# qq456cvb/CanonicalVoting

Measured on AMD Instinct MI355X. Metric: scenes/sec (80k-pt synthetic scans), higher is better.
Workload: dtype f32

## Files before the change

canonicalvoting_amd/_lib.py:

```python
import ctypes
import os
import threading

_HERE = os.path.dirname(os.path.abspath(__file__))
LIB_PATH = os.path.join(_HERE, "_C", "libcvhip.so")

c_float_p = ctypes.POINTER(ctypes.c_float)
c_int_p = ctypes.POINTER(ctypes.c_int)
c_i32_p = ctypes.POINTER(ctypes.c_int32)
c_i64_p = ctypes.POINTER(ctypes.c_int64)
vp = ctypes.c_void_p
ABI_VERSION = 6


class CvError(RuntimeError):
    pass


class DecodeParams(ctypes.Structure):
    _fields_ = [("thresh_high", ctypes.c_float), ("thresh_low", ctypes.c_float),
                ("valid_ratio", ctypes.c_float), ("elimination", ctypes.c_int),
                ("prob_thresh", ctypes.c_float), ("elim_hi_plus1", ctypes.c_int),
                ("max_iters", ctypes.c_int), ("err_thresh", ctypes.c_double)]

# ... 214 lines not shown
    "cv_hv_forward_workspace_bytes": (ctypes.c_size_t, [ctypes.c_int64, ctypes.c_int, c_int_p, ctypes.c_int]),
    "cv_hv_forward_f32": (ctypes.c_int, [vp, vp, vp, vp, ctypes.c_int64, ctypes.c_float, ctypes.c_int,
                                         c_float_p, c_int_p, vp, vp, vp, vp, ctypes.c_size_t,
                                         ctypes.c_int, vp]),
    "cv_hv_forward_cat_workspace_bytes": (ctypes.c_size_t, [ctypes.c_int64, ctypes.c_int, c_int_p, ctypes.c_int, ctypes.c_int]),
    "cv_hv_forward_cat_f32": (ctypes.c_int, [vp, vp, vp, vp, ctypes.c_int64, ctypes.c_float, ctypes.c_int, c_float_p, c_int_p,
                                             ctypes.c_int, vp, vp, vp, vp, ctypes.c_size_t, ctypes.c_int, vp]),
    "cv_hv_forward_peaks_f32": (ctypes.c_int, [vp, vp, vp, vp, ctypes.c_int64, ctypes.c_float, ctypes.c_int,
                                               c_float_p, c_int_p, vp, vp, vp, vp, ctypes.c_size_t,
                                               ctypes.c_int, ctypes.c_float, vp]),
    "cv_hv_forward_peaks_cat_f32": (ctypes.c_int, [vp, vp, vp, vp, ctypes.c_int64, ctypes.c_float, ctypes.c_int, c_float_p, c_int_p,
                                                   ctypes.c_int, vp, vp, vp, vp, ctypes.c_size_t, ctypes.c_int, ctypes.c_float,
                                                   vp]),
    "cv_hv_set_kernel_events": (ctypes.c_int, [vp, vp]),
    "cv_hv_backward_f32": (ctypes.c_int, [vp, vp, vp, vp, vp, ctypes.c_int64, ctypes.c_float,
                                          ctypes.c_int, c_float_p, c_int_p, vp, vp, vp, vp]),
    "cv_hv_count_votes_f32": (ctypes.c_int, [vp, vp, vp, ctypes.c_int64, ctypes.c_float, ctypes.c_int,
                                             c_float_p, c_int_p, c_i64_p, vp, ctypes.c_size_t, vp]),
    "cv_prop_workspace_bytes": (ctypes.c_size_t, [ctypes.c_int]),
    "cv_prop_columns_f32": (ctypes.c_int, [vp, c_int_p, ctypes.c_double, vp, vp, vp, vp, vp]),
    "cv_prop_select_f32": (ctypes.c_int, [ctypes.POINTER(PropSelectDesc), vp]),
    "cv_prop_cloud_ranges_i32": (ctypes.c_int, [vp, ctypes.c_longlong, ctypes.c_int, vp, vp, vp]),
    "cv_sizeof_prop_select_desc": (ctypes.c_size_t, []),
    "cv_decode_workspace_bytes": (ctypes.c_size_t, [c_int_p, ctypes.c_int64, ctypes.c_int]),
    "cv_decode_f32": (ctypes.c_int, [vp, vp, vp, c_int_p, c_float_p, ctypes.c_float, vp, vp, vp, vp,
                                     ctypes.c_int64, ctypes.POINTER(DecodeParams), ctypes.c_int, vp,
                                     ctypes.c_size_t, c_int_p, c_i64_p, c_i32_p, c_int_p, c_float_p,
                                     c_float_p, c_i32_p, c_int_p, vp]),
    "cv_decode_cat_workspace_bytes": (ctypes.c_size_t, [c_int_p, ctypes.c_int64, ctypes.c_int, ctypes.c_int]),
    "cv_decode_cat_f32": (ctypes.c_int, [vp, vp, vp, c_int_p, c_float_p, ctypes.c_float, vp, vp, vp, vp, ctypes.c_int64,
                                         ctypes.c_int, ctypes.POINTER(DecodeParams), ctypes.c_int, vp, ctypes.c_size_t, c_int_p,
                                         c_i64_p, c_i32_p, c_int_p, c_float_p, c_float_p, c_i32_p, c_int_p, vp]),
    "cv_detect_scene_separate_f32": (ctypes.c_int, [ctypes.POINTER(SceneSeparateDesc), ctypes.POINTER(SceneSeparateResult), vp]),
    "cv_sp_table_capacity": (ctypes.c_longlong, [ctypes.c_longlong]),
    "cv_sp_levels_workspace_bytes": (ctypes.c_size_t, [ctypes.c_longlong]),
    "cv_sp_build_levels": (ctypes.c_int, [ctypes.POINTER(vp), ctypes.POINTER(vp), ctypes.POINTER(vp),
                                          ctypes.c_longlong, ctypes.c_longlong, ctypes.c_int, vp,
                                          c_i32_p, vp, ctypes.c_size_t, vp]),
    "cv_sp_quantize_workspace_bytes": (ctypes.c_size_t, [ctypes.c_longlong]),
    "cv_sp_quantize_f32": (ctypes.c_int, [vp, ctypes.c_longlong, ctypes.c_longlong, ctypes.c_float, ctypes.c_int, c_i64_p,
                                          ctypes.c_int, vp, vp, vp, vp, c_i32_p, vp, ctypes.c_size_t, vp]),
    "cv_sp_quantize_f64": (ctypes.c_int, [vp, ctypes.c_longlong, ctypes.c_longlong, ctypes.c_double, ctypes.c_int, c_i64_p,
                                          ctypes.c_int, vp, vp, vp, vp, c_i32_p, vp, ctypes.c_size_t, vp]),
    "cv_sp_voxel_rows_f32": (ctypes.c_int, [vp, vp, ctypes.c_longlong, ctypes.c_float, vp, ctypes.POINTER(GatherJob), ctypes.c_int, vp]),
    "cv_sizeof_gather_job": (ctypes.c_size_t, []),
    "cv_sp_scan_rows_f32": (ctypes.c_int, [ctypes.POINTER(ScanRowsDesc), vp]),
    "cv_sizeof_scan_rows_desc": (ctypes.c_size_t, []),
    "cv_sym_loss_fwd_f32": (ctypes.c_int, [ctypes.POINTER(SymLossDesc), vp]),
    "cv_sym_loss_bwd_f32": (ctypes.c_int, [ctypes.POINTER(SymLossDesc), vp]),
    "cv_sym_loss_workspace_bytes": (ctypes.c_size_t, [ctypes.c_longlong, ctypes.c_int]),
    "cv_sym_loss_chunk_rows": (ctypes.c_int, []),
    "cv_sizeof_sym_loss_desc": (ctypes.c_size_t, []),
    "cv_row_loss_fwd_f32": (ctypes.c_int, [ctypes.POINTER(RowLossDesc), vp]),
    "cv_row_loss_bwd_f32": (ctypes.c_int, [ctypes.POINTER(RowLossDesc), vp]),
    "cv_row_loss_workspace_bytes": (ctypes.c_size_t, [ctypes.c_longlong]),
    "cv_row_loss_chunk_rows": (ctypes.c_int, []),
    "cv_sizeof_row_loss_desc": (ctypes.c_size_t, []),
    "cv_sp_sym_rows_f32": (ctypes.c_int, [ctypes.POINTER(SymRowsDesc), vp]),
    "cv_sp_sym_rows_workspace_bytes": (ctypes.c_size_t, [ctypes.c_longlong, ctypes.c_longlong, ctypes.c_int, ctypes.c_int]),
    "cv_sp_sym_rows_block": (ctypes.c_int, []),
    "cv_sp_sym_rows_scan_span": (ctypes.c_longlong, []),
    "cv_sizeof_sym_rows_desc": (ctypes.c_size_t, []),
    "cv_sp_morton_keys": (ctypes.c_int, [vp, ctypes.c_longlong, vp, vp]),
    "cv_sp_sort_workspace_bytes": (ctypes.c_size_t, [ctypes.c_longlong]),
    "cv_sp_sort_rows": (ctypes.c_int, [vp, ctypes.c_longlong, vp, vp, vp, vp, ctypes.c_size_t, vp]),
    "cv_sp_pack_weights_stem_h2_f32": (ctypes.c_int, [vp, ctypes.c_int, ctypes.c_int, vp, ctypes.c_int, vp, vp]),
    "cv_sp_to_hl_f32": (ctypes.c_int, [vp, ctypes.c_longlong, ctypes.c_int, ctypes.c_int, vp, ctypes.c_int, vp, vp]),
    "cv_sp_from_hl_f32": (ctypes.c_int, [vp, ctypes.c_longlong, ctypes.c_int, ctypes.c_int, vp, ctypes.c_int, vp]),
    "cv_sp_kernel_map": (ctypes.c_int, [vp, ctypes.c_longlong, vp, vp, ctypes.c_longlong, ctypes.c_int,
                                        ctypes.c_int, vp, vp]),
    "cv_sp_up_map": (ctypes.c_int, [vp, ctypes.c_longlong, ctypes.c_longlong, vp, vp]),
    "cv_sp_conv_workspace_bytes": (ctypes.c_size_t, [ctypes.c_longlong, ctypes.c_int, ctypes.c_int]),
    "cv_sp_conv_f32": (ctypes.c_int, [ctypes.POINTER(ConvDesc), vp]),
    "cv_sp_set_split_target": (ctypes.c_int, [ctypes.c_int]),
    "cv_hv_set_part_records": (ctypes.c_int, [ctypes.c_int]),
    "cv_hv_set_part_records_thread": (ctypes.c_int, [ctypes.c_int]),
    "cv_sp_pack_weights_h2_batch_f32": (ctypes.c_int, [ctypes.POINTER(PackJob), ctypes.c_int, vp, vp]),
    "cv_sp_copy_unless_flag": (ctypes.c_int, [ctypes.POINTER(vp), ctypes.POINTER(vp), ctypes.POINTER(ctypes.c_longlong), ctypes.c_int, vp, vp]),
    "cv_sp_pack_weights_t_f32": (ctypes.c_int, [vp, ctypes.c_int, ctypes.c_int, ctypes.c_int, ctypes.c_int, ctypes.c_int, vp, vp]),
    "cv_sp_set_split_target_thread": (ctypes.c_int, [ctypes.c_int]),
    "cv_sp_set_ablation": (ctypes.c_int, [ctypes.c_int]),
    "cv_sp_set_option": (ctypes.c_int, [ctypes.c_char_p, ctypes.c_longlong, ctypes.POINTER(ctypes.c_longlong)]),
    "cv_sp_get_option": (ctypes.c_int, [ctypes.c_char_p, ctypes.POINTER(ctypes.c_longlong)]),
    "cv_sp_pack_weights_x6_f32": (ctypes.c_int, [vp, ctypes.c_int, ctypes.c_int, ctypes.c_int, vp, vp, vp]),
    "cv_sp_pack_weights_h2_f32": (ctypes.c_int, [vp, ctypes.c_int, ctypes.c_int, ctypes.c_int, vp, ctypes.c_int, vp, vp]),
    "cv_sp_pack_weights_bf16_f32": (ctypes.c_int, [vp, ctypes.c_int, ctypes.c_int, ctypes.c_int, vp, vp, vp]),
    "cv_sp_scene_maps_words": (ctypes.c_size_t, [c_i64_p, ctypes.c_longlong, ctypes.c_int, ctypes.c_int,
                                                 ctypes.c_longlong, ctypes.POINTER(SceneMaps)]),
    "cv_sp_scene_maps": (ctypes.c_int, [ctypes.POINTER(vp), ctypes.POINTER(vp), ctypes.POINTER(vp), ctypes.c_longlong,
                                        c_i64_p, vp, ctypes.c_longlong, ctypes.c_int,
                                        ctypes.c_int, ctypes.c_longlong, vp, ctypes.c_size_t, vp]),
    "cv_sp_scene_plan_words": (ctypes.c_size_t, [ctypes.c_longlong, ctypes.c_int, ctypes.c_int, ctypes.c_longlong]),
    "cv_sp_scene_plan": (ctypes.c_int, [vp, ctypes.c_longlong, vp, vp, ctypes.POINTER(vp), ctypes.POINTER(vp),
                                        ctypes.POINTER(vp), ctypes.c_longlong, vp, c_i32_p, ctypes.c_int, ctypes.c_int,
                                        ctypes.c_longlong, vp, ctypes.c_size_t, ctypes.POINTER(SceneMaps), vp,
                                        ctypes.c_size_t, vp, ctypes.c_size_t, vp]),
    "cv_sp_scene_plan_layout": (ctypes.c_int, [ctypes.c_longlong, ctypes.c_int, ctypes.c_int, ctypes.c_longlong,
                                               ctypes.POINTER(ScenePlanLayout)]),
    "cv_sp_scene_plan_slots": (ctypes.c_int, [ctypes.POINTER(ScenePlanLayout), ctypes.POINTER(SceneMaps), c_i64_p,
                                              ctypes.c_longlong, vp, ctypes.POINTER(vp), ctypes.POINTER(vp)]),
    "cv_sp_scene_conv_workspace_bytes": (ctypes.c_size_t, [c_i64_p, c_int_p, ctypes.c_int, ctypes.c_int]),
    "cv_net_arena_bytes": (ctypes.c_size_t, [ctypes.POINTER(NetBuf), ctypes.c_int, c_i64_p, ctypes.c_int]),
    "cv_net_run_f32": (ctypes.c_int, [ctypes.POINTER(NetOp), ctypes.c_int, ctypes.POINTER(NetBuf), ctypes.c_int,
                                      c_i64_p, ctypes.c_int, vp, ctypes.c_size_t, ctypes.POINTER(vp), c_int_p,
                                      ctypes.POINTER(vp), ctypes.c_int, ctypes.POINTER(vp), ctypes.c_int,
                                      vp, ctypes.c_size_t, vp, vp]),
    "cv_net_models_params_bytes": (ctypes.c_size_t, [ctypes.c_int, ctypes.c_int]),
    "cv_net_models_params_fill": (ctypes.c_int, [ctypes.POINTER(vp), ctypes.c_int, ctypes.c_int, vp, ctypes.c_size_t]),
    "cv_net_models_arena_bytes": (ctypes.c_size_t, [ctypes.POINTER(NetBuf), ctypes.c_int, c_i64_p, ctypes.c_int, ctypes.c_int]),
    "cv_net_models_workspace_bytes": (ctypes.c_size_t, [ctypes.c_size_t, ctypes.c_int]),
    "cv_net_run_models_f32": (ctypes.c_int, [ctypes.POINTER(vp), ctypes.POINTER(vp), ctypes.c_int, ctypes.c_int, ctypes.c_int,
                                             c_i64_p, ctypes.c_int, vp, ctypes.c_size_t, ctypes.POINTER(vp), c_int_p,
                                             ctypes.POINTER(vp), ctypes.c_int, ctypes.POINTER(vp), ctypes.c_int,
                                             vp, ctypes.c_size_t, vp, vp, ctypes.c_int, vp]),
    "cv_head_separate_models_f32": (ctypes.c_int, [ctypes.POINTER(vp), ctypes.c_int, ctypes.c_longlong, ctypes.c_int, ctypes.c_int,
                                                   vp, vp, vp, vp]),
    "cv_sp_mask_keys": (ctypes.c_int, [vp, ctypes.c_longlong, ctypes.c_int, ctypes.c_int, ctypes.c_int, vp, vp]),
    "cv_sp_mask_perms": (ctypes.c_int, [vp, ctypes.c_longlong, ctypes.c_int, ctypes.c_int, vp, vp, ctypes.c_size_t,
                                        ctypes.c_int, vp]),
    "cv_sp_transpose_map": (ctypes.c_int, [vp, ctypes.c_longlong, ctypes.c_int, ctypes.c_longlong, vp, vp]),
    "cv_sp_wgrad_workspace_bytes": (ctypes.c_size_t, [ctypes.c_longlong, ctypes.c_int, ctypes.c_int, ctypes.c_int]),
    "cv_sp_conv_wgrad_f32": (ctypes.c_int, [vp, ctypes.c_int, ctypes.c_int, vp, ctypes.c_int, ctypes.c_int, vp,
                                            ctypes.c_int, ctypes.c_longlong, vp, vp, ctypes.c_size_t, vp]),
    "cv_sp_conv_wgrad_px_f32": (ctypes.c_int, [vp, ctypes.c_int, ctypes.c_int, vp, ctypes.c_int, ctypes.c_int, vp,
                                               ctypes.c_int, ctypes.c_longlong, vp, vp, ctypes.c_size_t, ctypes.c_int,
                                               vp]),
    "cv_sp_col_sum_f32": (ctypes.c_int, [vp, ctypes.c_longlong, ctypes.c_int, ctypes.c_int, vp, vp]),
    "cv_sp_col_sum_workspace_bytes": (ctypes.c_size_t, [ctypes.c_longlong, ctypes.c_int]),
    "cv_sp_col_sum_det_f32": (ctypes.c_int, [vp, ctypes.c_longlong, ctypes.c_int, ctypes.c_int, vp, vp, ctypes.c_size_t, vp]),
    "cv_sp_bn_workspace_bytes": (ctypes.c_size_t, [ctypes.c_int]),
    "cv_sp_bn_stats_f32": (ctypes.c_int, [vp, ctypes.c_longlong, ctypes.c_int, ctypes.c_int, vp, vp, ctypes.c_float,
                                          ctypes.c_float, vp, vp, vp, vp, vp, vp, vp, ctypes.c_size_t, vp]),
    "cv_sp_bn_backward_f32": (ctypes.c_int, [vp, vp, vp, ctypes.c_longlong, ctypes.c_int, ctypes.c_int, vp, vp,
                                             ctypes.c_float, vp, vp, vp, vp, vp, vp, ctypes.c_size_t, vp]),
    "cv_sp_bn_backward_hl_f32": (ctypes.c_int, [vp, vp, vp, ctypes.c_longlong, ctypes.c_int, ctypes.c_int, vp, vp,
                                                ctypes.c_float, vp, vp, vp, vp, vp, vp, ctypes.c_size_t, vp, vp, vp, vp, vp]),
    "cv_sp_affine_f32": (ctypes.c_int, [vp, ctypes.c_longlong, ctypes.c_int, ctypes.c_int, vp, vp, vp, ctypes.c_int,
                                        ctypes.c_int, vp, ctypes.c_int, vp]),
    "cv_sp_affine_hl_f32": (ctypes.c_int, [vp, ctypes.c_longlong, ctypes.c_int, ctypes.c_int, vp, vp, vp, ctypes.c_int,
                                           ctypes.c_int, vp, ctypes.c_int, vp, ctypes.c_int, vp, vp, vp]),
    "cv_sp_bn_fold_f32": (ctypes.c_int, [vp, vp, vp, vp, vp, ctypes.c_float, ctypes.c_int, vp, vp, vp]),
    "cv_head_joint_f32": (ctypes.c_int, [vp, ctypes.c_longlong, ctypes.c_int, ctypes.c_int, ctypes.c_int,
                                         vp, vp, vp, vp, vp]),
    "cv_head_separate_f32": (ctypes.c_int, [vp, ctypes.c_longlong, ctypes.c_int, ctypes.c_int, vp, vp, vp, vp]),
    "cv_detect_scene_f32": (ctypes.c_int, [ctypes.POINTER(SceneDesc), ctypes.POINTER(SceneResult), vp]),
    "cv_detect_points_f32": (ctypes.c_int, [ctypes.POINTER(PointsDesc), ctypes.POINTER(PointsResult), vp]),
    "cv_detect_points_separate_f32": (ctypes.c_int, [ctypes.POINTER(PointsSeparateDesc), ctypes.POINTER(PointsSeparateResult), vp]),
    "cv_sizeof_points_desc": (ctypes.c_size_t, []),
    "cv_sizeof_points_separate_desc": (ctypes.c_size_t, []),
    "cv_sizeof_points_result": (ctypes.c_size_t, []),
    "cv_sizeof_points_separate_result": (ctypes.c_size_t, []),
    "cv_iou_obb": (ctypes.c_double, [c_float_p, c_float_p]),
    "cv_nms_obb": (ctypes.c_int, [c_float_p, c_float_p, ctypes.c_int, ctypes.c_double, c_i32_p]),
}

_lib = None


def lib():
    global _lib
    if _lib is None:
        if not os.path.exists(LIB_PATH):
            raise CvError(
                "canonicalvoting_amd: HIP library %s not found. Build it with "
                "`python -m canonicalvoting_amd.csrc.build` (hipcc, gfx950). There is no CPU "
                "fallback for this op." % LIB_PATH)
# ... 60 lines not shown
```

canonicalvoting_amd/csrc/conv_prep.hip:

```cpp
#include "cv_common.h"

#include <algorithm>

#include "sparse_conv_common.h"

using namespace cvsc;

namespace {

__global__ __launch_bounds__(256) void pack_weights_h2(const float* __restrict__ w, int K, int cin, int cout,
                                                       const float* __restrict__ col_scale, float mult,
                                                       unsigned short* __restrict__ wp, int trans = 0) {
    const long long total = (long long)K * cin * cout / 2;
    const int nch = cin / 32;
    for (long long i = blockIdx.x * 256ll + threadIdx.x; i < total; i += (long long)gridDim.x * 256) {
        long long r = i;
        const int k2 = (int)(r % 16); r /= 16;
        const int col = (int)(r % cout); r /= cout;
        const int c = (int)(r % nch); r /= nch;
        const int j = (int)r;
        const float* p = trans ? w + ((long long)j * cout + col) * cin + c * 32 + 2 * k2
                               : w + ((long long)j * cin + c * 32 + 2 * k2) * cout + col;
        const float sc = (col_scale ? col_scale[col] : 1.f) * mult;
        unsigned h, l;
// ... 30 lines not shown

__global__ __launch_bounds__(256) void pack_weights_x6(const float* __restrict__ w, int K, int cin, int cout,
                                                       const float* __restrict__ col_scale,
                                                       unsigned short* __restrict__ wp, int trans = 0) {
    const long long total = (long long)K * cin * cout / 2;
    const int nch = cin / 32;
    for (long long i = blockIdx.x * 256ll + threadIdx.x; i < total; i += (long long)gridDim.x * 256) {
        long long r = i;
        const int k2 = (int)(r % 16); r /= 16;
        const int col = (int)(r % cout); r /= cout;
        const int c = (int)(r % nch); r /= nch;
        const int j = (int)r;
        const float* p = trans ? w + ((long long)j * cout + col) * cin + c * 32 + 2 * k2
                               : w + ((long long)j * cin + c * 32 + 2 * k2) * cout + col;
        unsigned h, m, l;
        const float sc = col_scale ? col_scale[col] : 1.f;
        split3(p[0] * sc, p[trans ? 1 : cout] * sc, h, m, l);
        const long long base = ((long long)(j * nch + c) * 3 * cout + col) * 32 + 2 * k2;
        *reinterpret_cast<unsigned*>(wp + base) = h;
        *reinterpret_cast<unsigned*>(wp + base + (long long)cout * 32) = m;
        *reinterpret_cast<unsigned*>(wp + base + 2ll * cout * 32) = l;
    }
}

__global__ __launch_bounds__(256) void pack_weights_b1(const float* __restrict__ w, int K, int cin, int cout,
                                                       const float* __restrict__ col_scale,
                                                       unsigned short* __restrict__ wp, int trans = 0) {
    const long long total = (long long)K * cin * cout / 2;
    const int nch = cin / 32;
    for (long long i = blockIdx.x * 256ll + threadIdx.x; i < total; i += (long long)gridDim.x * 256) {
        long long r = i;
        const int k2 = (int)(r % 16); r /= 16;
        const int col = (int)(r % cout); r /= cout;
        const int c = (int)(r % nch); r /= nch;
        const int j = (int)r;
        const float* p = trans ? w + ((long long)j * cout + col) * cin + c * 32 + 2 * k2
                               : w + ((long long)j * cin + c * 32 + 2 * k2) * cout + col;
        const float sc = col_scale ? col_scale[col] : 1.f;
        *reinterpret_cast<unsigned*>(wp + ((long long)(j * nch + c) * cout + col) * 32 + 2 * k2) =
            cvt_pk_bf16(p[0] * sc, p[trans ? 1 : cout] * sc);
    }
}

__global__ __launch_bounds__(256) void pack_weights_stem_h2(const float* __restrict__ w, int K, int cin,
                                                            const float* __restrict__ col_scale, float mult,
                                                            unsigned short* __restrict__ wp) {
    const int total = 8 * cin * 32 * 2 * 4;
    for (int t = blockIdx.x * 256 + threadIdx.x; t < total; t += gridDim.x * 256) {
        int r = t;
        const int q = r % 4; r /= 4;
        const int hf = r % 2; r /= 2;
        const int col = r % 32; r /= 32;
        const int ci = r % cin; r /= cin;
        const int g = r;
        const int j0 = g * 16 + hf * 8 + 2 * q;
        const float sc = (col_scale ? col_scale[col] : 1.f) * mult;
        const float v0 = j0 < K ? w[((long long)j0 * cin + ci) * 32 + col] * sc : 0.f;
        const float v1 = j0 + 1 < K ? w[((long long)(j0 + 1) * cin + ci) * 32 + col] * sc : 0.f;
        unsigned h, l;
        split2h(v0, v1, h, l);
        const long long base = ((((long long)(g * cin + ci) * 2) * 32 + col) * 2 + hf) * 8 + 2 * q;
        *reinterpret_cast<unsigned*>(wp + base) = h;
        *reinterpret_cast<unsigned*>(wp + base + 512) = l;
    }
}

__global__ __launch_bounds__(256) void mask_keys(const int* __restrict__ nbr, long long n, int K, int j_begin,
                                                 int j_end, long long* __restrict__ keys) {
    const long long i = blockIdx.x * 256ll + threadIdx.x;
    if (i >= n) return;
    unsigned long long m = 0;
    for (int j = j_begin; j < j_end; ++j)
        if (nbr[i * K + j] >= 0) m |= 1ull << (j - j_begin);
    keys[i] = (long long)m;
}

constexpr int MP_BINS = 1024;
constexpr int MP_THREADS = 1024;

__device__ __forceinline__ int group_mask(const int* __restrict__ nbr, long long row, long long n, int K, int jb, int je) {
    int m = 0;
    for (int j = jb; j < je; ++j)
        if (nbr[row * K + j] >= 0) m |= 1 << (j - jb);
    if (je - jb <= 7) m |= __popc(m) << 7;
    (void)n;
    return m;
}

__device__ __forceinline__ int group_mask_of_word(int word, int jb, int je) {
    int m = (int)(((unsigned)word >> jb) & ((1u << (je - jb)) - 1u));
    if (je - jb <= 7) m |= __popc(m) << 7;
    return m;
}

__global__ __launch_bounds__(MP_THREADS) void mp_hist(const int* __restrict__ nbr, long long n, int K, int groups,
                                                      int* __restrict__ hist ) {
    __shared__ int lh[MP_BINS];
    const int g = blockIdx.y;
    const int jb = K * g / groups, je = K * (g + 1) / groups;
    for (int i = threadIdx.x; i < MP_BINS; i += MP_THREADS) lh[i] = 0;
    __syncthreads();
    const long long row = blockIdx.x * (long long)MP_THREADS + threadIdx.x;
    if (row < n) atomicAdd(&lh[group_mask(nbr, row, n, K, jb, je)], 1);
    __syncthreads();
    for (int i = threadIdx.x; i < MP_BINS; i += MP_THREADS)
        if (lh[i]) atomicAdd(&hist[g * MP_BINS + i], lh[i]);
}

__global__ __launch_bounds__(MP_BINS) void mp_scan(int* __restrict__ hist) {
    __shared__ int s[MP_BINS];
    int* h = hist + blockIdx.x * MP_BINS;
    const int v = h[threadIdx.x];
    s[threadIdx.x] = v;
    __syncthreads();
    for (int off = 1; off < MP_BINS; off <<= 1) {
        const int t = threadIdx.x >= off ? s[threadIdx.x - off] : 0;
        __syncthreads();
        s[threadIdx.x] += t;
        __syncthreads();
    }
    h[threadIdx.x] = s[threadIdx.x] - v;
}

__global__ __launch_bounds__(MP_THREADS) void mp_scatter(const int* __restrict__ nbr, long long n, int K, int groups,
                                                         int* __restrict__ cursor, int* __restrict__ perm,
                                                         int* __restrict__ nbrp, int W) {
    unsigned char* gv = nbrp ? reinterpret_cast<unsigned char*>(nbrp + (long long)groups * n * W) : nullptr;
    __shared__ int lh[MP_BINS];
    const int g = blockIdx.y;
    const int jb = K * g / groups, je = K * (g + 1) / groups;
    for (int i = threadIdx.x; i < MP_BINS; i += MP_THREADS) lh[i] = 0;
    __syncthreads();
    const long long row = blockIdx.x * (long long)MP_THREADS + threadIdx.x;
    int key = 0, rank = 0;
    if (row < n) {
        key = group_mask(nbr, row, n, K, jb, je);
        rank = atomicAdd(&lh[key], 1);
    }
    __syncthreads();
    for (int i = threadIdx.x; i < MP_BINS; i += MP_THREADS)
        if (lh[i]) lh[i] = atomicAdd(&cursor[g * MP_BINS + i], lh[i]);
    __syncthreads();
    if (row < n) {
        const long long pos = (long long)g * n + lh[key] + rank;
        perm[pos] = (int)row;
        if (nbrp) {
            for (int j = jb; j < je; ++j) nbrp[pos * W + (j - jb)] = nbr[row * K + j];
            gv[(long long)g * n + row] = key != 0;
        }
    }
}

struct PermJobsDev {
    CvPermJob j[CV_MAX_PERM_JOBS];
    int group_begin[CV_MAX_PERM_JOBS + 1];
    int n;
};

__device__ __forceinline__ int perm_job_of(const PermJobsDev& jobs, int gy) {
    int ji = 0;
    while (ji + 1 < jobs.n && gy >= jobs.group_begin[ji + 1]) ++ji;
    return ji;
}

__global__ __launch_bounds__(MP_THREADS) void mp_hist_batch(const PermJobsDev jobs, int* __restrict__ hist) {
    __shared__ int lh[MP_BINS];
    const int ji = perm_job_of(jobs, blockIdx.y);
    const CvPermJob& jb = jobs.j[ji];
    const long long row = blockIdx.x * (long long)MP_THREADS + threadIdx.x;
    if (blockIdx.x * (long long)MP_THREADS >= jb.n) return;
    const int g = blockIdx.y - jobs.group_begin[ji];
    const int jlo = jb.K * g / jb.groups, jhi = jb.K * (g + 1) / jb.groups;
    for (int i = threadIdx.x; i < MP_BINS; i += MP_THREADS) lh[i] = 0;
    __syncthreads();
// ... 230 lines not shown
```

canonicalvoting_amd/csrc/cv_common.h:

```cpp
#pragma once
#include <hip/hip_runtime.h>

#include <cstdarg>
#include <cstdint>
#include <cstdio>

#include "cv_hip.h"

void cv_set_error(const char* fmt, ...);

#define CV_HIP_CHECK(expr)                                                                  \
    do {                                                                                    \
        hipError_t e_ = (expr);                                                             \
        if (e_ != hipSuccess) {                                                             \
            cv_set_error("%s failed: %s (%s:%d)", #expr, hipGetErrorString(e_), __FILE__,   \
                         __LINE__);                                                         \
            return CV_EHIP;                                                                 \
        }                                                                                   \
    } while (0)

#define CV_LAUNCH_CHECK() CV_HIP_CHECK(hipGetLastError())

#define CV_REQUIRE(cond, code, ...)     \
    do {                                \
        if (!(cond)) {                  \
            cv_set_error(__VA_ARGS__);  \
            return (code);              \
        }                               \
    } while (0)

__host__ __device__ static inline size_t cv_align_up(size_t v, size_t a) { return (v + a - 1) / a * a; }

struct CvCarver {
    char* base;
    size_t off = 0;
    explicit CvCarver(void* p) : base(static_cast<char*>(p)) {}
    template <typename T>
    T* take(size_t count) {
        off = cv_align_up(off, 256);
        T* r = reinterpret_cast<T*>(base + off);
        off += count * sizeof(T);
        return r;
    }
};

struct CvMapJob {
    const int32_t* out_coords; long long n_out;
    const unsigned long long* keys; const int32_t* vals; long long cap;
    int k, ts;
    int32_t* nbr;
    const int32_t* compose;
    const unsigned* bitmap;
    const int32_t* bbox;
    int up;
    int32_t* nbr3;
    int32_t* mask_words;
};
constexpr int CV_MAX_MAP_JOBS = 12;
int cv_sp_kernel_maps_batch(const CvMapJob* jobs, int n_jobs, void* stream);
constexpr long long CV_BITMAP_WORDS = 1ll << 20;

int cv_sp_build_levels_zero(int32_t* const* d_coords, unsigned long long* const* d_keys, int32_t* const* d_vals,
                            long long n, long long cap, int num_levels, int32_t* d_counts, int32_t* h_counts, void* d_ws,
                            size_t ws_bytes, int32_t* d_zero, long long n_zero, int32_t* d_bbox, uint32_t* d_bits,
                            void* stream);

struct CvPermJob {
    const int32_t* nbr; long long n; int K, groups; int32_t* perm; int with_map;
    const int32_t* mask_words;
};
constexpr int CV_MAX_PERM_JOBS = 8;
int cv_hv_minmax_async_ex(const float* d_points, int64_t n, float* h_minmax6, void* d_ws, size_t ws_bytes, int32_t* d_zero_word,
                          int32_t* d_fill7f, void* stream);
struct DecodeCall {
    float* d_grid_obj; const float* d_grid_rot; const float* d_grid_scale;
    const int* dims; const float* h_corner3; float res;
    const float* d_points; const float* d_xyz; const float* d_prob; const int32_t* d_class; int64_t n;
    const cv_decode_params* params; int mutate_grid;
    void* d_ws; size_t ws_bytes;
    int* h_n_cand; int64_t* h_cand_idx; int32_t* h_verdict; int* h_n_boxes; float* h_boxes; float* h_scores; int32_t* h_classes;
    int* h_truncated;
    void* stream; void* ev_done;
};
int cv_decode_run(const DecodeCall& c, int num_cats, bool need_class);
int cv_sp_sort_rows_ex(const int32_t* d_coords, long long n, int32_t* d_sorted, int32_t* d_perm, int32_t* d_inv, void* d_ws,
                       size_t ws_bytes, bool single_batch, void* stream, bool bounds_prefilled);
int cv_sp_scene_plan_ex(const int32_t* d_input, long long n, int32_t* d_perm, int32_t* d_inv, int32_t* const* d_coords,
                        unsigned long long* const* d_keys, int32_t* const* d_vals, long long cap, int32_t* d_counts,
                        int32_t* h_counts, int stem_k, int mask_groups, long long masked_min_rows,
                        int32_t* d_arena, size_t arena_words, cv_scene_maps* offsets, void* d_sort_ws, size_t sort_ws_bytes,
                        void* d_levels_ws, size_t levels_ws_bytes, bool single_batch, void* stream,
                        bool bounds_prefilled);
int cv_net_run_ex(const cv_net_op* ops, int n_ops, const cv_net_buf* bufs, int n_bufs, const long long* level_rows,
                  int n_levels, void* d_arena, size_t arena_bytes, const void* const* ext_ptr, const int* ext_ld,
                  const int32_t* const* maps, int n_maps, const int32_t* const* perms, int n_perms,
                  void* d_ws, size_t ws_bytes, int32_t* range_flag, bool plan_maps, void* stream);
int cv_net_run_models_ex(const cv_net_op* const* ops, const cv_net_buf* const* bufs, int n_ops, int n_bufs, int K,
                         const long long* level_rows, int n_levels, void* d_arena, size_t arena_bytes,
                         const void* const* const* ext_ptr, const int* ext_ld, const int32_t* const* maps, int n_maps,
                         const int32_t* const* perms, int n_perms, void* d_ws, size_t ws_bytes, int32_t* range_flag,
                         const void* d_params, int params_ld, bool plan_maps, void* stream);
int cv_sp_mask_perms_batch(const CvPermJob* jobs, int n_jobs, void* d_ws, size_t ws_bytes, void* stream,
                           bool pre_zeroed);

struct CvConvModels {
    int models;
    const cv_net_model_params* d_params;
    long long in_stride, in2_stride, res_stride, out_stride, ws_stride;
    int out_ext;
    float* ext_out[CV_MAX_CATEGORIES];
};
int cv_sp_conv_models_f32(const cv_conv_desc* d, const CvConvModels* mm, void* stream);
```

canonicalvoting_amd/csrc/net_exec.cpp:

```cpp
#include <algorithm>
#include <mutex>
#include <unordered_map>
#include <vector>

#include "cv_common.h"

namespace {

struct Slot { char* ptr; int ld; long long rows; int ext; };

struct NetModels {
    int K;
    const void* const* const* ext_ptr;
    size_t arena_stride, ws_stride;
    const cv_net_model_params* d_params;
    int params_ld;
};

int net_run(const cv_net_op* ops, int n_ops, const cv_net_buf* bufs, int n_bufs, const long long* level_rows, int n_levels,
            void* d_arena, size_t arena_bytes, const void* const* ext_ptr, const int* ext_ld, const int32_t* const* maps,
            int n_maps, const int32_t* const* perms, int n_perms, void* d_ws, size_t ws_bytes, int32_t* range_flag,
            const NetModels* nm, bool plan_maps, void* stream);

}

extern "C" {

static void scene_maps_layout(const long long* rows, int stem_k, int mask_groups, long long masked_min_rows, cv_scene_maps* o,
                              size_t* total) {
    size_t off = 0;
    auto take = [&](size_t words) { const size_t at = off; off += cv_align_up(words, 64); return (long long)at; };
    const size_t K5 = (size_t)stem_k * stem_k * stem_k;
    const size_t mp_w = mask_groups > 1 ? (size_t)mask_groups * (1 + (27 + mask_groups - 1) / mask_groups) + (mask_groups + 3) / 4 : 0;
    o->stem = take((size_t)rows[0] * K5);
    o->k3[0] = take((size_t)rows[0] * 28);
    o->mask_perm[0] = (mask_groups > 1 && rows[0] >= masked_min_rows) ? take(mp_w * rows[0]) : -1;
    o->scratch = take((size_t)(5 * std::max(mask_groups, 1) + 4) * 2048);
    o->bitmap = take((size_t)CV_BITMAP_WORDS);
    o->out = -1;
    for (int i = 0; i < 4; ++i) o->down[i] = take((size_t)rows[i + 1] * 8);
    for (int i = 1; i < 5; ++i) o->k3[i] = take((size_t)rows[i] * 28);
    for (int i = 0; i < 4; ++i) o->up[i] = take((size_t)rows[3 - i] * 8);
    for (int i = 1; i < 5; ++i) o->mask_perm[i] = (mask_groups > 1 && rows[i] >= masked_min_rows) ? take(mp_w * rows[i]) : -1;
    for (int i = 0; i < 4; ++i) o->up_perm[i] = take((size_t)rows[3 - i]);
    *total = off;
}

static int32_t* scene_mask_words(int32_t* d_arena, const cv_scene_maps& o, int level, long long rows) {
    return d_arena + o.k3[level] + rows * 27;
}

size_t cv_sp_scene_maps_words(const long long* level_rows, long long n_orig, int stem_k, int mask_groups,
                              long long masked_min_rows, cv_scene_maps* offsets) {
    if (!level_rows || !offsets || n_orig <= 0 || stem_k < 1) return 0;
    size_t total = 0;
    scene_maps_layout(level_rows, stem_k, mask_groups, masked_min_rows, offsets, &total);
    return total;
}

static int scene_maps_level0(int32_t* const* d_coords, const unsigned long long* const* d_keys, const int32_t* const* d_vals,
                             long long cap, long long n, const int32_t* d_perm, int stem_k, int mask_groups,
                             const cv_scene_maps& o, int32_t* d_arena, const int32_t* d_bbox, void* stream) {
    const unsigned* bits = d_bbox ? reinterpret_cast<const unsigned*>(d_arena + o.bitmap) : nullptr;
    CvMapJob mj[2];
    int32_t* mw = scene_mask_words(d_arena, o, 0, n);
    int nm = 1;
    if (stem_k == 5) {
        mj[0] = {d_coords[0], n, d_keys[0], d_vals[0], cap, 5, 1, d_arena + o.stem, d_perm, bits, d_bbox, 0, d_arena + o.k3[0], mw};
    } else {
        mj[0] = {d_coords[0], n, d_keys[0], d_vals[0], cap, stem_k, 1, d_arena + o.stem, d_perm, bits, d_bbox, 0, nullptr, nullptr};
        mj[1] = {d_coords[0], n, d_keys[0], d_vals[0], cap, 3, 1, d_arena + o.k3[0], nullptr, bits, d_bbox, 0, nullptr, mw};
        nm = 2;
    }
    int rc = cv_sp_kernel_maps_batch(mj, nm, stream);
    if (rc != CV_OK) return rc;
    if (o.mask_perm[0] >= 0) {
        CvPermJob pj = {d_arena + o.k3[0], n, 27, mask_groups, d_arena + o.mask_perm[0], 1, mw};
        rc = cv_sp_mask_perms_batch(&pj, 1, d_arena + o.scratch, sizeof(int) * (size_t)mask_groups * 2048, stream,
                                     d_bbox != nullptr);
        if (rc != CV_OK) return rc;
    }
    return CV_OK;
}

static int scene_maps_coarse(int32_t* const* d_coords, const unsigned long long* const* d_keys, const int32_t* const* d_vals,
                             long long cap, const long long* level_rows, int mask_groups, const cv_scene_maps& o,
                             int32_t* d_arena, void* stream, bool from_plan) {
    CvMapJob mj[CV_MAX_MAP_JOBS];
    int nm = 0;
    for (int i = 0; i < 4; ++i)
        mj[nm++] = {d_coords[i + 1], level_rows[i + 1], d_keys[i], d_vals[i], cap, 2, 1 << i, d_arena + o.down[i], nullptr, nullptr, nullptr, 0,
                    nullptr, nullptr};
    for (int i = 1; i < 5; ++i)
        mj[nm++] = {d_coords[i], level_rows[i], d_keys[i], d_vals[i], cap, 3, 1 << i, d_arena + o.k3[i], nullptr, nullptr, nullptr, 0,
                    nullptr, o.mask_perm[i] >= 0 ? scene_mask_words(d_arena, o, i, level_rows[i]) : nullptr};
    for (int i = 0; i < 4; ++i) {
        const int fine = 3 - i;
        mj[nm++] = {d_coords[fine], level_rows[fine], d_keys[fine + 1], d_vals[fine + 1], cap, 2, 1 << fine, d_arena + o.up[i],
                    nullptr, nullptr, nullptr, 1, nullptr, nullptr};
    }
    int rc = cv_sp_kernel_maps_batch(mj, nm, stream);
    if (rc != CV_OK) return rc;
    CvPermJob pj[CV_MAX_PERM_JOBS];
    int np = 0, groups = 0;
    for (int i = 1; i < 5; ++i)
        if (o.mask_perm[i] >= 0) {
            pj[np++] = {d_arena + o.k3[i], level_rows[i], 27, mask_groups, d_arena + o.mask_perm[i], 1,
                        scene_mask_words(d_arena, o, i, level_rows[i])};
            groups += mask_groups;
        }
    for (int i = 0; i < 4; ++i) {
        pj[np++] = {d_arena + o.up[i], level_rows[3 - i], 8, 1, d_arena + o.up_perm[i], 0, nullptr};
        groups += 1;
    }
    return cv_sp_mask_perms_batch(pj, np, d_arena + o.scratch + (size_t)std::max(mask_groups, 1) * 2048,
                                  sizeof(int) * (size_t)groups * 2048, stream,  from_plan);
}

int cv_sp_scene_maps(int32_t* const* d_coords, const unsigned long long* const* d_keys, const int32_t* const* d_vals,
                     long long cap, const long long* level_rows, const int32_t* d_perm, long long n_orig, int stem_k,
                     int mask_groups, long long masked_min_rows, int32_t* d_arena, size_t arena_words, void* stream) {
    CV_REQUIRE(d_coords && d_keys && d_vals && level_rows && d_perm && d_arena, CV_EINVAL, "null pointer argument");
    CV_REQUIRE(n_orig == level_rows[0], CV_EINVAL, "the sorted set must hold the caller's %lld rows", n_orig);
    cv_scene_maps o;
    size_t total = 0;
    scene_maps_layout(level_rows, stem_k, mask_groups, masked_min_rows, &o, &total);
    CV_REQUIRE(arena_words >= total, CV_ENOMEM, "scene map arena too small");
    int rc = scene_maps_level0(d_coords, d_keys, d_vals, cap, n_orig, d_perm, stem_k, mask_groups, o, d_arena,
                                nullptr, stream);
    if (rc != CV_OK) return rc;
    return scene_maps_coarse(d_coords, d_keys, d_vals, cap, level_rows, mask_groups, o, d_arena, stream,  false);
}

namespace {
struct PlanSide { hipEvent_t ev; int32_t* h_pinned; int device; };
std::mutex g_plan_mu;
std::unordered_map<int, std::vector<PlanSide>> g_plan_free;
int plan_side_acquire(PlanSide* out) {
    int dev = 0;
    CV_HIP_CHECK(hipGetDevice(&dev));
    {
        std::lock_guard<std::mutex> lk(g_plan_mu);
        auto& pool = g_plan_free[dev];
        if (!pool.empty()) {
            *out = pool.back();
            pool.pop_back();
            return CV_OK;
        }
    }
    PlanSide p{};
    p.device = dev;
    CV_HIP_CHECK(hipEventCreateWithFlags(&p.ev, hipEventDisableTiming));
    CV_HIP_CHECK(hipHostMalloc(reinterpret_cast<void**>(&p.h_pinned), 64, hipHostMallocDefault));
    *out = p;
    return CV_OK;
}
struct PlanSideLease {
    PlanSide ps{};
    bool held = false;
    ~PlanSideLease() {
        if (!held) return;
        (void)hipEventSynchronize(ps.ev);
        std::lock_guard<std::mutex> lk(g_plan_mu);
        g_plan_free[ps.device].push_back(ps);
    }
};
}

size_t cv_sp_scene_plan_words(long long n, int stem_k, int mask_groups, long long masked_min_rows) {
    if (n <= 0 || stem_k < 1) return 0;
    const long long rows[5] = {n, n, n, n, n};
    cv_scene_maps o;
    size_t total = 0;
    scene_maps_layout(rows, stem_k, mask_groups, masked_min_rows, &o, &total);
    return total;
}

int cv_sp_scene_plan_layout(long long n, int stem_k, int mask_groups, long long masked_min_rows, cv_scene_plan_layout* out) {
    CV_REQUIRE(out && n > 0, CV_EINVAL, "bad scene plan layout arguments");
    auto up64 = [](long long v) { return (v + 63) / 64 * 64; };
    cv_scene_plan_layout& l = *out;
    l.cap = cv_sp_table_capacity(n);
    l.perm = 0, l.inv = up64(n);
    for (int i = 0; i < 5; ++i) l.coords[i] = l.inv + up64(n) + i * up64(4 * n);
    for (int i = 0; i < 5; ++i) l.vals[i] = l.coords[4] + up64(4 * n) + i * up64(l.cap);
    l.counts = l.vals[4] + up64(l.cap), l.arena = l.counts + 64;
    l.int_words = l.arena + (long long)cv_sp_scene_plan_words(n, stem_k, mask_groups, masked_min_rows);
    l.key_words = 5 * l.cap;
    l.sort_ws_bytes = cv_sp_sort_workspace_bytes(n), l.levels_ws_bytes = cv_sp_levels_workspace_bytes(n);
    return CV_OK;
}

int cv_sp_scene_plan_slots(const cv_scene_plan_layout* layout, const cv_scene_maps* offsets, const long long* level_rows,
                           long long min_rows, const int32_t* d_ibuf, const int32_t** maps, const int32_t** perms) {
    CV_REQUIRE(layout && offsets && level_rows && maps && perms, CV_EINVAL, "null pointer argument");
    const cv_scene_maps& off = *offsets;
    const int32_t* ap = d_ibuf + layout->arena;
    maps[0] = ap + off.stem;
    for (int i = 0; i < 4; ++i) maps[1 + i] = ap + off.down[i];
    for (int i = 0; i < 5; ++i) maps[5 + i] = ap + off.k3[i];
    for (int i = 0; i < 4; ++i) maps[10 + i] = ap + off.up[i];
    maps[14] = d_ibuf + layout->inv;
    for (int i = 0; i < 5; ++i) perms[i] = (off.mask_perm[i] >= 0 && level_rows[i] >= min_rows) ? ap + off.mask_perm[i] : nullptr;
    for (int i = 0; i < 4; ++i) perms[5 + i] = ap + off.up_perm[i];
    return CV_OK;
}

size_t cv_sp_scene_conv_workspace_bytes(const long long* level_rows, const int* masked, int mask_groups, int max_channels) {
    if (!level_rows || !masked) return 0;
    size_t bytes = 0;
    for (int i = 0; i < 5; ++i) {
        if (masked[i]) bytes = std::max(bytes, (size_t)4 * mask_groups * (size_t)level_rows[i] * max_channels + 256);
        bytes = std::max(bytes, cv_sp_conv_workspace_bytes(std::min<long long>(level_rows[i], 128 * 384 - 1), max_channels, 27));
    }
    return bytes;
}

int cv_sp_scene_plan(const int32_t* d_input, long long n, int32_t* d_perm, int32_t* d_inv, int32_t* const* d_coords,
                     unsigned long long* const* d_keys, int32_t* const* d_vals, long long cap, int32_t* d_counts,
                     int32_t* h_counts, int stem_k, int mask_groups, long long masked_min_rows, int32_t* d_arena,
                     size_t arena_words, cv_scene_maps* offsets, void* d_sort_ws, size_t sort_ws_bytes, void* d_levels_ws,
                     size_t levels_ws_bytes, void* stream) {
    return cv_sp_scene_plan_ex(d_input, n, d_perm, d_inv, d_coords, d_keys, d_vals, cap, d_counts, h_counts, stem_k, mask_groups,
                               masked_min_rows, d_arena, arena_words, offsets, d_sort_ws, sort_ws_bytes, d_levels_ws,
                               levels_ws_bytes,  false, stream,  false);
}

}

int cv_sp_scene_plan_ex(const int32_t* d_input, long long n, int32_t* d_perm, int32_t* d_inv, int32_t* const* d_coords,
                        unsigned long long* const* d_keys, int32_t* const* d_vals, long long cap, int32_t* d_counts,
                        int32_t* h_counts, int stem_k, int mask_groups, long long masked_min_rows,
                        int32_t* d_arena, size_t arena_words, cv_scene_maps* offsets, void* d_sort_ws, size_t sort_ws_bytes,
                        void* d_levels_ws, size_t levels_ws_bytes, bool single_batch, void* stream, bool bounds_prefilled) {
    CV_REQUIRE(d_input && d_perm && d_inv && d_coords && d_keys && d_vals && d_counts && h_counts && d_arena && offsets &&
                   d_sort_ws && d_levels_ws, CV_EINVAL, "null pointer argument");
    CV_REQUIRE(arena_words >= cv_sp_scene_plan_words(n, stem_k, mask_groups, masked_min_rows), CV_ENOMEM,
               "scene map arena too small (cv_sp_scene_plan_words)");
    hipStream_t st = static_cast<hipStream_t>(stream);
    int rc = cv_sp_sort_rows_ex(d_input, n, d_coords[0], d_perm, d_inv, d_sort_ws, sort_ws_bytes, single_batch, stream, bounds_prefilled);
    if (rc != CV_OK) return rc;
    long long rows[5] = {n, 1, 1, 1, 1};
    cv_scene_maps o;
    size_t total = 0;
    scene_maps_layout(rows, stem_k, mask_groups, masked_min_rows, &o, &total);
    int32_t* d_bbox = static_cast<int32_t*>(d_sort_ws);
    rc = cv_sp_build_levels_zero(d_coords, d_keys, d_vals, n, cap, 5, d_counts, nullptr, d_levels_ws, levels_ws_bytes,
                                 d_arena + o.scratch, o.bitmap + CV_BITMAP_WORDS - o.scratch, d_bbox,
                                 reinterpret_cast<uint32_t*>(d_arena + o.bitmap), stream);
    if (rc != CV_OK) return rc;
    PlanSideLease lease;
    rc = plan_side_acquire(&lease.ps);
    if (rc != CV_OK) return rc;
    lease.held = true;
    const PlanSide& ps = lease.ps;
    CV_HIP_CHECK(hipMemcpyAsync(ps.h_pinned, d_counts, sizeof(int32_t) * 8, hipMemcpyDeviceToHost, st));
    CV_HIP_CHECK(hipEventRecord(ps.ev, st));
    rc = scene_maps_level0(d_coords, d_keys, d_vals, cap, n, d_perm, stem_k, mask_groups, o, d_arena, d_bbox, stream);
    if (rc != CV_OK) return rc;
    CV_HIP_CHECK(hipEventSynchronize(ps.ev));
    for (int i = 0; i < 8; ++i) h_counts[i] = ps.h_pinned[i];
    if (h_counts[5] != 0 || h_counts[6] != 0) return CV_OK;
    for (int i = 0; i < 5; ++i) rows[i] = h_counts[i];
    CV_REQUIRE(rows[0] == n, CV_EINVAL, "level 0 lost rows (%lld of %lld)", rows[0], n);
    scene_maps_layout(rows, stem_k, mask_groups, masked_min_rows, &o, &total);
    CV_REQUIRE(arena_words >= total, CV_ENOMEM, "scene map arena too small");
    *offsets = o;
    return scene_maps_coarse(d_coords, d_keys, d_vals, cap, rows, mask_groups, o, d_arena, stream,  true);
}

extern "C" {

size_t cv_net_arena_bytes(const cv_net_buf* bufs, int n_bufs, const long long* level_rows, int n_levels) {
    if (!bufs || !level_rows || n_bufs <= 0) return 0;
    size_t total = 256;
    for (int i = 0; i < n_bufs; ++i) {
        if (bufs[i].level < 0 || bufs[i].level >= n_levels) continue;
        total += cv_align_up(sizeof(float) * (size_t)level_rows[bufs[i].level] * (size_t)bufs[i].channels, 256);
    }
    return total;
}

int cv_net_run_f32(const cv_net_op* ops, int n_ops, const cv_net_buf* bufs, int n_bufs, const long long* level_rows,
                   int n_levels, void* d_arena, size_t arena_bytes, const void* const* ext_ptr, const int* ext_ld,
                   const int32_t* const* maps, int n_maps, const int32_t* const* perms, int n_perms,
                   void* d_ws, size_t ws_bytes, int32_t* range_flag, void* stream) {
    return cv_net_run_ex(ops, n_ops, bufs, n_bufs, level_rows, n_levels, d_arena, arena_bytes, ext_ptr, ext_ld, maps, n_maps, perms,
                         n_perms, d_ws, ws_bytes, range_flag,  false, stream);
}

}

int cv_net_run_ex(const cv_net_op* ops, int n_ops, const cv_net_buf* bufs, int n_bufs, const long long* level_rows,
                  int n_levels, void* d_arena, size_t arena_bytes, const void* const* ext_ptr, const int* ext_ld,
                  const int32_t* const* maps, int n_maps, const int32_t* const* perms, int n_perms,
                  void* d_ws, size_t ws_bytes, int32_t* range_flag, bool plan_maps, void* stream) {
    return net_run(ops, n_ops, bufs, n_bufs, level_rows, n_levels, d_arena, arena_bytes, ext_ptr, ext_ld, maps, n_maps, perms,
                   n_perms, d_ws, ws_bytes, range_flag, nullptr, plan_maps, stream);
}

extern "C" {

size_t cv_net_models_params_bytes(int n_ops, int K) {
    if (n_ops <= 0 || K < 1 || K > CV_MAX_CATEGORIES) return 0;
    return sizeof(cv_net_model_params) * (size_t)n_ops * (size_t)K;
}

int cv_net_models_params_fill(const cv_net_op* const* ops, int n_ops, int K, void* h_params, size_t params_bytes) {
    CV_REQUIRE(K >= 1 && K <= CV_MAX_CATEGORIES, CV_EINVAL, "number of models out of range (%d, 1..%d)", K, CV_MAX_CATEGORIES);
    CV_REQUIRE(ops && h_params && n_ops > 0, CV_EINVAL, "bad model table arguments");
    CV_REQUIRE(params_bytes >= cv_net_models_params_bytes(n_ops, K), CV_ENOMEM, "model table too small (cv_net_models_params_bytes)");
    for (int m = 0; m < K; ++m) CV_REQUIRE(ops[m], CV_EINVAL, "model %d: null program", m);
    cv_net_model_params* t = static_cast<cv_net_model_params*>(h_params);
    for (int k = 0; k < n_ops; ++k)
        for (int m = 0; m < K; ++m) {
            const cv_net_op& o = ops[m][k];
            t[(size_t)k * K + m] = {o.weight_x6, o.weight2_x6, o.scale, o.shift, o.acc_scale != 0.f ? o.acc_scale : 1.f, {0, 0, 0}};
        }
    return CV_OK;
}

size_t cv_net_models_arena_bytes(const cv_net_buf* bufs, int n_bufs, const long long* level_rows, int n_levels, int K) {
    if (K < 1 || K > CV_MAX_CATEGORIES) return 0;
    return (size_t)K * cv_net_arena_bytes(bufs, n_bufs, level_rows, n_levels);
}

size_t cv_net_models_workspace_bytes(size_t one_model_bytes, int K) {
    if (K < 1 || K > CV_MAX_CATEGORIES) return 0;
    return (size_t)(K - 1) * cv_align_up(one_model_bytes, 256) + one_model_bytes;
}

int cv_net_run_models_f32(const cv_net_op* const* ops, const cv_net_buf* const* bufs, int n_ops, int n_bufs, int K,
                          const long long* level_rows, int n_levels, void* d_arena, size_t arena_bytes,
                          const void* const* const* ext_ptr, const int* ext_ld, const int32_t* const* maps, int n_maps,
                          const int32_t* const* perms, int n_perms, void* d_ws, size_t ws_bytes, int32_t* range_flag,
                          const void* d_params, int params_ld, void* stream) {
    return cv_net_run_models_ex(ops, bufs, n_ops, n_bufs, K, level_rows, n_levels, d_arena, arena_bytes, ext_ptr, ext_ld, maps, n_maps,
                                perms, n_perms, d_ws, ws_bytes, range_flag, d_params, params_ld,  false, stream);
}

}

int cv_net_run_models_ex(const cv_net_op* const* ops, const cv_net_buf* const* bufs, int n_ops, int n_bufs, int K,
                         const long long* level_rows, int n_levels, void* d_arena, size_t arena_bytes,
                         const void* const* const* ext_ptr, const int* ext_ld, const int32_t* const* maps, int n_maps,
                         const int32_t* const* perms, int n_perms, void* d_ws, size_t ws_bytes, int32_t* range_flag,
                         const void* d_params, int params_ld, bool plan_maps, void* stream) {
    CV_REQUIRE(K >= 1 && K <= CV_MAX_CATEGORIES, CV_EINVAL, "number of models out of range (%d, 1..%d)", K, CV_MAX_CATEGORIES);
    CV_REQUIRE(ops && bufs && level_rows && d_arena && ext_ptr && n_ops > 0 && n_bufs > 0 && n_levels > 0, CV_EINVAL,
               "bad network program arguments");
    CV_REQUIRE(d_params, CV_EINVAL, "null model parameter table (cv_net_models_params_fill)");
    CV_REQUIRE(params_ld >= K, CV_EINVAL, "params_ld (%d) is smaller than the number of models (%d)", params_ld, K);
    for (int m = 0; m < K; ++m)
        CV_REQUIRE(ops[m] && bufs[m] && ext_ptr[m], CV_EINVAL, "model %d: null program, buffer list or pointer table", m);
    for (int m = 1; m < K; ++m) {
        for (int i = 0; i < n_bufs; ++i) {
            const cv_net_buf &x = bufs[0][i], &y = bufs[m][i];
            CV_REQUIRE(x.level == y.level && x.channels == y.channels && x.rows_level == y.rows_level && x.hl == y.hl, CV_EINVAL,
                       "buffer %d of model %d differs from model 0's: the programs are not structurally identical", i, m);
        }
        for (int k = 0; k < n_ops; ++k) {
            const cv_net_op &x = ops[0][k], &y = ops[m][k];
            const bool same = x.in_buf == y.in_buf && x.in_col == y.in_col && x.cin == y.cin && x.out_buf == y.out_buf &&
                              x.out_col == y.out_col && x.cout == y.cout && x.res_buf == y.res_buf && x.res_col == y.res_col &&
                              x.map == y.map && x.K == y.K && x.perm == y.perm && x.perm_groups == y.perm_groups &&
                              x.relu == y.relu && x.in2_buf == y.in2_buf && x.in2_col == y.in2_col && x.cin2 == y.cin2 &&
                              x.weight_pieces == y.weight_pieces && !x.weight == !y.weight && !x.scale == !y.scale &&
                              !x.shift == !y.shift && !x.weight_x6 == !y.weight_x6 && !x.weight2_x6 == !y.weight2_x6;
            CV_REQUIRE(same, CV_EINVAL, "op %d of model %d differs from model 0's: the programs are not structurally identical", k, m);
        }
    }
    for (int k = 0; k < n_ops; ++k)
        for (int m = 0; m < K; ++m) {
            const cv_net_op& o = ops[m][k];
            CV_REQUIRE(o.weight_pieces == 2, CV_EINVAL, "op %d: the model axis runs fp16-pair programs only (weight_pieces == 2)", k);
            CV_REQUIRE(((reinterpret_cast<uintptr_t>(o.scale) | reinterpret_cast<uintptr_t>(o.shift) |
                         reinterpret_cast<uintptr_t>(o.weight_x6) | reinterpret_cast<uintptr_t>(o.weight2_x6)) & 15) == 0, CV_EINVAL,
                       "op %d of model %d: scale, shift and packed weights must be 16-byte aligned", k, m);
        }
    const size_t arena_one = cv_net_arena_bytes(bufs[0], n_bufs, level_rows, n_levels);
    CV_REQUIRE(arena_bytes >= (size_t)K * arena_one, CV_ENOMEM, "arena too small (cv_net_models_arena_bytes)");
    const size_t ws_stride = K > 1 ? (ws_bytes / (size_t)K) & ~(size_t)255 : 0;
    const size_t ws_one = K > 1 ? ws_stride : ws_bytes;
    NetModels nm = {K, ext_ptr, arena_one, ws_stride, static_cast<const cv_net_model_params*>(d_params), params_ld};
    return net_run(ops[0], n_ops, bufs[0], n_bufs, level_rows, n_levels, d_arena, arena_one, ext_ptr[0], ext_ld, maps, n_maps,
                   perms, n_perms, d_ws, ws_one, range_flag, &nm, plan_maps, stream);
}

namespace {

int net_run(const cv_net_op* ops, int n_ops, const cv_net_buf* bufs, int n_bufs, const long long* level_rows, int n_levels,
            void* d_arena, size_t arena_bytes, const void* const* ext_ptr, const int* ext_ld, const int32_t* const* maps,
            int n_maps, const int32_t* const* perms, int n_perms, void* d_ws, size_t ws_bytes, int32_t* range_flag,
            const NetModels* nm, bool plan_maps, void* stream) {
    CV_REQUIRE(ops && bufs && level_rows && d_arena && n_ops > 0 && n_bufs > 0 && n_levels > 0, CV_EINVAL,
               "bad network program arguments");
    CV_REQUIRE(arena_bytes >= cv_net_arena_bytes(bufs, n_bufs, level_rows, n_levels), CV_ENOMEM, "arena too small");
    std::vector<Slot> slot((size_t)n_bufs);
    {
        CvCarver cv(d_arena);
        int ext = 0;
        for (int i = 0; i < n_bufs; ++i) {
            const int lv = bufs[i].level;
            if (lv < 0 || lv >= n_levels) {
                CV_REQUIRE(ext_ptr && ext_ld && ext_ptr[ext], CV_EINVAL, "external buffer %d has no pointer", ext);
                slot[i] = {static_cast<char*>(const_cast<void*>(ext_ptr[ext])), ext_ld[ext], bufs[i].rows_level >= 0 &&
                           bufs[i].rows_level < n_levels ? level_rows[bufs[i].rows_level] : 0, ext};
                if (nm)
                    for (int m = 1; m < nm->K; ++m)
                        CV_REQUIRE(nm->ext_ptr[m][ext], CV_EINVAL, "external buffer %d of model %d has no pointer", ext, m);
                ++ext;
            } else {
                slot[i] = {reinterpret_cast<char*>(cv.take<float>((size_t)level_rows[lv] * bufs[i].channels)),
                           bufs[i].channels, level_rows[lv], -1};
            }
        }
    }
    for (int k = 0; k < n_ops; ++k) {
        const cv_net_op& o = ops[k];
        CV_REQUIRE(o.in_buf >= 0 && o.in_buf < n_bufs && o.out_buf >= 0 && o.out_buf < n_bufs &&
                       o.res_buf < n_bufs && o.map < n_maps && o.perm < n_perms, CV_EINVAL, "op %d: bad slot", k);
        const Slot& in = slot[o.in_buf];
        const Slot& out = slot[o.out_buf];
        cv_conv_desc d = {};
        d.in_hl = bufs[o.in_buf].hl;
        d.out_hl = bufs[o.out_buf].hl;
        d.res_hl = o.res_buf >= 0 ? bufs[o.res_buf].hl : 0;
        CV_REQUIRE(o.in2_buf < 0 || bufs[o.in2_buf].hl == d.in_hl, CV_EINVAL, "op %d: both sources must share a format", k);
        d.in = reinterpret_cast<const float*>(in.ptr) + o.in_col;
        d.n_in = in.rows;
        d.in_ld = in.ld;
        d.cin = o.cin;
        d.weight = o.weight;
        d.weight_x6 = o.weight_x6;
        d.weight_pieces = o.weight_pieces;
        d.acc_scale = o.acc_scale;
        d.range_flag = (o.weight_pieces == 2 || d.out_hl) ? range_flag : nullptr;
        if (o.in2_buf >= 0) {
            CV_REQUIRE(o.in2_buf < n_bufs, CV_EINVAL, "op %d: bad second-source slot", k);
            d.in2 = reinterpret_cast<const float*>(slot[o.in2_buf].ptr) + o.in2_col;
            d.in2_ld = slot[o.in2_buf].ld;
            d.cin2 = o.cin2;
            d.weight2_x6 = o.weight2_x6;
        }
        d.K = o.K;
        d.cout = o.cout;
        d.nbr = o.map >= 0 ? maps[o.map] : nullptr;
        d.n_out = out.rows;
        d.scale = o.scale;
        d.shift = o.shift;
        if (o.res_buf >= 0) {
            d.residual = reinterpret_cast<const float*>(slot[o.res_buf].ptr) + o.res_col;
            d.res_ld = slot[o.res_buf].ld;
        }
        d.relu = o.relu;
        d.out = reinterpret_cast<float*>(out.ptr) + o.out_col;
        d.out_ld = out.ld;
        d.ws = d_ws;
        d.ws_bytes = ws_bytes;
        const int32_t* perm = o.perm >= 0 ? perms[o.perm] : nullptr;
        if (perm) {
            d.row_perm = perm;
            d.perm_groups = o.perm_groups;
            d.perm_has_map = o.perm_groups > 1;
            if (plan_maps && d.perm_has_map && o.K == 27 && d.nbr) d.valid_words = d.nbr + out.rows * 27;
        }
        int rc;
        if (nm) {
            CvConvModels cm = {};
            cm.models = nm->K;
            cm.d_params = nm->d_params + (size_t)k * nm->params_ld;
            cm.ws_stride = (long long)nm->ws_stride;
            auto stride_of = [&](int buf, long long* stride) -> int {
                const int e = slot[buf].ext;
                if (e < 0) { *stride = (long long)nm->arena_stride; return CV_OK; }
                for (int m = 1; m < nm->K; ++m)
                    CV_REQUIRE(nm->ext_ptr[m][e] == nm->ext_ptr[0][e], CV_EINVAL,
                               "op %d: the external buffer it reads must be the same tensor for every model (model %d differs)", k, m);
                *stride = 0;
                return CV_OK;
            };
            if ((rc = stride_of(o.in_buf, &cm.in_stride)) != CV_OK) return rc;
            if (o.in2_buf >= 0 && (rc = stride_of(o.in2_buf, &cm.in2_stride)) != CV_OK) return rc;
            if (o.res_buf >= 0 && (rc = stride_of(o.res_buf, &cm.res_stride)) != CV_OK) return rc;
            if (out.ext >= 0) {
                cm.out_ext = 1;
                for (int m = 0; m < nm->K; ++m) {
                    float* p = reinterpret_cast<float*>(const_cast<void*>(nm->ext_ptr[m][out.ext])) + o.out_col;
                    CV_REQUIRE((reinterpret_cast<uintptr_t>(p) & 15) == 0, CV_EINVAL, "op %d: output of model %d is not 16-byte aligned", k, m);
                    cm.ext_out[m] = p;
                }
            } else {
                cm.out_stride = (long long)nm->arena_stride;
            }
            rc = cv_sp_conv_models_f32(&d, &cm, stream);
        } else {
            rc = cv_sp_conv_f32(&d, stream);
        }
        if (rc != CV_OK) return rc;
    }
    return CV_OK;
}

}
```

canonicalvoting_amd/csrc/scene_exec.cpp:

```cpp
#include <algorithm>
#include <atomic>
#include <chrono>
#include <cstdlib>
#include <cstring>
#include <vector>

#include "cv_common.h"

namespace {

struct Carver {
    char* base; size_t off = 0, cap;
    Carver(void* p, size_t c) : base(static_cast<char*>(p)), cap(c) {}
    template <typename T> T* take(size_t count) {
        off = cv_align_up(off, 256);
        T* r = (base && off + count * sizeof(T) <= cap) ? reinterpret_cast<T*>(base + off) : nullptr;
        off += count * sizeof(T);
        return r;
    }
};

std::atomic<int> g_scenes_inside{0};
struct SceneCount {
    int before;
    bool set_target, set_records;
    int prev_target = 0, prev_records = 0;
    SceneCount(bool adaptive, int split_target, int part_records)
        : before(g_scenes_inside.fetch_add(1, std::memory_order_relaxed)), set_target(adaptive || split_target > 0),
          set_records(part_records > 0) {
        if (set_target) prev_target = cv_sp_set_split_target_thread(split_target > 0 ? split_target : before + 1 >= 4 ? 256 : 768);
        if (set_records) prev_records = cv_hv_set_part_records_thread(part_records);
    }
    ~SceneCount() {
        if (set_target) cv_sp_set_split_target_thread(prev_target);
        if (set_records) cv_hv_set_part_records_thread(prev_records);
        g_scenes_inside.fetch_sub(1, std::memory_order_relaxed);
    }
};

struct StageClock {
    void* const* events; hipStream_t st; float* host_us;
    std::chrono::steady_clock::time_point t_prev = std::chrono::steady_clock::now();
    hipError_t mark(int i) const { return events[i] ? hipEventRecord(static_cast<hipEvent_t>(events[i]), st) : hipSuccess; }
    void lap(int i) {
        const auto t = std::chrono::steady_clock::now();
        host_us[i] += std::chrono::duration<float, std::micro>(t - t_prev).count();
        t_prev = t;
    }
};

struct SceneFront {
    const int32_t* d_coords4; long long n; const float* d_points; float res;
    int stem_k, mask_groups; long long masked_min_rows; int max_channels;
    float* h_minmax;
    cv_scene_plan_layout lay;
    void* mm_ws; int32_t* ibuf; unsigned long long* kbuf; char* sort_ws; char* lev_ws;
    cv_scene_maps off;
    long long rows[5];
    float mn[3]; int dims[3]; size_t cells;
    const int32_t* maps[CV_NET_MAP_SLOTS]; const int32_t* perms[CV_NET_PERM_SLOTS];
    size_t conv_ws_b;

    template <class D> explicit SceneFront(const D* d)
        : d_coords4(d->d_coords4), n(d->n), d_points(d->d_points), res(d->res), stem_k(d->stem_k), mask_groups(d->mask_groups),
          masked_min_rows(d->masked_min_rows), max_channels(d->max_channels), h_minmax(static_cast<float*>(d->h_pinned)) {}

    bool carve(Carver& cv) {
        mm_ws = cv.take<char>(cv_hv_minmax_workspace_bytes());
        cv_sp_scene_plan_layout(n, stem_k, mask_groups, masked_min_rows, &lay);
        ibuf = cv.take<int32_t>((size_t)lay.int_words);
        kbuf = cv.take<unsigned long long>((size_t)lay.key_words);
        sort_ws = cv.take<char>(lay.sort_ws_bytes);
        lev_ws = cv.take<char>(lay.levels_ws_bytes);
        return mm_ws && ibuf && kbuf && sort_ws && lev_ws;
    }

    template <class R> int run(int32_t* d_zero_word, R* r, StageClock& clock, void* stream) {
        int rc = cv_hv_minmax_async_ex(d_points, n, h_minmax, mm_ws, cv_hv_minmax_workspace_bytes(), d_zero_word,
                                       reinterpret_cast<int32_t*>(sort_ws), stream);
        if (rc != CV_OK) return rc;
        int32_t *c_coords[5], *c_vals[5];
        unsigned long long* c_keys[5];
        for (int i = 0; i < 5; ++i) {
            c_coords[i] = ibuf + lay.coords[i];
            c_keys[i] = kbuf + (size_t)lay.cap * i;
            c_vals[i] = ibuf + lay.vals[i];
        }
        int32_t counts_h[8] = {0};
        rc = cv_sp_scene_plan_ex(d_coords4, n, ibuf + lay.perm, ibuf + lay.inv, c_coords, c_keys, c_vals, lay.cap, ibuf + lay.counts,
                                 counts_h, stem_k, mask_groups, masked_min_rows, ibuf + lay.arena, (size_t)(lay.int_words - lay.arena),
                                 &off, sort_ws, lay.sort_ws_bytes, lev_ws, lay.levels_ws_bytes,
                                  true, stream,  true);
        if (rc != CV_OK) return rc;
        r->duplicates = counts_h[5];
        r->out_of_window = counts_h[6];
        CV_REQUIRE(counts_h[5] == 0 && counts_h[6] == 0, CV_EINVAL,
                   "duplicate coordinates (%d) or coordinates outside the 16-bit key window (%d)", counts_h[5], counts_h[6]);
        clock.lap(0);
        for (int i = 0; i < 5; ++i) { rows[i] = counts_h[i]; r->level_rows[i] = counts_h[i]; }
        float mx[3];
        for (int k = 0; k < 3; ++k) { mn[k] = h_minmax[k]; mx[k] = h_minmax[3 + k]; r->corner[k] = mn[k]; }
        rc = cv_hv_grid_dims_f32(mn, mx, res, dims);
        if (rc != CV_OK) return rc;
        for (int k = 0; k < 3; ++k) r->dims[k] = dims[k];
        cells = (size_t)dims[0] * dims[1] * dims[2];
        int masked[5];
        for (int i = 0; i < 5; ++i) masked[i] = off.mask_perm[i] >= 0;
        conv_ws_b = cv_sp_scene_conv_workspace_bytes(rows, masked, mask_groups, max_channels);
        return cv_sp_scene_plan_slots(&lay, &off, rows, masked_min_rows, ibuf, maps, perms);
    }
};

template <class R> int fixed_part_too_small(R* r, size_t fixed_end) {
    r->needed_ws_bytes = fixed_end * 2 + ((size_t)256 << 20);
    cv_set_error("scene workspace too small (needs at least %zu bytes)", r->needed_ws_bytes);
    return CV_ENOMEM;
}

}

extern "C" {

int cv_detect_scene_f32(const cv_scene_desc* d, cv_scene_result* r, void* stream) {
    CV_REQUIRE(d && r, CV_EINVAL, "null scene descriptor / result");
    CV_REQUIRE(d->d_coords4 && d->d_feats && d->d_points && d->n > 0 && d->ops && d->bufs && d->n_ops > 0 && d->n_bufs > 0,
               CV_EINVAL, "bad scene descriptor");
    CV_REQUIRE(d->d_out_feats && d->out_ld >= d->out_channels && d->out_channels > 0, CV_EINVAL, "bad network output buffer");
    CV_REQUIRE(d->h_pinned && d->pinned_bytes >= 256 && d->d_ws, CV_EINVAL, "pinned scratch (>= 256 bytes) and a device workspace are required");
    CV_REQUIRE(d->h_boxes && d->h_scores && d->h_classes && d->h_cand_idx && d->h_verdict && d->h_pick && d->max_candidates > 0,
               CV_EINVAL, "null result arrays");
    hipStream_t st = static_cast<hipStream_t>(stream);
    const long long n = d->n;
    std::memset(r, 0, sizeof(*r));
    CV_REQUIRE(d->conv_split_target >= 0 && d->vote_part_records >= 0, CV_EINVAL, "negative launch sizing");
    CV_REQUIRE(d->vote_algo >= 0 && d->vote_algo <= 2, CV_EINVAL, "vote_algo out of range (%d: 0 auto, 1 direct, 2 tiles)", d->vote_algo);
    SceneCount in_flight(d->adaptive_split != 0, d->conv_split_target, d->vote_part_records);
    r->scenes_in_flight = in_flight.before + 1;
    Carver cv(d->d_ws, d->ws_bytes);
    StageClock clock{d->events, st, r->host_us};
    CV_HIP_CHECK(clock.mark(0));

    SceneFront f(d);
    int32_t* h_flag = reinterpret_cast<int32_t*>(static_cast<char*>(d->h_pinned) + 64);
    const bool plan_fits = f.carve(cv);
    float* xyz = cv.take<float>((size_t)n * 3);
    float* scale = cv.take<float>((size_t)n * 3);
    float* prob = cv.take<float>((size_t)n);
    int32_t* cls = cv.take<int32_t>((size_t)n);
    int32_t* d_flag = cv.take<int32_t>(64);
    if (!plan_fits || !xyz || !scale || !prob || !cls || !d_flag) return fixed_part_too_small(r, cv.off);
    int rc = f.run(d_flag, r, clock, stream);
    if (rc != CV_OK) return rc;
    const size_t cells = f.cells;

    const size_t arena_b = cv_net_arena_bytes(d->bufs, d->n_bufs, f.rows, 5);
    const size_t vote_ws_b = cv_hv_forward_workspace_bytes(n, d->num_rots, f.dims, d->vote_algo);
    const size_t dec_ws_b = cv_decode_workspace_bytes(f.dims, n, d->max_candidates);
    char* arena = cv.take<char>(arena_b);
    char* conv_ws = cv.take<char>(f.conv_ws_b);
    char* vote_ws = cv.take<char>(std::max<size_t>(vote_ws_b, 256));
    char* dec_ws = cv.take<char>(dec_ws_b);
    float* grids = d->d_grids ? d->d_grids : cv.take<float>(6 * cells);
    r->needed_ws_bytes = cv.off + 4096;
    r->needed_grid_floats = 6 * cells;
    CV_REQUIRE(arena && conv_ws && vote_ws && dec_ws && grids, CV_ENOMEM, "scene workspace too small (needs %zu bytes)", r->needed_ws_bytes);
    CV_REQUIRE(!d->d_grids || d->grid_capacity_floats >= 6 * cells, CV_ENOMEM, "grid buffer too small (needs %zu floats)", 6 * cells);
    float* g_obj = grids;
    float* g_rot = grids + cells;
    float* g_scale = grids + 3 * cells;
    r->d_grid_obj = g_obj; r->d_grid_rot = g_rot; r->d_grid_scale = g_scale;

    const void* ext_ptr[2] = {d->d_feats, d->d_out_feats};
    const int ext_ld[2] = {d->feats_ld, d->out_ld};
    rc = cv_net_run_ex(d->ops, d->n_ops, d->bufs, d->n_bufs, f.rows, 5, arena, arena_b, ext_ptr, ext_ld, f.maps, CV_NET_MAP_SLOTS,
                       f.perms, CV_NET_PERM_SLOTS, conv_ws, f.conv_ws_b, d->use_range_flag ? d_flag : nullptr,  true, stream);
    if (rc != CV_OK) return rc;
    clock.lap(1);
    CV_HIP_CHECK(clock.mark(1));
    rc = cv_head_joint_f32(d->d_out_feats, n, d->out_ld, d->nclasses, d->log_scale, xyz, scale, prob, cls, stream);
    if (rc != CV_OK) return rc;
    if (d->use_range_flag) CV_HIP_CHECK(hipMemcpyAsync(h_flag, d_flag, sizeof(int32_t), hipMemcpyDeviceToHost, st));
    r->d_xyz = xyz; r->d_scale = scale; r->d_prob = prob; r->d_class = cls;
    CV_HIP_CHECK(clock.mark(2));

    const float* v_xyz = d->d_xyz_in ? d->d_xyz_in : xyz;
    const float* v_scale = d->d_scale_in ? d->d_scale_in : scale;
    const float* v_prob = d->d_prob_in ? d->d_prob_in : prob;
    const int32_t* v_cls = d->d_class_in ? d->d_class_in : cls;
    rc = d->peak_quotients
             ? cv_hv_forward_peaks_f32(d->d_points, v_xyz, v_scale, v_prob, n, d->res, d->num_rots, f.mn, f.dims, g_obj, g_rot, g_scale,
                                       vote_ws, std::max<size_t>(vote_ws_b, 256), d->vote_algo, d->decode.thresh_high, stream)
             : cv_hv_forward_f32(d->d_points, v_xyz, v_scale, v_prob, n, d->res, d->num_rots, f.mn, f.dims, g_obj, g_rot, g_scale, vote_ws,
                                 std::max<size_t>(vote_ws_b, 256), d->vote_algo, stream);
    if (rc != CV_OK) return rc;
    CV_HIP_CHECK(clock.mark(3));
    clock.lap(2);
    cv_decode_params prm = d->decode;
    prm.max_iters = d->max_candidates;
    int n_cand = 0, n_boxes = 0, truncated = 0;
    const DecodeCall dc{g_obj, g_rot, g_scale, f.dims, f.mn, d->res, d->d_points, v_xyz, v_prob, v_cls, n, &prm, 0, dec_ws, dec_ws_b, &n_cand,
                        d->h_cand_idx, d->h_verdict, &n_boxes, d->h_boxes, d->h_scores, d->h_classes, &truncated, stream, d->events[4]};
    rc = cv_decode_run(dc, 1, true);
    if (rc != CV_OK) return rc;
    r->n_cand = n_cand;
    r->n_boxes = n_boxes;
    r->truncated = truncated;
    r->range_flag = d->use_range_flag ? *h_flag : 0;

    int n_det = 0;
    std::vector<float> bc, sc;
    std::vector<int32_t> idx, pick;
    for (int c = 0; c < d->nclasses; ++c) {
        bc.clear(); sc.clear(); idx.clear();
        for (int i = 0; i < n_boxes; ++i)
            if (d->h_classes[i] == c) {
                bc.insert(bc.end(), d->h_boxes + (size_t)i * 24, d->h_boxes + (size_t)i * 24 + 24);
                sc.push_back(d->h_scores[i]);
                idx.push_back(i);
            }
        if (idx.empty()) continue;
        pick.assign(idx.size(), 0);
        const int k = cv_nms_obb(bc.data(), sc.data(), (int)idx.size(), d->nms_threshold, pick.data());
        if (k < 0) return k;
        for (int j = 0; j < k; ++j) d->h_pick[n_det++] = idx[(size_t)pick[j]];
    }
    r->n_det = n_det;
    clock.lap(3);
    return CV_OK;
}

int cv_detect_scene_separate_f32(const cv_scene_separate_desc* d, cv_scene_separate_result* r, void* stream) {
    CV_REQUIRE(d && r, CV_EINVAL, "null scene descriptor / result");
    std::memset(r, 0, sizeof(*r));
    const int K = d->num_models;
    CV_REQUIRE(K >= 1 && K <= CV_MAX_CATEGORIES, CV_EINVAL, "num_models out of range (%d, 1..%d)", K, CV_MAX_CATEGORIES);
    CV_REQUIRE(d->d_coords4 && d->d_feats && d->d_points && d->n > 0 && d->ops && d->n_ops && d->bufs && d->n_bufs && d->d_out_feats,
               CV_EINVAL, "bad scene descriptor");
    for (int k = 0; k < K; ++k)
        CV_REQUIRE(d->ops[k] && d->bufs[k] && d->n_ops[k] > 0 && d->n_bufs[k] > 0 && d->d_out_feats[k], CV_EINVAL,
                   "bad program or output buffer of model %d", k);
    CV_REQUIRE(d->out_ld >= d->out_channels && d->out_channels >= 8, CV_EINVAL, "bad network output buffer");
    CV_REQUIRE(d->h_pinned && d->pinned_bytes >= 64 + 64 * (size_t)K && d->d_ws, CV_EINVAL,
               "pinned scratch (>= 64 + 64 K bytes) and a device workspace are required");
    CV_REQUIRE(d->h_boxes && d->h_scores && d->h_cand_idx && d->h_verdict && d->h_det_cat && d->h_det_box && d->max_candidates > 0,
               CV_EINVAL, "null result arrays");
    CV_REQUIRE(!!d->d_xyz_in == !!d->d_scale_in && !!d->d_xyz_in == !!d->d_prob_in, CV_EINVAL, "predictions: all three or none");
    CV_REQUIRE(d->conv_split_target >= 0 && d->vote_part_records >= 0, CV_EINVAL, "negative launch sizing");
    CV_REQUIRE(d->vote_algo >= 0 && d->vote_algo <= 2, CV_EINVAL, "vote_algo out of range (%d: 0 auto, 1 direct, 2 tiles)", d->vote_algo);
    CV_REQUIRE(d->models_per_pass >= 0, CV_EINVAL, "negative models_per_pass (%d)", d->models_per_pass);
    const int G = std::min(d->models_per_pass, K);
    if (G > 0) {
        CV_REQUIRE(d->d_model_params, CV_EINVAL, "models_per_pass needs d_model_params (cv_net_models_params_fill)");
        for (int k = 1; k < K; ++k)
            CV_REQUIRE(d->n_ops[k] == d->n_ops[0] && d->n_bufs[k] == d->n_bufs[0], CV_EINVAL,
                       "models_per_pass: the program of model %d has another length than model 0's", k);
    }
    hipStream_t st = static_cast<hipStream_t>(stream);
    const long long n = d->n;
    SceneCount in_flight(false, d->conv_split_target, d->vote_part_records);
    Carver cv(d->d_ws, d->ws_bytes);
    StageClock clock{d->events, st, r->host_us};
    CV_HIP_CHECK(clock.mark(0));

    SceneFront f(d);
    int32_t* h_flags = reinterpret_cast<int32_t*>(static_cast<char*>(d->h_pinned) + 64);
    const bool plan_fits = f.carve(cv);
    float* xyz = cv.take<float>((size_t)K * n * 3);
    float* scale = cv.take<float>((size_t)K * n * 3);
    float* prob = cv.take<float>((size_t)K * n);
    int32_t* d_flags = cv.take<int32_t>(16 * (size_t)K);
    if (!plan_fits || !xyz || !scale || !prob || !d_flags) return fixed_part_too_small(r, cv.off);
    if (d->use_range_flag) CV_HIP_CHECK(hipMemsetAsync(d_flags, 0, sizeof(int32_t) * 16 * K, st));
    int rc = f.run(nullptr, r, clock, stream);
    if (rc != CV_OK) return rc;
    const size_t cells = f.cells;

    size_t arena_b = 0;
    for (int k = 0; k < K; ++k) arena_b = std::max(arena_b, cv_net_arena_bytes(d->bufs[k], d->n_bufs[k], f.rows, 5));
    const size_t vote_ws_b = cv_hv_forward_cat_workspace_bytes(n, d->num_rots, f.dims, d->vote_algo, K);
    const size_t dec_ws_b = cv_decode_cat_workspace_bytes(f.dims, n, d->max_candidates, K);
    const size_t arena_all = G > 0 ? (size_t)G * arena_b : arena_b;
    const size_t conv_ws_all = G > 0 ? cv_net_models_workspace_bytes(f.conv_ws_b, G) : f.conv_ws_b;
    char* arena = cv.take<char>(arena_all);
    char* conv_ws = cv.take<char>(conv_ws_all);
    char* vote_ws = cv.take<char>(std::max<size_t>(vote_ws_b, 256));
    char* dec_ws = cv.take<char>(dec_ws_b);
    float* grids = cv.take<float>(6 * cells * (size_t)K);
    r->needed_ws_bytes = cv.off + 4096;
    CV_REQUIRE(arena && conv_ws && vote_ws && dec_ws && grids, CV_ENOMEM, "scene workspace too small (needs %zu bytes)", r->needed_ws_bytes);
    float* g_obj = grids;
    float* g_rot = grids + cells * K;
    float* g_scale = grids + 3 * cells * K;
    r->d_grid_obj = g_obj; r->d_grid_rot = g_rot; r->d_grid_scale = g_scale;

    for (int m0 = 0; G > 0 && m0 < K; m0 += G) {
        const int g = std::min(G, K - m0);
        const void* ext_ptr[CV_MAX_CATEGORIES][2];
        const void* const* ext_tab[CV_MAX_CATEGORIES];
        for (int m = 0; m < g; ++m) {
            ext_ptr[m][0] = d->d_feats, ext_ptr[m][1] = d->d_out_feats[m0 + m];
            ext_tab[m] = ext_ptr[m];
        }
        const int ext_ld[2] = {d->feats_ld, d->out_ld};
        rc = cv_net_run_models_ex(d->ops + m0, d->bufs + m0, d->n_ops[0], d->n_bufs[0], g, f.rows, 5, arena, arena_all, ext_tab, ext_ld,
                                  f.maps, CV_NET_MAP_SLOTS, f.perms, CV_NET_PERM_SLOTS, conv_ws, conv_ws_all,
                                  d->use_range_flag ? d_flags + 16 * m0 : nullptr,
                                  static_cast<const cv_net_model_params*>(d->d_model_params) + m0, K,  true, stream);
        if (rc != CV_OK) return rc;
    }
    for (int k = 0; G == 0 && k < K; ++k) {
        const void* ext_ptr[2] = {d->d_feats, d->d_out_feats[k]};
        const int ext_ld[2] = {d->feats_ld, d->out_ld};
        rc = cv_net_run_ex(d->ops[k], d->n_ops[k], d->bufs[k], d->n_bufs[k], f.rows, 5, arena, arena_b, ext_ptr, ext_ld, f.maps,
                           CV_NET_MAP_SLOTS, f.perms, CV_NET_PERM_SLOTS, conv_ws, f.conv_ws_b,
                           d->use_range_flag ? d_flags + 16 * k : nullptr,  true, stream);
        if (rc != CV_OK) return rc;
    }
    clock.lap(1);
    CV_HIP_CHECK(clock.mark(1));
    if (G > 0) {
        rc = cv_head_separate_models_f32(d->d_out_feats, K, n, d->out_ld, d->log_scale, xyz, scale, prob, stream);
        if (rc != CV_OK) return rc;
    }
    for (int k = 0; G == 0 && k < K; ++k) {
        rc = cv_head_separate_f32(d->d_out_feats[k], n, d->out_ld, d->log_scale, xyz + (size_t)k * n * 3, scale + (size_t)k * n * 3,
                                  prob + (size_t)k * n, stream);
        if (rc != CV_OK) return rc;
    }
    if (d->use_range_flag) CV_HIP_CHECK(hipMemcpyAsync(h_flags, d_flags, sizeof(int32_t) * 16 * K, hipMemcpyDeviceToHost, st));
    r->d_xyz = xyz; r->d_scale = scale; r->d_prob = prob;
    CV_HIP_CHECK(clock.mark(2));

    const float* v_xyz = d->d_xyz_in ? d->d_xyz_in : xyz;
    const float* v_scale = d->d_xyz_in ? d->d_scale_in : scale;
    const float* v_prob = d->d_xyz_in ? d->d_prob_in : prob;
    rc = cv_hv_forward_cat_f32(d->d_points, v_xyz, v_scale, v_prob, n, d->res, d->num_rots, f.mn, f.dims, K, g_obj, g_rot, g_scale, vote_ws,
                               std::max<size_t>(vote_ws_b, 256), d->vote_algo, stream);
    if (rc != CV_OK) return rc;
    CV_HIP_CHECK(clock.mark(3));
    clock.lap(2);
    cv_decode_params prm = d->decode;
    prm.max_iters = d->max_candidates;
    const int M = d->max_candidates;
    std::vector<int32_t> classes((size_t)K * M);
    const DecodeCall dc{g_obj, g_rot, g_scale, f.dims, f.mn, d->res, d->d_points, v_xyz, v_prob, nullptr, n, &prm, 0, dec_ws, dec_ws_b,
                        r->n_cand, d->h_cand_idx, d->h_verdict, r->n_boxes, d->h_boxes, d->h_scores, classes.data(), r->truncated, stream,
                        d->events[4]};
    rc = cv_decode_run(dc, K, false);
    if (rc != CV_OK) return rc;
    if (d->use_range_flag)
        for (int k = 0; k < K; ++k) r->range_flag |= h_flags[16 * k] ? (1 << k) : 0;

    int n_det = 0;
    std::vector<int32_t> pick((size_t)M);
    for (int k = 0; k < K; ++k) {
        const int nb = r->n_boxes[k];
        if (nb == 0) continue;
        const int kept = cv_nms_obb(d->h_boxes + (size_t)k * M * 24, d->h_scores + (size_t)k * M, nb, d->nms_threshold, pick.data());
        if (kept < 0) return kept;
        for (int j = 0; j < kept; ++j) { d->h_det_cat[n_det] = k; d->h_det_box[n_det] = pick[(size_t)j]; ++n_det; }
    }
    r->n_det = n_det;
    clock.lap(3);
    return CV_OK;
}

}

namespace {

int check_points_front(const cv_points_front& f, bool joint) {
    CV_REQUIRE(f.d_raw_points && f.d_raw_feats && f.d_coords4 && f.d_index, CV_EINVAL, "raw cloud: null pointer argument");
    CV_REQUIRE(f.m > 0 && f.m <= (1ll << 29), CV_EINVAL, "raw cloud: bad point count %lld", f.m);
    CV_REQUIRE(f.points_ld >= 3, CV_EINVAL, "raw cloud: bad row stride %lld", f.points_ld);
    CV_REQUIRE(f.quantization_size > 0 && f.quantization_size <= 3.0e38 && (float)f.quantization_size > 0.0f, CV_EINVAL,
               "raw cloud: quantization_size must be positive and finite (got %g)", f.quantization_size);
    CV_REQUIRE(f.in_channels > 0 && f.in_channels <= f.raw_feats_ld, CV_EINVAL, "raw cloud: bad feature width %d (row stride %lld)",
               f.in_channels, f.raw_feats_ld);
    CV_REQUIRE(f.recentre_from <= f.in_channels, CV_EINVAL, "raw cloud: recentre_from %d beyond the feature width %d", f.recentre_from,
               f.in_channels);
    const int given = !!f.d_raw_xyz + !!f.d_raw_scale + !!f.d_raw_prob + (joint ? !!f.d_raw_class : 0);
    CV_REQUIRE(given == 0 || given == (joint ? 4 : 3), CV_EINVAL, "raw cloud: predictions: all %d arrays or none", joint ? 4 : 3);
    CV_REQUIRE(joint || !f.d_raw_class, CV_EINVAL, "raw cloud: separate mode takes no class array");
    return CV_OK;
}

template <class PD, class PR, class Inner>
int detect_points(const PD* pd, PR* r, int K, int32_t** d_class_view, Inner inner, void* stream) {
    const bool joint = d_class_view != nullptr;
    const auto t0 = std::chrono::steady_clock::now();
    const cv_points_front& f = pd->front;
    auto sd = pd->scene;
    hipStream_t st = static_cast<hipStream_t>(stream);
    const long long m = f.m;
    const int C = f.in_channels;
    const bool pred = f.d_raw_xyz != nullptr;
    const float res = (float)f.quantization_size;

// ... 120 lines not shown
```

canonicalvoting_amd/csrc/sparse_conv.hip:

```cpp
#include "cv_common.h"

#include <atomic>
#include <cstring>
#include <type_traits>
#include <utility>

#include "sparse_conv_common.h"

using namespace cvsc;

namespace {

template <int CIN, class... MA>
__global__ __launch_bounds__(THREADS, (CIN <= 3 ? 3 : 1)) void conv_stem_mfma(ConvArgs a, MA... ma) {
    model_enter_y(a, ma...);
    constexpr int G = 8;
    constexpr int W_BYTES = G * CIN * 2 * 1024;
    constexpr int EP_BYTES = 4 * 32 * EP_LD * 4;
    constexpr int SM_BYTES = W_BYTES > EP_BYTES ? W_BYTES : EP_BYTES;
    __shared__ __attribute__((aligned(16))) unsigned char w_s[SM_BYTES];
    __shared__ int rows_s[TM];
    const int tid = threadIdx.x, lane = tid & 63, wave = tid >> 6;
    const int half = lane >> 5, l31 = lane & 31;
    const long long r0 = (long long)blockIdx.x * TM;
// ... 117 lines not shown

template <int SMAX, class IDX, class... MA>
__global__ __launch_bounds__(256) void conv_finish_small(ConvArgs a, FinishMasks<SMAX> gm, MA... ma) {
    model_enter_y(a, ma...);
    const IDX cq = (IDX)(a.cout >> 2);
    const IDX total4 = (IDX)a.n_out * cq;
    const IDX e4 = (IDX)blockIdx.x * (IDX)256 + (IDX)threadIdx.x;
    if (e4 >= total4) return;
    const IDX row = e4 / cq;
    const int col = (int)(e4 - row * cq) * 4;
    const unsigned w = a.gvalid ? (unsigned)a.gvalid[row] : ~0u;
    const float4* p = reinterpret_cast<const float4*>(a.partial) + e4;
    float4 pv[SMAX];
#pragma unroll
    for (int k = 0; k < SMAX; ++k)
        pv[k] = (w & gm.m[k]) ? partial_load4(p + (long long)k * (long long)total4) : make_float4(0.f, 0.f, 0.f, 0.f);
    float4 sq[4];
#pragma unroll
    for (int q = 0; q < 4; ++q) sq[q] = make_float4(0.f, 0.f, 0.f, 0.f);
#pragma unroll
    for (int k = 0; k < SMAX; ++k)
        if (k < a.splits) { sq[k & 3].x += pv[k].x; sq[k & 3].y += pv[k].y; sq[k & 3].z += pv[k].z; sq[k & 3].w += pv[k].w; }
    const float4 x = make_float4(sq[0].x + sq[1].x + sq[2].x + sq[3].x, sq[0].y + sq[1].y + sq[2].y + sq[3].y,
                                 sq[0].z + sq[1].z + sq[2].z + sq[3].z, sq[0].w + sq[1].w + sq[2].w + sq[3].w);
    epilogue_apply4(a, (long long)row, col, x);
}

template <class... MA>
__global__ __launch_bounds__(256) void conv_finish_scalar(ConvArgs a, MA... ma) {
    model_enter_y(a, ma...);
    const long long total = a.n_out * (long long)a.cout;
    for (long long t = blockIdx.x * 256ll + threadIdx.x; t < total; t += (long long)gridDim.x * 256) {
        const long long row = t / a.cout;
        const int col = (int)(t - row * a.cout);
        float v = 0.f;
        for (int sidx = 0; sidx < a.splits; ++sidx) v += a.partial[sidx * total + t];
        epilogue_apply1(a, row, col, v);
    }
}

template <int SMAX, class IDX>
void launch_finish_small(const ConvArgs& a, hipStream_t st, const ModelArgs* ma, int models) {
    FinishMasks<SMAX> gm;
    for (int k = 0; k < SMAX; ++k) {
        gm.m[k] = k < a.splits ? ~0u : 0u;
        if (a.gvalid && k < a.splits) {
            const int jb = a.K * k / a.splits, je = a.K * (k + 1) / a.splits;
            gm.m[k] = (unsigned)(((1ull << je) - 1) & ~((1ull << jb) - 1));
        }
    }
    const long long items = a.n_out * (long long)a.cout / 4;
    const dim3 grid((unsigned)((items + 255) / 256), (unsigned)models);
    with_models(ma, [&](auto... m) { conv_finish_small<SMAX, IDX, decltype(m)...><<<grid, 256, 0, st>>>(a, gm, m...); });
}

std::atomic<int> g_ablation{0};
int launch_finish(const ConvArgs& a, hipStream_t st, const ModelArgs* ma, int models) {
    if (g_ablation.load(std::memory_order_relaxed) & 1) return CV_OK;
    const long long total = a.n_out * (long long)a.cout;
    const auto grid = [&](long long items, int per_block, long long cap) {
        return dim3((unsigned)std::min<long long>((items + per_block - 1) / per_block, cap), (unsigned)models);
    };
    if (a.wide && a.splits <= FINISH_SMALL_MAX) {
        const auto with_idx = [&](auto smax) {
            if (total < (1ll << 31)) launch_finish_small<smax.value, unsigned>(a, st, ma, models);
            else launch_finish_small<smax.value, long long>(a, st, ma, models);
        };
        if (a.splits <= 4) with_idx(std::integral_constant<int, 4>{});
        else if (a.splits <= 8) with_idx(std::integral_constant<int, 8>{});
        else with_idx(std::integral_constant<int, FINISH_SMALL_MAX>{});
    } else if (a.cout % 4 == 0)
        with_models(ma, [&](auto... m) { conv_finish<decltype(m)...><<<grid(total / 4, 64, 8192), 256, 0, st>>>(a, m...); });
    else
        with_models(ma, [&](auto... m) { conv_finish_scalar<decltype(m)...><<<grid(total, 256, 4096), 256, 0, st>>>(a, m...); });
    CV_LAUNCH_CHECK();
    return CV_OK;
}

std::atomic<long long> g_opt_zskip{getenv("CV_ZSKIP") ? atoll(getenv("CV_ZSKIP")) : 1};
std::atomic<long long> g_zskip_launches{0};
std::atomic<long long> g_opt_hd_mask{getenv("CV_HD") ? atoll(getenv("CV_HD")) : 4};
std::atomic<long long> g_opt_hd_min_rows{getenv("CV_HD_MIN_ROWS") ? atoll(getenv("CV_HD_MIN_ROWS")) : 16384};
std::atomic<long long> g_opt_hd_shape{getenv("CV_HD_SHAPE") ? atoll(getenv("CV_HD_SHAPE")) : 2};

int launch_rows(ConvArgs a, const int NB, bool vec, hipStream_t st, ModelArgs* ma, int models) {
    dim3 grid((unsigned)((a.n_out + TM - 1) / TM), (unsigned)((a.cout + NB * 32 - 1) / (NB * 32)),
              (unsigned)a.splits);
    int per_wg = 0;
    if (vec) {
        const int nj_wp = a.j_end - a.j_begin, nch_wp = a.cin / KC;
        for (int z = 0; z < a.splits; ++z) {
            long long lo, hi;
            if (a.perm_per_split) {
                lo = (long long)nj_wp * z / a.splits * nch_wp;
                hi = (long long)nj_wp * (z + 1) / a.splits * nch_wp;
            } else {
                lo = (long long)nj_wp * nch_wp * z / a.splits;
                hi = (long long)nj_wp * nch_wp * (z + 1) / a.splits;
            }
            if (hi > lo) per_wg = std::max(per_wg, (int)((hi - 1) / nch_wp - lo / nch_wp + 1));
        }
    }
    if (ma) {
        CV_REQUIRE(a.in_hl && !a.tickets, CV_EINVAL,
                   "the model axis runs fp16-pair programs on hl buffers only (no fp32 / bf16 convolution, no split_tickets)");
        ma->ncb = (int)grid.y;
        grid.y *= (unsigned)models;
    }
    if (a.in_hl) {
        CV_REQUIRE(per_wg * (a.cin / KC) + (a.in2 ? a.cin2 / KC : 0) <= HL_MAX_UNITS, CV_EINVAL,
                   "hl-format convolution: more than %d units per workgroup (Cin too wide)", HL_MAX_UNITS);
        CV_REQUIRE(vec && a.wp6 && a.pieces == 2 && a.wide && per_wg <= WP_NPRE && NB <= 4, CV_EINVAL,
                   "hl-format input needs the fp16-pair weights, Cin %% 32 == 0, 16-byte aligned operands and at most %d "
                   "kernel offsets per workgroup", WP_NPRE);
        const int hd_mask = (int)g_opt_hd_mask.load(std::memory_order_relaxed);
        const long long hd_min_rows = g_opt_hd_min_rows.load(std::memory_order_relaxed);
        const int hd_shape = (int)g_opt_hd_shape.load(std::memory_order_relaxed);
        const bool hd = NB <= 3 && ((hd_mask >> (NB - 1)) & 1) && a.n_out >= hd_min_rows;
        if (hd || !(a.splits > 1 && !a.perm_per_split && (long long)grid.x * grid.y <= CV_SPLIT_TICKETS)) a.tickets = nullptr;
        if (hd) {
            const int nw = hd_shape == 1 ? 4 : 8;
            launch_conv_hd(a, NB, hd_shape, ma, dim3((unsigned)((a.n_out + nw * 32 - 1) / (nw * 32)), grid.y, grid.z), st);
        } else {
            launch_conv_hl(a, NB, ma, grid, st);
        }
    } else if (vec && a.wp6 && per_wg <= WP_NPRE) {
        launch_conv_rows_wp(a, NB, a.pieces, false, grid, st);
    } else if (vec && a.wp6 && per_wg <= WP_NPRE_BIG) {
        launch_conv_rows_wp(a, NB, a.pieces, true, grid, st);
    } else {
        CV_REQUIRE(a.pieces != 1 || !(vec && a.wp6), CV_EINVAL, "the bf16 compute mode takes at most %d kernel offsets per workgroup", WP_NPRE_BIG);
        CV_REQUIRE(!a.in2, CV_EINVAL,
                   "a second source takes at most %d kernel offsets per workgroup (%d here: flavour 0 with a workspace splits the "
                   "launch, or pass fewer offsets per call)", WP_NPRE_BIG, per_wg);
        launch_conv_rows(a, NB, vec, grid, st);
    }
    CV_LAUNCH_CHECK();
    return a.splits > 1 && !a.tickets ? launch_finish(a, st, ma, models) : CV_OK;
}

int nb_for(int cout) {
    static const int nb_max = getenv("CV_NB_MAX") ? atoi(getenv("CV_NB_MAX")) : 0;
    if (nb_max > 0) return std::min(nb_max, nb_full(cout));
    if (cout <= 32) return 1;
    if (cout <= 64) return 2;
    if (cout <= 96) return 3;
    static const int nb_wide = getenv("CV_NB_WIDE") ? atoi(getenv("CV_NB_WIDE")) : 2;
    return std::max(1, std::min(nb_wide, 2));
}

std::atomic<long long> g_split_target{-1};
thread_local long long t_split_target = 0;
long long process_split_target() {
    long long v = g_split_target.load(std::memory_order_relaxed);
    if (v <= 0) {
        v = getenv("CV_SPLIT_TARGET") ? std::max(1ll, atoll(getenv("CV_SPLIT_TARGET"))) : 768;
        g_split_target.store(v, std::memory_order_relaxed);
    }
    return v;
}
long long split_target() { return t_split_target > 0 ? t_split_target : process_split_target(); }

int pick_splits(long long n_out, int cout, int K, int cin, bool vec) {
    const int nb = nb_for(cout);
    const long long tiles = ((n_out + TM - 1) / TM) * ((cout + nb * 32 - 1) / (nb * 32));
    const long long units = vec ? (long long)K * (cin / KC) : ((long long)K * cin + KC - 1) / KC;
    if (tiles >= 384 || units <= 1) return 1;
    const long long target = split_target();
    long long s = (target + tiles - 1) / tiles;
    s = std::min(s, units);
    static const long long traffic_mb = getenv("CV_SPLIT_TRAFFIC_MB") ? atoll(getenv("CV_SPLIT_TRAFFIC_MB")) : 24;
    const long long by_traffic = (traffic_mb << 20) / std::max<long long>(1, n_out * cout * 4);
    s = std::min(s, std::max<long long>(by_traffic, 2));
    s = std::min<long long>(s, 64);
    return (int)std::max<long long>(s, 1);
}

}

static std::atomic<long long>* option_named(const char* name) {
    return !strcmp(name, "hd_mask") ? &g_opt_hd_mask : !strcmp(name, "hd_min_rows") ? &g_opt_hd_min_rows :
           !strcmp(name, "hd_shape") ? &g_opt_hd_shape : !strcmp(name, "zskip") ? &g_opt_zskip :
           !strcmp(name, "zskip_launches") ? &g_zskip_launches : nullptr;
}

int cv_sp_set_option(const char* name, long long value, long long* previous) {
    CV_REQUIRE(name, CV_EINVAL, "null option name");
    std::atomic<long long>* o = option_named(name);
    CV_REQUIRE(o, CV_EINVAL, "unknown option '%s' (hd_mask, hd_min_rows, hd_shape, zskip, zskip_launches)", name);
    const long long before = o->exchange(value, std::memory_order_relaxed);
    if (previous) *previous = before;
    return CV_OK;
}

int cv_sp_get_option(const char* name, long long* value) {
    CV_REQUIRE(name && value, CV_EINVAL, "null option name / value");
    const std::atomic<long long>* o = option_named(name);
    CV_REQUIRE(o, CV_EINVAL, "unknown option '%s'", name);
    *value = o->load(std::memory_order_relaxed);
    return CV_OK;
}

int cv_sp_set_ablation(int bits) { return g_ablation.exchange(bits, std::memory_order_relaxed); }

int cv_sp_set_split_target_thread(int workgroups) {
    const int before = (int)t_split_target;
    t_split_target = workgroups > 0 ? workgroups : 0;
    return before;
}

int cv_sp_set_split_target(int workgroups) {
    const int before = (int)process_split_target();
    g_split_target.store(workgroups > 0 ? workgroups : -1, std::memory_order_relaxed);
    return before;
}

static int conv_dispatch(const cv_conv_desc* d, const CvConvModels* mm, void* stream);

extern "C" {

size_t cv_sp_conv_workspace_bytes(long long n_out, int cout, int K) {
    if (n_out <= 0 || cout <= 0 || K <= 0) return 0;
    const size_t one = sizeof(float) * (size_t)n_out * (size_t)cout;
    return 256 + std::min<size_t>(64 * one, std::max<size_t>((size_t)48 << 20, 3 * one));
}

int cv_sp_conv_f32(const cv_conv_desc* d, void* stream) { return conv_dispatch(d, nullptr, stream); }

}

int cv_sp_conv_models_f32(const cv_conv_desc* d, const CvConvModels* mm, void* stream) {
    CV_REQUIRE(d && mm && mm->d_params && mm->models >= 1 && mm->models <= CV_MAX_CATEGORIES, CV_EINVAL, "bad model-axis arguments");
    CV_REQUIRE(!d->split_tickets, CV_EINVAL, "the model axis does not take split_tickets");
    CV_REQUIRE(d->weight_pieces == 2 && !d->acc_in && !d->acc_scale_dev, CV_EINVAL,
               "the model axis runs fp16-pair programs only (weight_pieces == 2; no bf16 triples, no fp32 convolution)");
    CV_REQUIRE(((mm->in_stride | mm->in2_stride | mm->res_stride | mm->out_stride | mm->ws_stride) & 127) == 0, CV_EINVAL,
               "model strides must keep rows 128-byte aligned");
    return conv_dispatch(d, mm, stream);
}

static int conv_dispatch(const cv_conv_desc* d, const CvConvModels* mm, void* stream) {
    CV_REQUIRE(d, CV_EINVAL, "null descriptor");
    CV_REQUIRE(d->in && d->weight && d->out, CV_EINVAL, "null pointer argument");
    CV_REQUIRE(d->n_in > 0 && d->n_out > 0 && d->cin > 0 && d->cout > 0 && d->K > 0, CV_EINVAL, "bad conv sizes");
    CV_REQUIRE(d->nbr || (d->K == 1 && d->n_in == d->n_out), CV_EINVAL, "a kernel map is required unless K == 1");
    CV_REQUIRE(d->in_ld >= d->cin && d->out_ld >= d->cout && (!d->residual || d->res_ld >= d->cout) &&
                   (!d->acc_in || d->acc_ld >= d->cout), CV_EINVAL, "bad leading dimension");
    CV_REQUIRE(d->out != d->in, CV_EINVAL, "conv cannot run in place");
    const int jb = d->j_begin, je = d->j_end > 0 ? d->j_end : d->K;
    CV_REQUIRE(jb >= 0 && jb < je && je <= d->K, CV_EINVAL, "bad kernel offset range");
    hipStream_t st = static_cast<hipStream_t>(stream);
    ConvArgs a = {};
    a.in = d->in, a.n_in = d->n_in, a.in_ld = d->in_ld, a.cin = d->cin;
    a.w = d->weight, a.K = d->K, a.cout = d->cout;
    a.nbr = d->nbr, a.n_out = d->n_out;
    a.scale = d->scale, a.shift = d->shift;
    a.res = d->residual, a.res_ld = d->res_ld;
    a.relu = d->relu;
    a.out = d->out, a.out_ld = d->out_ld;
    a.splits = 1;
    a.row_perm = d->row_perm;
    a.j_begin = jb, a.j_end = je;
    a.acc_in = d->acc_in, a.acc_ld = d->acc_ld;
    a.wp6 = static_cast<const unsigned short*>(d->weight_x6);
    a.in2 = d->in2, a.in2_ld = d->in2_ld, a.cin2 = d->cin2;
    a.wp6_2 = static_cast<const unsigned short*>(d->weight2_x6);
    a.pieces = d->weight_pieces == 2 ? 2 : d->weight_pieces == 1 ? 1 : 3;
    a.acc_scale = d->acc_scale != 0.f ? d->acc_scale : 1.f;
    a.range_flag = d->range_flag;
    a.in_hl = d->in_hl, a.out_hl = d->out_hl, a.res_hl = d->res_hl;
    a.tickets = d->in_hl ? d->split_tickets : nullptr;
    if (d->in_hl || d->out_hl || d->res_hl) {
        CV_REQUIRE(!d->in_hl || (d->weight_pieces == 2 && d->cin % 32 == 0 && d->in_ld % 32 == 0 &&
                                 (reinterpret_cast<uintptr_t>(d->in) & 127) == 0 &&
                                 (!d->in2 || (d->cin2 % 32 == 0 && d->in2_ld % 32 == 0 &&
                                              (reinterpret_cast<uintptr_t>(d->in2) & 127) == 0))),
                   CV_EINVAL, "hl-format input: fp16-pair weights, channels and leading dimensions %% 32 == 0, 128-byte aligned rows");
        CV_REQUIRE(!d->out_hl || (d->cout % 32 == 0 && d->out_ld % 32 == 0 && (reinterpret_cast<uintptr_t>(d->out) & 127) == 0),
                   CV_EINVAL, "hl-format output: Cout and leading dimension %% 32 == 0, 128-byte aligned rows");
        CV_REQUIRE(!d->res_hl || !d->residual || (d->res_ld % 32 == 0 && (reinterpret_cast<uintptr_t>(d->residual) & 127) == 0),
                   CV_EINVAL, "hl-format residual: leading dimension %% 32 == 0, 128-byte aligned rows");
        CV_REQUIRE(d->flavour == 0, CV_EINVAL, "the hl format runs with flavour 0 only");
        CV_REQUIRE(!d->in_hl || ((unsigned long long)d->n_in * (unsigned long long)d->in_ld * 4ull + (unsigned long long)d->cin * 4ull < (1ull << 32) &&
                                 (!d->in2 || (unsigned long long)d->n_out * (unsigned long long)d->in2_ld * 4ull + (unsigned long long)d->cin2 * 4ull < (1ull << 32))),
                   CV_EINVAL, "hl-format input larger than 4 GiB (rows x leading dimension x 4): split the batch");
    }
    CV_REQUIRE(d->weight_pieces >= 0 && d->weight_pieces <= 3, CV_EINVAL,
               "weight_pieces is 0/3 (bf16 triples), 2 (fp16 pairs) or 1 (single bf16 product)");
    CV_REQUIRE(d->weight_pieces != 1 || (d->weight_x6 && d->cin % KC == 0), CV_EINVAL,
               "weight_pieces = 1 needs weight_x6 from cv_sp_pack_weights_bf16_f32 and Cin %% 32 == 0");
    const bool stem_h2 = d->weight_pieces == 2 && d->weight_x6 && d->cout == 32 && (d->cin == 3 || d->cin == 6) && d->K <= 128;
    CV_REQUIRE(d->weight_pieces != 2 || stem_h2 || (d->weight_x6 && d->cin % KC == 0), CV_EINVAL,
               "weight_pieces = 2 needs weight_x6 from cv_sp_pack_weights_h2_f32 and Cin %% 32 == 0 (or the stem shape with "
               "cv_sp_pack_weights_stem_h2_f32)");

    ModelArgs ma = {};
    if (mm) {
        ma.params = mm->d_params;
        ma.in_stride = mm->in_stride, ma.in2_stride = mm->in2_stride, ma.res_stride = mm->res_stride, ma.out_stride = mm->out_stride;
        ma.partial_stride = mm->ws_stride;
        ma.out_ext = mm->out_ext;
        for (int m = 0; m < mm->models; ++m) ma.ext_out[m] = mm->ext_out[m];
    }
    ModelArgs* const pma = mm ? &ma : nullptr;
    const int models = mm ? mm->models : 1;
    CV_REQUIRE(!d->plan_ent && !d->plan_cnt && !d->weight_packed && (d->flavour == 0 || d->flavour == 1), CV_EINVAL,
               "flavours 3 / 4 (the experimental wave / tile kernels of rounds 1-3) are gone: flavour is 0 or 1, plan_ent / plan_cnt / "
// ... 67 lines not shown
```

canonicalvoting_amd/me/__init__.py:

```python
import ctypes
import math
import os
import threading
import weakref

import numpy as np
import torch
import torch.nn as nn

from .. import _lib
from .._lib import ptr as _ptr, stream as _stream, vp
from . import utils

__version__ = "0.5.3-cvhip"


class _NoSwitch:
    def __enter__(self):
        return self

    def __exit__(self, *exc):
        return False


_NO_SWITCH = _NoSwitch()


def _on(dev):
    if dev.index is None or torch.cuda.current_device() == dev.index:
        return _NO_SWITCH
    return torch.cuda.device(dev)


class _FusedPlan:
    __slots__ = ("keep", "counts", "cap", "stem_k", "groups", "off", "layout", "map_ptrs", "perm_ptrs", "views")


class CoordinateManager:

    NUM_LEVELS = 5

    def __init__(self, coords, num_levels=NUM_LEVELS, check=True, lazy=False):
        assert coords.is_cuda and coords.dtype == torch.int32 and coords.dim() == 2 and coords.shape[1] == 4
        self.device = coords.device
        if coords.shape[0] == 0:
            raise RuntimeError("SparseTensor: empty coordinate set")
        self.cap = int(_lib.lib().cv_sp_table_capacity(coords.shape[0]))
        self._input = coords.contiguous()
        self._fused = None
        self._lazy = (num_levels, check) if lazy else None
        if not lazy:
            self._build(num_levels, check)

    def __getattr__(self, name):
        if name in ("coords", "counts", "_level", "_keys", "_vals", "_coords_buf", "_counts_d", "_verified", "_maps",
                    "num_levels") and self.__dict__.get("_lazy") is not None:
            lazy, self._lazy = self._lazy, None
            self._build(*lazy)
            return self.__dict__[name]
        raise AttributeError(name)

    @classmethod
    def _from_levels(cls, coords_buf, keys, vals, counts_d, counts, cap):
        self = object.__new__(cls)
        self.device = coords_buf[0].device
        self.cap = cap
        self._input = coords_buf[0]
        self._fused = None
        self._lazy = None
        self.num_levels = len(coords_buf)
        self._coords_buf, self._keys, self._vals, self._counts_d = coords_buf, keys, vals, counts_d
        self._verified = True
        self.counts = counts
        self.coords = {1 << i: coords_buf[i][:counts[i]] for i in range(self.num_levels)}
        self._level = {1 << i: i for i in range(self.num_levels)}
        self._maps = {}
        return self

    def _build(self, num_levels, check):
        L = _lib.lib()
        dev = self.device
        n = self._input.shape[0]
        self.num_levels = num_levels
        self._coords_buf = [self._input] + [torch.empty((n, 4), dtype=torch.int32, device=dev)
                                            for _ in range(num_levels - 1)]
        self._keys = [torch.empty(self.cap, dtype=torch.int64, device=dev) for _ in range(num_levels)]
        self._vals = [torch.empty(self.cap, dtype=torch.int32, device=dev) for _ in range(num_levels)]
        self._counts_d = torch.empty(8, dtype=torch.int32, device=dev)
        counts_h = (ctypes.c_int32 * 8)()
        ws = torch.empty(int(L.cv_sp_levels_workspace_bytes(n)), dtype=torch.uint8, device=dev)
        arr = lambda ts: (ctypes.c_void_p * len(ts))(*[t.data_ptr() for t in ts])
        sync = check or num_levels > 1
        with _on(dev):
            _lib.check(L.cv_sp_build_levels(arr(self._coords_buf), arr(self._keys), arr(self._vals), n,
                                            self.cap, num_levels, _ptr(self._counts_d),
                                            counts_h if sync else None, _ptr(ws), ws.numel(), _stream(dev)),
                       "cv_sp_build_levels")
        self._verified = sync
        if sync:
            self._raise_on_dups(counts_h[5], counts_h[6])
            self.counts = [int(counts_h[i]) for i in range(num_levels)]
        else:
            self.counts = [n]
        self.coords = {1 << i: self._coords_buf[i][:self.counts[i]] for i in range(num_levels)}
        self._level = {1 << i: i for i in range(num_levels)}
        self._maps = {}

    @staticmethod
    def _raise_on_dups(count, out_of_range=0):
        if out_of_range != 0:
            raise RuntimeError("SparseTensor: %d coordinates outside the supported window (spatial coordinates in "
                               "[-32704, 32703], batch index < 65536)" % out_of_range)
        if count != 0:
            raise RuntimeError("SparseTensor: %d duplicate coordinates (quantise with "
                               "utils.sparse_quantize first, as utils/dataloader.py:197 does)" % count)

    def _verify(self):
        if not self._verified:
            c = self._counts_d[5:7].tolist()
            self._raise_on_dups(int(c[0]), int(c[1]))
            self._verified = True

    def ensure_levels(self, num_levels=NUM_LEVELS):
        if self.num_levels < num_levels:
            self._build(num_levels, True)

    def mask_perms(self, k, ts, groups=2):
        key = ("mp", k, ts, groups)
        m = self._maps.get(key)
        if m is None:
            L = _lib.lib()
            nbr = self.kernel_map(k, ts)
            n, K = nbr.shape
            if (K + groups - 1) // groups <= 10:
                m = _perms_with_map(nbr, groups)
            else:
                m = torch.empty((groups, n), dtype=torch.int32, device=self.device)
                keys = torch.empty(n, dtype=torch.int64, device=self.device)
                for g in range(groups):
                    jb, je = K * g // groups, K * (g + 1) // groups
                    with torch.cuda.device(self.device):
                        _lib.check(L.cv_sp_mask_keys(_ptr(nbr), n, K, jb, je, _ptr(keys), _stream(self.device)),
                                   "cv_sp_mask_keys")
                    m[g] = torch.argsort(keys).to(torch.int32)
            self._maps[key] = m
        return m

    def up_perm(self, ts_coarse):
        key = ("upperm", ts_coarse)
        m = self._maps.get(key)
        if m is None:
            L = _lib.lib()
            up = self.up_map(ts_coarse)
            m = torch.empty((1, up.shape[0]), dtype=torch.int32, device=self.device)
            ws = torch.empty(4096, dtype=torch.uint8, device=self.device)
            with torch.cuda.device(self.device):
                _lib.check(L.cv_sp_mask_perms(_ptr(up), up.shape[0], 8, 1, _ptr(m), _ptr(ws), ws.numel(), 0,
                                              _stream(self.device)), "cv_sp_mask_perms")
            m = m[0]
            self._maps[key] = m
        return m

    MASK_GROUPS = int(os.environ.get("CV_NET_MASK_GROUPS", "3"))
    MASKED_MIN_ROWS = int(os.environ.get("CV_MASKED_MIN_ROWS", "16384"))
    LIB_MASKED_MIN_ROWS = MASKED_MIN_ROWS

    @classmethod
    def plan_mask_groups(cls):
        return cls.MASK_GROUPS if (27 + cls.MASK_GROUPS - 1) // cls.MASK_GROUPS <= 10 else 0

    def fused_fast(self, stem_k=5):
        cache = self.__dict__.setdefault("_fused_cache", {})
        mmr = masked_min_rows()
        if (stem_k, mmr) in cache:
            return cache[(stem_k, mmr)]
        L = _lib.lib()
        dev = self.device
        n = self._input.shape[0]
        NL = CoordinateManager.NUM_LEVELS
        G = self.plan_mask_groups()
        lay = _lib.ScenePlanLayout()
        _lib.check(L.cv_sp_scene_plan_layout(n, stem_k, G, mmr, ctypes.byref(lay)), "cv_sp_scene_plan_layout")
        ibuf = torch.empty(lay.int_words, dtype=torch.int32, device=dev)
        kbuf = torch.empty(lay.key_words, dtype=torch.int64, device=dev)
        sws_b, lws_b = lay.sort_ws_bytes, lay.levels_ws_bytes
        o_lws = (sws_b + 63) & ~63
        wbuf = _lib.scratch(dev, "scene_plan", o_lws + lws_b)
        ib, kb, wb = ibuf.data_ptr(), kbuf.data_ptr(), wbuf.data_ptr()
        c_coords = (vp * NL)(*[ib + 4 * o for o in lay.coords])
        c_keys = (vp * NL)(*[kb + 8 * lay.cap * i for i in range(NL)])
        c_vals = (vp * NL)(*[ib + 4 * o for o in lay.vals])
        counts_h = (ctypes.c_int32 * 8)()
        off = _lib.SceneMaps()
        with _on(dev):
            _lib.check(L.cv_sp_scene_plan(_ptr(self._input), n, vp(ib + 4 * lay.perm), vp(ib + 4 * lay.inv), c_coords, c_keys,
                                          c_vals, lay.cap, vp(ib + 4 * lay.counts), counts_h, stem_k, G, mmr,
                                          vp(ib + 4 * lay.arena), lay.int_words - lay.arena, ctypes.byref(off), vp(wb), sws_b,
                                          vp(wb + o_lws), lws_b, _stream(dev)), "cv_sp_scene_plan")
        self._raise_on_dups(counts_h[5], counts_h[6])
        plan = _FusedPlan()
        plan.keep = (ibuf, kbuf)
        plan.counts = [int(counts_h[i]) for i in range(NL)]
        plan.cap, plan.stem_k, plan.groups, plan.off, plan.layout = lay.cap, stem_k, G, off, lay
        maps, perms = (vp * _lib.NET_MAP_SLOTS)(), (vp * _lib.NET_PERM_SLOTS)()
        _lib.check(L.cv_sp_scene_plan_slots(ctypes.byref(lay), ctypes.byref(off), (ctypes.c_int64 * NL)(*plan.counts), 0, vp(ib),
                                            maps, perms), "cv_sp_scene_plan_slots")
        plan.map_ptrs, plan.perm_ptrs = list(maps), list(perms)
        plan.views = None
        cache[(stem_k, mmr)] = plan
        self._fused = plan
        return plan

    def fused_plan(self, stem_k=5):
        plan = self.fused_fast(stem_k)
        if plan.views is None:
            ibuf, kbuf = plan.keep
            n, cap, G, off = self._input.shape[0], plan.cap, plan.groups, plan.off
            lay, o_inv, o_counts, o_arena = plan.layout, plan.layout.inv, plan.layout.counts, plan.layout.arena
            c = plan.counts
            NL = len(c)
            coords_buf = [ibuf[o:o + 4 * n].view(n, 4) for o in lay.coords]
            keys = [kbuf[i * cap:(i + 1) * cap] for i in range(NL)]
            vals = [ibuf[o:o + cap] for o in lay.vals]
            cm_s = CoordinateManager._from_levels(coords_buf, keys, vals, ibuf[o_counts:o_counts + 8], c, cap)
            arena = ibuf[o_arena:]
            view = lambda o, r, k: arena[o:o + r * k].view(r, k)
            stem_map = view(off.stem, c[0], stem_k ** 3)
            out_map = ibuf[o_inv:o_inv + n].view(n, 1)
            for i in range(4):
                cm_s._maps[("k", 2, 1 << i, 2)] = view(off.down[i], c[i + 1], 8)
                cm_s._maps[("up", 16 >> i)] = view(off.up[i], c[3 - i], 8)
                cm_s._maps[("upperm", 16 >> i)] = arena[off.up_perm[i]:off.up_perm[i] + c[3 - i]]
            for i in range(5):
                cm_s._maps[("k", 3, 1 << i, 1)] = view(off.k3[i], c[i], 27)
                if i == 0 or off.mask_perm[i] >= 0:
                    cm_s._maps[("k", 3, 1 << i, 1)]._cv_valid_words = arena[off.k3[i] + 27 * c[i]:off.k3[i] + 28 * c[i]]
                if off.mask_perm[i] >= 0:
                    mp = view(off.mask_perm[i], G, c[i])
                    mp._cv_has_map = True
                    mp._cv_from_plan = True
                    cm_s._maps[("mp", 3, 1 << i, G)] = mp
                    cm_s._maps[("k", 3, 1 << i, 1)]._cv_mask_perms = mp
            plan.views = (cm_s, stem_map, out_map)
        return plan.views

    def num_rows(self, ts):
        if ts == 1:
            return self._input.shape[0]
        if ts not in self._level:
            self.ensure_levels()
        return self.counts[self._level[ts]]

    def kernel_map(self, k, ts_in, stride=1):
        if ts_in * stride not in self._level:
            self.ensure_levels()
        self._verify()
        key = ("k", k, ts_in, stride)
        m = self._maps.get(key)
        if m is None:
            L = _lib.lib()
            li = self._level[ts_in]
            out = self.coords[ts_in * stride]
            m = torch.empty((out.shape[0], k ** 3), dtype=torch.int32, device=self.device)
            with torch.cuda.device(self.device):
                _lib.check(L.cv_sp_kernel_map(_ptr(out), out.shape[0], _ptr(self._keys[li]),
                                              _ptr(self._vals[li]), self.cap, k, ts_in, _ptr(m),
                                              _stream(self.device)), "cv_sp_kernel_map")
            self._maps[key] = m
        return m

    def up_map(self, ts_coarse):
        key = ("up", ts_coarse)
        m = self._maps.get(key)
        if m is None:
            L = _lib.lib()
            down = self.kernel_map(2, ts_coarse // 2, 2)
            n_fine = self.num_rows(ts_coarse // 2)
            m = torch.empty((n_fine, 8), dtype=torch.int32, device=self.device)
            with torch.cuda.device(self.device):
                _lib.check(L.cv_sp_up_map(_ptr(down), down.shape[0], n_fine, _ptr(m), _stream(self.device)),
                           "cv_sp_up_map")
            self._maps[key] = m
        return m


class SparseTensor:

    def __init__(self, features, coordinates=None, device=None, coordinate_manager=None, tensor_stride=1,
                 **_):
        if device is None:
            device = features.device if coordinates is None else (
                features.device if features.is_cuda else torch.device("cuda"))
        device = torch.device(device)
        if device.type != "cuda":
            raise RuntimeError("canonicalvoting_amd SparseTensor runs on the GPU only (no CPU engine); "
                               "pass device='cuda'")
        self.F = features.to(device=device, dtype=torch.float32)
        self.F_hl = None
        if coordinate_manager is None:
            if coordinates is None:
                raise ValueError("coordinates or coordinate_manager required")
            c = coordinates
            if c.is_floating_point():
                c = torch.floor(c)
            coordinate_manager = CoordinateManager(c.to(device=device, dtype=torch.int32).contiguous(),
                                                   num_levels=1, check=False, lazy=True)
        self.coordinate_manager = coordinate_manager
        self.tensor_stride = tensor_stride if isinstance(tensor_stride, int) else int(tensor_stride[0])
        if self.F.shape[0] != coordinate_manager.num_rows(self.tensor_stride):
            raise RuntimeError("features have %d rows, coordinate set has %d" % (
                self.F.shape[0], coordinate_manager.num_rows(self.tensor_stride)))

    @property
    def C(self):
        cm = self.coordinate_manager
        if self.tensor_stride not in cm.coords:
            cm.ensure_levels()
        return cm.coords[self.tensor_stride]

    @property
    def coordinates(self):
        return self.C

    @property
# ... 930 lines not shown
```

canonicalvoting_amd/minkunet.py:

```python
import ctypes
import os

import torch
import torch.nn as nn

from . import _lib
from . import me as ME
from ._lib import ptr, stream, vp
from .me.modules.resnet_block import BasicBlock


class ResNetBase(nn.Module):
    BLOCK = None
    LAYERS = ()
    INIT_DIM = 64
    PLANES = (64, 128, 256, 512)

    def __init__(self, in_channels, out_channels, D=3):
        nn.Module.__init__(self)
        self.D = D
        assert self.BLOCK is not None
        self.network_initialization(in_channels, out_channels, D)
        self.weight_initialization()

# ... 34 lines not shown
    OUT_TENSOR_STRIDE = 1

    def network_initialization(self, in_channels, out_channels, D):
        exp = self.BLOCK.expansion
        self.inplanes = self.INIT_DIM
        self.conv0p1s1 = ME.MinkowskiConvolution(in_channels, self.inplanes, kernel_size=5, dimension=D)
        self.bn0 = ME.MinkowskiBatchNorm(self.inplanes)
        for i, (cname, bname) in enumerate(_DOWN):
            setattr(self, cname, ME.MinkowskiConvolution(self.inplanes, self.inplanes, kernel_size=2,
                                                         stride=2, dimension=D))
            setattr(self, bname, ME.MinkowskiBatchNorm(self.inplanes))
            setattr(self, "block%d" % (i + 1), self._make_layer(self.BLOCK, self.PLANES[i], self.LAYERS[i]))
        skip = (self.PLANES[2] * exp, self.PLANES[1] * exp, self.PLANES[0] * exp, self.INIT_DIM)
        for i, (cname, bname) in enumerate(_UP):
            setattr(self, cname, ME.MinkowskiConvolutionTranspose(self.inplanes, self.PLANES[4 + i],
                                                                  kernel_size=2, stride=2, dimension=D))
            setattr(self, bname, ME.MinkowskiBatchNorm(self.PLANES[4 + i]))
            self.inplanes = self.PLANES[4 + i] + skip[i]
            setattr(self, "block%d" % (5 + i),
                    self._make_layer(self.BLOCK, self.PLANES[4 + i], self.LAYERS[4 + i]))
        self.final = ME.MinkowskiConvolution(self.PLANES[7] * exp, out_channels, kernel_size=1, bias=True,
                                             dimension=D)
        self.relu = ME.MinkowskiReLU(inplace=True)

    def train(self, mode=True):
        self.__dict__.pop("_fold_cache", None)
        self.__dict__.pop("_prog", None)
        ME.invalidate_weight_caches()
        return super().train(mode)

    def forward(self, x, defer_check=None):
        if (not self.training) and (not torch.is_grad_enabled()) and self.BLOCK is BasicBlock:
            return self.program_forward(x, defer_check=defer_check) if self.USE_PROGRAM else self.fused_forward(x)
        with ME.batched_counter_updates():
            return self.modular_forward(x)

    SORTED_TRAINING = os.environ.get("CV_TRAIN_SORTED", "1") != "0"

    def modular_forward(self, x):
        if self.SORTED_TRAINING and x.tensor_stride == 1 and type(self.conv0p1s1) is ME.MinkowskiConvolution:
            cm_s, stem_map, out_map = x.coordinate_manager.fused_plan(self.conv0p1s1.kernel_size)
            n = x.F.shape[0]
            f0 = ME._ConvFn.apply(x.F, self.conv0p1s1.kernel, self.conv0p1s1.bias, stem_map, n)
            out = self._modular_body(ME.SparseTensor(f0, coordinate_manager=cm_s, tensor_stride=1))
            k = self.final.kernel
            y = ME._ConvFn.apply(out.F, k, self.final.bias, out_map, n)
            return x._like(y, 1)
        return self.final(self._modular_body(self.conv0p1s1(x)))

    def _modular_body(self, stem_out):
        out_p1 = self.bn0.forward_fused(stem_out, relu=True)
        skips = [out_p1]
        out = out_p1
        for i, (cname, bname) in enumerate(_DOWN):
            out = getattr(self, bname).forward_fused(getattr(self, cname)(out), relu=True)
            out = getattr(self, "block%d" % (i + 1))(out)
            skips.append(out)
        skips.pop()
        for i, (cname, bname) in enumerate(_UP):
            out = getattr(self, bname).forward_fused(getattr(self, cname)(out), relu=True)
            out = ME.cat(out, skips.pop())
            out = getattr(self, "block%d" % (5 + i))(out)
        return out

    def _fold(self, bn_module):
        bn = bn_module.bn
        ver = (bn.weight._version, bn.bias._version, bn.running_mean._version, bn.running_var._version,
               bn.weight.data_ptr())
        cache = self.__dict__.setdefault("_fold_cache", {})
        hit = cache.get(id(bn))
        if hit is None or hit[0] != ver:
            hit = (ver, ME.bn_affine(bn))
            cache[id(bn)] = hit
        return hit[1]

    MASKED_MIN_ROWS = None

    def masked_min_rows(self):
        v = getattr(ME._policy_tls, "masked_min_rows", None)
        if v is not None:
            return v
        return self.MASKED_MIN_ROWS if self.MASKED_MIN_ROWS is not None else ME.CoordinateManager.MASKED_MIN_ROWS
    MASK_GROUPS = ME.CoordinateManager.MASK_GROUPS
    USE_PROGRAM = os.environ.get("CV_NET_PROGRAM", "1") != "0"
    FUSE_DOWNSAMPLE = os.environ.get("CV_FUSE_DOWNSAMPLE", "1") != "0"
    PIECES = 2 if os.environ.get("CV_CONV_H2", "1") != "0" else 3
    HL_BUFFERS = os.environ.get("CV_NET_HL", "1") != "0"
    STEM_MFMA = os.environ.get("CV_STEM_MFMA", "1") != "0"
    defer_range_check = False

    def _conv3(self, x, kernel, nbr, perms, n, **ep):
        if perms is not None:
            return ME.conv_forward_masked(x, kernel, nbr, perms, n, **ep)
        return ME.conv_forward(x, kernel, nbr, n, **ep)

    def _run_layer(self, layer, x, nbr, n, out_view, perms=None):
        for bi, blk in enumerate(layer):
            s1, b1 = self._fold(blk.norm1)
            t = self._conv3(x, blk.conv1.kernel, nbr, perms, n, scale=s1, shift=b1, relu=True)
            if blk.downsample is not None:
                sd, bd = self._fold(blk.downsample[1])
                res = ME.conv_forward(x, blk.downsample[0].kernel, None, n, scale=sd, shift=bd)
            else:
                res = x
            s2, b2 = self._fold(blk.norm2)
            last = bi == len(layer) - 1
            x = self._conv3(t, blk.conv2.kernel, nbr, perms, n, scale=s2, shift=b2, residual=res, relu=True,
                            out=out_view if (last and out_view is not None) else None)
        return x

    def fused_forward(self, x):
        cm, stem_map, out_map = x.coordinate_manager.fused_plan(self.conv0p1s1.kernel_size)
        dev = x.F.device
        exp = self.BLOCK.expansion
        n = [cm.num_rows(1 << i) for i in range(5)]
        perms = lambda ts, rows: cm.mask_perms(3, ts, self.MASK_GROUPS) if rows >= self.masked_min_rows() else None
        up_c = [self.PLANES[4 + i] for i in range(4)]
        skip_c = (self.PLANES[2] * exp, self.PLANES[1] * exp, self.PLANES[0] * exp, self.INIT_DIM)
        cat = [torch.empty((n[3 - i], up_c[i] + skip_c[i]), dtype=torch.float32, device=dev) for i in range(4)]
        skip_view = [cat[i][:, up_c[i]:] for i in range(4)]
        s, b = self._fold(self.bn0)
        out = ME.conv_forward(x.F.contiguous(), self.conv0p1s1.kernel, stem_map, n[0], scale=s,
                              shift=b, relu=True, out=skip_view[3])
        for i, (cname, bname) in enumerate(_DOWN):
            ts = 1 << i
            s, b = self._fold(getattr(self, bname))
            out = ME.conv_forward(out, getattr(self, cname).kernel, cm.kernel_map(2, ts, 2), n[i + 1],
                                  scale=s, shift=b, relu=True)
            out = self._run_layer(getattr(self, "block%d" % (i + 1)), out, cm.kernel_map(3, 2 * ts), n[i + 1],
                                  skip_view[2 - i] if i < 3 else None, perms(2 * ts, n[i + 1]))
        for i, (cname, bname) in enumerate(_UP):
            ts_coarse = 16 >> i
            lvl = 3 - i
            s, b = self._fold(getattr(self, bname))
            ME.conv_forward(out, getattr(self, cname).kernel, cm.up_map(ts_coarse), n[lvl], scale=s, shift=b,
                            relu=True, out=cat[i][:, :up_c[i]], row_perm=cm.up_perm(ts_coarse))
            out = self._run_layer(getattr(self, "block%d" % (5 + i)), cat[i], cm.kernel_map(3, ts_coarse // 2),
                                  n[lvl], None, perms(ts_coarse // 2, n[lvl]))
        y = ME.conv_forward(out, self.final.kernel, out_map, n[0], shift=self.final.bias.reshape(-1))
        return x._like(y, 1)


    MAP_STEM, MAP_DOWN, MAP_K3, MAP_UP, MAP_OUT = 0, 1, 5, 10, 14
    PERM_K3, PERM_UP = 0, 5

    def _program(self, dev, pieces=3):
        progs = self.__dict__.setdefault("_prog", {})
        hit = progs.get(pieces)
        if hit is not None:
            tensors, ver = hit[0]
            if ver == (sum(t._version for t in tensors), tensors[0].data_ptr(), str(dev), self.training):
                return hit[1]
        tensors = list(self.parameters()) + list(self.buffers())
        ver = ((tensors, (sum(t._version for t in tensors), tensors[0].data_ptr(), str(dev), self.training)))
        exp = self.BLOCK.expansion
        bufs, ops, keep, free = [], [], [], {}
        hl = 1 if (pieces == 2 and self.HL_BUFFERS and ME.CONV_X6) else 0

        def alloc(level, ch):
            pool = free.get((level, ch))
            if pool:
                return pool.pop()
            bufs.append((level, ch, level, hl))
            return len(bufs) - 1

        def release(slot):
            level, ch = bufs[slot][:2]
            if level >= 0:
                free.setdefault((level, ch), []).append(slot)

        def conv(src, dst, kernel, K, map_slot, scale=None, shift=None, res=None, relu=False, perm=-1, groups=0,
                 second=None):
            w = (kernel if kernel.dim() == 3 else kernel[None]).detach().contiguous()
            in2, cin2 = (-1, 0), 0
            if second is not None:
                in2, kernel2, scale2 = second
                w2 = (kernel2 if kernel2.dim() == 3 else kernel2[None]).detach().contiguous()
                cin2, second = w2.shape[1], (w2, scale2)
            w6, w6_2, op_pieces, acc_scale, folded = ME.resolve_weights(kernel, w, pieces, stem=bool(hl) and self.STEM_MFMA,
                                                                        col_scale=scale, second=second, cache=True)
            if folded:
                scale = None
            keep.extend([w, scale, shift, w6, w6_2])
            ops.append(dict(in_buf=src[0], in_col=src[1], cin=w.shape[1], out_buf=dst[0], out_col=dst[1],
                            cout=w.shape[2], res_buf=res[0] if res else -1, res_col=res[1] if res else 0,
                            map=map_slot, K=K, perm=perm, perm_groups=groups, relu=1 if relu else 0,
                            weight=w.data_ptr(), scale=scale.data_ptr() if scale is not None else None,
                            shift=shift.data_ptr() if shift is not None else None,
                            weight_x6=w6.data_ptr() if w6 is not None else None,
                            in2_buf=in2[0], in2_col=in2[1], cin2=cin2,
                            weight2_x6=w6_2.data_ptr() if w6_2 is not None else None,
                            weight_pieces=op_pieces, acc_scale=acc_scale))

        def layer(seq, x, level, out_view):
            for bi, blk in enumerate(seq):
                planes = blk.conv1.out_channels
                s1, b1 = self._fold(blk.norm1)
                t = (alloc(level, planes), 0)
                k3 = dict(K=27, map_slot=self.MAP_K3 + level, perm=self.PERM_K3 + level, groups=self.MASK_GROUPS)
                conv(x, t, blk.conv1.kernel, scale=s1, shift=b1, relu=True, **k3)
                s2, b2 = self._fold(blk.norm2)
                last = bi == len(seq) - 1
                y = out_view if (last and out_view is not None) else (alloc(level, planes), 0)
                fuse_ds = (blk.downsample is not None and self.FUSE_DOWNSAMPLE and ME.CONV_X6 and
                           blk.conv1.in_channels % 32 == 0 and planes % 32 == 0)
                if fuse_ds:
                    sd, bd = self._fold(blk.downsample[1])
                    shift = (b2 + bd).contiguous()
                    conv(t, y, blk.conv2.kernel, scale=s2, shift=shift, relu=True,
                         second=(x, blk.downsample[0].kernel, sd), **k3)
                    res = x
                else:
                    if blk.downsample is not None:
                        sd, bd = self._fold(blk.downsample[1])
                        res = (alloc(level, planes), 0)
                        conv(x, res, blk.downsample[0].kernel, 1, -1, scale=sd, shift=bd)
                    else:
                        res = x
                    conv(t, y, blk.conv2.kernel, scale=s2, shift=b2, res=res, relu=True, **k3)
                release(t[0])
                if res is not x:
                    release(res[0])
                if x[1] == 0 and bufs[x[0]][1] == (blk.conv1.in_channels):
                    release(x[0])
                x = y
            return x

        bufs.append((-1, self.conv0p1s1.in_channels, 0, 0))
        bufs.append((-1, self.final.out_channels, 0, 0))
        up_c = [self.PLANES[4 + i] for i in range(4)]
        skip_c = (self.PLANES[2] * exp, self.PLANES[1] * exp, self.PLANES[0] * exp, self.INIT_DIM)
        cat = []
        for i in range(4):
            bufs.append((3 - i, up_c[i] + skip_c[i], 3 - i, hl))
            cat.append(len(bufs) - 1)
        s, b = self._fold(self.bn0)
        out = (cat[3], up_c[3])
        conv((0, 0), out, self.conv0p1s1.kernel, self.conv0p1s1.kernel.shape[0], self.MAP_STEM, scale=s, shift=b,
             relu=True)
        for i, (cname, bname) in enumerate(_DOWN):
            s, b = self._fold(getattr(self, bname))
            c = getattr(self, cname)
            d = (alloc(i + 1, c.out_channels), 0)
            conv(out, d, c.kernel, 8, self.MAP_DOWN + i, scale=s, shift=b, relu=True)
            out = layer(getattr(self, "block%d" % (i + 1)), d, i + 1, (cat[2 - i], up_c[2 - i]) if i < 3 else None)
        for i, (cname, bname) in enumerate(_UP):
            lvl = 3 - i
            s, b = self._fold(getattr(self, bname))
            conv(out, (cat[i], 0), getattr(self, cname).kernel, 8, self.MAP_UP + i, scale=s, shift=b, relu=True,
                 perm=self.PERM_UP + i)
            if bufs[out[0]][0] >= 0 and out[1] == 0 and out[0] not in cat:
                release(out[0])
            out = layer(getattr(self, "block%d" % (5 + i)), (cat[i], 0), lvl, None)
        bias = self.final.bias.detach().reshape(-1).contiguous()
        conv(out, (1, 0), self.final.kernel, 1, self.MAP_OUT, shift=bias)
        c_ops = (_lib.NetOp * len(ops))(*[_lib.NetOp(**o) for o in ops])
        c_bufs = (_lib.NetBuf * len(bufs))(*[_lib.NetBuf(*bf) for bf in bufs])
        prog = (c_ops, c_bufs, keep)
        progs[pieces] = (ver, prog)
        return prog

    def check_range(self, x, y):
        flag = ME.range_flag(x.F.device)
        if int(flag[0]) == 0:
            return y
        flag.zero_()
        self.range_fallbacks = getattr(self, "range_fallbacks", 0) + 1
        return self.program_forward(x, pieces=3)

    def eval_pieces(self):
        return 1 if ME.COMPUTE_DTYPE == "bf16" else self.PIECES

    def launch_args(self, plan, level_orders=None, max_planes=None):
        masked = [c >= self.masked_min_rows() for c in plan.counts[:5]]
        orders = plan.perm_ptrs[:5] if level_orders is None else level_orders
        if any(m and o is None for m, o in zip(masked, orders)):
            return None
        perm_ptrs = [o if m else None for m, o in zip(masked, orders)] + plan.perm_ptrs[5:]
        rows = (ctypes.c_int64 * 5)(*plan.counts)
        sorted_levels = (ctypes.c_int * 5)(*[p is not None for p in perm_ptrs[:5]])
        ws_bytes = _lib.lib().cv_sp_scene_conv_workspace_bytes(rows, sorted_levels, self.MASK_GROUPS,
                                                               max_planes or max(self.PLANES))
        return rows, ws_bytes, (vp * len(plan.map_ptrs))(*plan.map_ptrs), (vp * len(perm_ptrs))(*perm_ptrs)

    def program_forward(self, x, pieces=None, defer_check=None):
        L = _lib.lib()
        dev = x.F.device
        if pieces is None:
            pieces = self.eval_pieces()
        c_ops, c_bufs, _ = self._program(dev, pieces)
        plan = x.coordinate_manager.fused_fast(self.conv0p1s1.kernel_size)
        flag = ME.range_flag(dev) if pieces == 2 else None
        n = plan.counts
        args = self.launch_args(plan)
        if args is None:
            cm = x.coordinate_manager.fused_plan(self.conv0p1s1.kernel_size)[0]
            wide = [cm.mask_perms(3, 1 << i, self.MASK_GROUPS) if n[i] >= self.masked_min_rows() else None for i in range(5)]
            args = self.launch_args(plan, [w.data_ptr() if w is not None else None for w in wide])
        rows, ws_bytes, c_maps, c_perms = args
        feats = x.F.contiguous()
        y = torch.empty((n[0], self.final.out_channels), dtype=torch.float32, device=dev)
        arena = _lib.scratch(dev, "net_arena", L.cv_net_arena_bytes(c_bufs, len(c_bufs), rows, 5))
        ws = ME._workspace(dev, ws_bytes)
        ext_ptr = (vp * 2)(feats.data_ptr(), y.data_ptr())
        ext_ld = (ctypes.c_int * 2)(feats.stride(0), y.stride(0))
        with torch.cuda.device(dev):
            _lib.check(L.cv_net_run_f32(c_ops, len(c_ops), c_bufs, len(c_bufs), rows, 5, ptr(arena), arena.numel(), ext_ptr,
                                        ext_ld, c_maps, len(c_maps), c_perms, len(c_perms), ptr(ws), ws.numel(),
                                        ptr(flag), stream(dev)), "cv_net_run_f32")
        out = x._like(y, 1)
        if flag is not None and not (self.defer_range_check if defer_check is None else defer_check):
            torch.cuda.current_stream(dev).synchronize()
            out = self.check_range(x, out)
        return out

    def forward_flops(self, x):
        cm = x.coordinate_manager.fused_plan()[0]
        n = [cm.num_rows(1 << i) for i in range(5)]
        pairs = lambda m: int((m >= 0).sum().item())
        p5, p3 = pairs(x.coordinate_manager.fused_plan()[1]), {1 << i: pairs(cm.kernel_map(3, 1 << i)) for i in range(5)}
        pd = {1 << i: pairs(cm.kernel_map(2, 1 << i, 2)) for i in range(4)}
        sparse = dense = 0

        def add(p, full, cin, cout):
            nonlocal sparse, dense
            sparse += 2 * p * cin * cout
            dense += 2 * full * cin * cout

        def layer(seq, ts, lvl):
            for blk in seq:
                cin, cout = blk.conv1.in_channels, blk.conv1.out_channels
                add(p3[ts], n[lvl] * 27, cin, cout)
                add(p3[ts], n[lvl] * 27, cout, cout)
                if blk.downsample is not None:
                    add(n[lvl], n[lvl], cin, cout)

        add(p5, n[0] * 125, self.conv0p1s1.in_channels, self.conv0p1s1.out_channels)
        for i, (cname, _) in enumerate(_DOWN):
            c = getattr(self, cname)
            add(pd[1 << i], n[i + 1] * 8, c.in_channels, c.out_channels)
            layer(getattr(self, "block%d" % (i + 1)), 2 << i, i + 1)
        for i, (cname, _) in enumerate(_UP):
            c = getattr(self, cname)
            lvl = 3 - i
            add(n[lvl], n[lvl], c.in_channels, c.out_channels)
            layer(getattr(self, "block%d" % (5 + i)), 8 >> i, lvl)
        add(n[0], n[0], self.final.in_channels, self.final.out_channels)
        return sparse, dense


class MinkUNet14(MinkUNetBase):
    BLOCK = BasicBlock
    LAYERS = (1, 1, 1, 1, 1, 1, 1, 1)


class MinkUNet18(MinkUNetBase):
    BLOCK = BasicBlock
    LAYERS = (2, 2, 2, 2, 2, 2, 2, 2)


class MinkUNet34(MinkUNetBase):
    BLOCK = BasicBlock
    LAYERS = (2, 3, 4, 6, 2, 2, 2, 2)


class MinkUNet14A(MinkUNet14):
    PLANES = (32, 64, 128, 256, 128, 128, 96, 96)


class MinkUNet18A(MinkUNet18):
    PLANES = (32, 64, 128, 256, 128, 128, 96, 96)


class MinkUNet18B(MinkUNet18):
    PLANES = (32, 64, 128, 256, 128, 128, 128, 128)


class MinkUNet18D(MinkUNet18):
    PLANES = (32, 64, 128, 256, 384, 384, 384, 384)

# ... 34 lines not shown
```

canonicalvoting_amd/pipeline.py:

```python
import collections
import contextlib
import ctypes
import threading

import numpy as np
import torch

from . import _lib, decode, hv_cuda
from . import me as ME
from ._lib import ptr, stream, vp

SCRATCH_FLOOR = 64 << 20


class ScenePolicy(collections.namedtuple("ScenePolicy", "conv_split_target vote_part_records masked_min_rows")):
    __slots__ = ()

    def as_config(self):
        return {"conv_split_target": self.conv_split_target, "vote_part_records": self.vote_part_records,
                "masked_min_rows": self.masked_min_rows}


def policy_for_scenes_in_flight(n):
    lib_rows = ME.CoordinateManager.LIB_MASKED_MIN_ROWS
# ... 327 lines not shown
    y = torch.empty((coords4.shape[0], model.final.out_channels), dtype=torch.float32, device=dev)
    host = _host(dev, max_candidates)
    _fill_scene_desc(d.scene, model, hv, None, None, None, res, policy, pieces, max(model.PLANES), log_scale)
    _fill_joint_desc(d.scene, host, program, y, nclasses, decode_kw, adaptive_split, events, keep)
    ws = _call_points(_lib.lib().cv_detect_points_f32, "cv_detect_points_f32", d, r, dev, "scene_call", host.ws_hint)
    del alive
    n = int(r.n)
    coords4, index, y = coords4[:n], index[:n], y[:n]
    tail = (index, inverse) if return_inverse else (index,)
    view = lambda p, shape, dt=torch.float32: _device_view(p, shape, dt, dev, ws)
    gathered = lambda: dict(scan_points=view(r.d_points, (n, 3)), feats=view(r.d_feats, (n, d.front.in_channels)),
                            host_us=tuple(r.scene.host_us), host_us_front=float(r.host_us_front),
                            front_ws_bytes=int(r.front_ws_bytes))
    out = _finish_joint(host, r.scene, keep, y, n, dev, ws, gathered)
    if out is not None:
        return out + tail
    pred = None
    if predictions is not None:
        pred = (view(r.d_xyz_in, (n, 3)), view(r.d_scale_in, (n, 3)), view(r.d_prob_in, (n,)), view(r.d_class_in, (n,), torch.int32))
    return detect_scene_c(model, hv, coords4, view(r.d_feats, (n, d.front.in_channels)), res, nclasses=nclasses,
                          log_scale=log_scale, predictions=pred, max_candidates=max_candidates, keep=keep, events=events,
                          adaptive_split=adaptive_split, policy=policy, **decode_kw) + tail



def model_params_table(mods, dev, pieces):
    progs = [m._program(dev, pieces) for m in mods]
    key = (str(dev), pieces, tuple(id(m) for m in mods))
    with _scene_lock:
        hit = _model_tables.get(key)
    if hit is not None and len(hit[0]) == len(progs) and all(a is b for a, b in zip(hit[0], progs)):
        return progs, hit[1]
    L = _lib.lib()
    K, n_ops = len(progs), len(progs[0][0])
    if any(len(p[0]) != n_ops for p in progs):
        raise ValueError("model_params_table: the models' programs differ in length")
    nbytes = L.cv_net_models_params_bytes(n_ops, K)
    host = np.zeros(nbytes, np.uint8)
    ops = (vp * K)(*[ctypes.cast(p[0], vp) for p in progs])
    _lib.check(L.cv_net_models_params_fill(ops, n_ops, K, vp(host.ctypes.data), nbytes), "cv_net_models_params_fill")
    table = torch.from_numpy(host).to(dev)
    with _scene_lock:
        _model_tables[key] = (progs, table)
    return progs, table


def _model_set(who, mods, dev, models_per_pass, scene_call=True):
    K = len(mods)
    if scene_call and not 1 <= K <= _lib.MAX_CATEGORIES:
        raise ValueError("%s: 1..%d models (got %d)" % (who, _lib.MAX_CATEGORIES, K))
    pieces = mods[0].eval_pieces()
    G = int(models_per_pass or 0)
    if scene_call and G < 0:
        raise ValueError("%s: models_per_pass must be >= 0 (got %d)" % (who, G))
    if not scene_call:
        G = min(G, K) if G else K
    if G > 0 or not scene_call:
        return (K, pieces, G) + model_params_table(mods, dev, pieces)
    return K, pieces, G, [m._program(dev, pieces) for m in mods], None


def forward_models(mods, x, models_per_pass=None, range_flags=None):
    L = _lib.lib()
    dev = x.F.device
    mods = list(mods)
    K, pieces, G, progs, table = _model_set("forward_models", mods, dev, models_per_pass, scene_call=False)
    m0 = mods[0]
    plan = x.coordinate_manager.fused_fast(m0.conv0p1s1.kernel_size)
    args = m0.launch_args(plan, max_planes=max(max(m.PLANES) for m in mods))
    if args is None:
        raise ValueError("forward_models: the plan has no mask orders for a level that runs mask-sorted")
    rows, ws_one, c_maps, c_perms = args
    feats = x.F.contiguous()
    ys = [torch.empty((plan.counts[0], m.final.out_channels), dtype=torch.float32, device=dev) for m in mods]
    c_bufs0 = progs[0][1]
    arena = _lib.scratch(dev, "net_arena_models", L.cv_net_models_arena_bytes(c_bufs0, len(c_bufs0), rows, 5, G))
    ws = _lib.scratch(dev, "conv_ws_models", L.cv_net_models_workspace_bytes(ws_one, G))
    ext_ld = (ctypes.c_int * 2)(feats.stride(0), ys[0].stride(0))
    n_ops = len(progs[0][0])
    entry = ctypes.sizeof(_lib.NetModelParams)
    with torch.cuda.device(dev):
        for k0 in range(0, K, G):
            g = min(G, K - k0)
            ops = (vp * g)(*[ctypes.cast(p[0], vp) for p in progs[k0:k0 + g]])
            bufs = (vp * g)(*[ctypes.cast(p[1], vp) for p in progs[k0:k0 + g]])
            ext = [(vp * 2)(feats.data_ptr(), y.data_ptr()) for y in ys[k0:k0 + g]]
            c_ext = (vp * g)(*[ctypes.cast(e, vp) for e in ext])
            flag = vp(range_flags.data_ptr() + 64 * k0) if range_flags is not None else None
            _lib.check(L.cv_net_run_models_f32(ops, bufs, n_ops, len(c_bufs0), g, rows, 5, ptr(arena), arena.numel(), c_ext,
                                               ext_ld, c_maps, len(c_maps), c_perms, len(c_perms), ptr(ws), ws.numel(), flag,
                                               vp(table.data_ptr() + entry * k0), K, stream(dev)), "cv_net_run_models_f32")
    return ys


def _fill_separate_desc(d, host, progs, table, G, ys, decode_kw, overlap_threshold, events):
    K = len(progs)
    d.num_models = K
    if G > 0:
        d.models_per_pass, d.d_model_params = G, ptr(table)
    ops = (vp * K)(*[ctypes.cast(p[0], vp) for p in progs])
    n_ops = (ctypes.c_int * K)(*[len(p[0]) for p in progs])
    bufs = (vp * K)(*[ctypes.cast(p[1], vp) for p in progs])
    n_bufs = (ctypes.c_int * K)(*[len(p[1]) for p in progs])
    outs = (vp * K)(*[y.data_ptr() for y in ys])
    d.ops, d.n_ops, d.bufs, d.n_bufs = ctypes.cast(ops, vp), ctypes.cast(n_ops, vp), ctypes.cast(bufs, vp), ctypes.cast(n_bufs, vp)
    d.d_out_feats, d.out_ld, d.out_channels = ctypes.cast(outs, vp), ys[0].stride(0), ys[0].shape[1]
    d.h_det_cat, d.h_det_box = vp(host.det_cat.ctypes.data), vp(host.det_box.ctypes.data)
    _fill_landing(d, host, decode_kw, True, overlap_threshold, events)
    return ops, n_ops, bufs, n_bufs, outs


def _finish_separate(host, r, keep, categories, ys, n, dev, ws, **more_keep):
    K = len(categories)
    host.ws_hint = max(host.ws_hint, int(r.needed_ws_bytes))
    host.last_host_us = tuple(r.host_us)
    if keep is not None:
        keep.update(range_flag=int(r.range_flag), needed_ws_bytes=int(r.needed_ws_bytes), **more_keep)
    if r.range_flag or any(r.truncated[k] for k in range(K)):
        return None
    dets = [(categories[int(c)], host.boxes[int(c), int(b)].copy(), float(host.scores[int(c), int(b)]))
            for c, b in zip(host.det_cat[:r.n_det], host.det_box[:r.n_det])]
    if keep is not None:
        X, Y, Z = r.dims
        view = lambda p, shape: _device_view(p, shape, torch.float32, dev, ws)
        raw = [dict(boxes=host.boxes[k, :r.n_boxes[k]].copy(), scores=host.scores[k, :r.n_boxes[k]].copy(),
                    cand_idx=host.cand[k, :r.n_cand[k]].copy(), verdict=host.verdict[k, :r.n_cand[k]].copy())
               for k in range(K)]
        keep.update(y=ys, dims=(X, Y, Z), corner=tuple(r.corner), level_rows=list(r.level_rows), raw=raw,
                    grids=(view(r.d_grid_obj, (K, X, Y, Z)), view(r.d_grid_rot, (K, X, Y, Z, 2)),
                           view(r.d_grid_scale, (K, X, Y, Z, 3))),
                    net_pred=(view(r.d_xyz, (K, n, 3)), view(r.d_scale, (K, n, 3)), view(r.d_prob, (K, n))),
                    host_us=tuple(r.host_us))
    return dets


def detect_scene_separate_c(models, hv, coords4, feats, res, predictions=None, policy=None, keep=None, events=None,
                            log_scale=True, overlap_threshold=0.3, max_candidates=512, scan_points=None,
                            models_per_pass=None, **decode_kw):
    _separate_defaults(decode_kw)
    dev = feats.device
    n = coords4.shape[0]
    categories, mods = list(models.keys()), list(models.values())
    if scan_points is None:
        scan_points = (coords4[:, 1:].to(dev) * res).float().contiguous()
    K, pieces, G, progs, table = _model_set("detect_scene_separate_c", mods, dev, models_per_pass)
    coords4 = coords4.to(device=dev, dtype=torch.int32).contiguous()
    feats = feats.contiguous()
    ys = [torch.empty((n, m.final.out_channels), dtype=torch.float32, device=dev) for m in mods]
    M = int(max_candidates)
    host = _host(dev, M, K)
    d, r = _lib.SceneSeparateDesc(), _lib.SceneSeparateResult()
    _fill_scene_desc(d, mods[0], hv, coords4, feats, scan_points, res, policy, pieces, max(max(m.PLANES) for m in mods), log_scale)
    if predictions is not None:
        px, ps, pp = [a.contiguous() for a in predictions]
        d.d_xyz_in, d.d_scale_in, d.d_prob_in = ptr(px), ptr(ps), ptr(pp)
    alive = _fill_separate_desc(d, host, progs, table, G, ys, decode_kw, overlap_threshold, events)
    ws = _call_growing(_lib.lib().cv_detect_scene_separate_f32, "cv_detect_scene_separate_f32", d, r, dev,
                       "scene_call_separate", host.ws_hint)
    del alive
    dets = _finish_separate(host, r, keep, categories, ys, n, dev, ws)
    if dets is not None:
        return dets
    kw = dict(decode_kw, max_candidates=M)
    if predictions is None:
        return detect_scene_separate(models, hv, coords4, feats, res, log_scale=log_scale, overlap_threshold=overlap_threshold, **kw)
    return _separate_by_calls(hv, scan_points, zip(*predictions), res, categories, overlap_threshold, **kw)

# ... 33 lines not shown
```

include/cv_hip.h:

```cpp
#ifndef CV_HIP_H
#define CV_HIP_H

#include <stddef.h>
#include <stdint.h>

#ifdef __cplusplus
extern "C" {
#endif

#define CV_OK 0
#define CV_EINVAL (-22)
#define CV_ENOMEM (-12)
#define CV_EHIP (-5)
#define CV_ERANGE (-34)

#define CV_ABI_VERSION 6
int cv_abi_version(void);
const char* cv_last_error(void);


size_t cv_hv_minmax_workspace_bytes(void);
int cv_hv_minmax_f32(const float* d_points, int64_t n, float* h_min3, float* h_max3,
                     void* d_ws, size_t ws_bytes, void* stream);
int cv_hv_minmax_async_f32(const float* d_points, int64_t n, float* h_minmax6, void* d_ws, size_t ws_bytes,
// ... 178 lines not shown
size_t cv_sp_sort_workspace_bytes(long long n);
int cv_sp_sort_rows(const int32_t* d_coords, long long n, int32_t* d_sorted, int32_t* d_perm, int32_t* d_inv,
                    void* d_ws, size_t ws_bytes, void* stream);

int cv_sp_morton_keys(const int32_t* d_coords, long long n, long long* d_keys, void* stream);

int cv_sp_kernel_map(const int32_t* d_out_coords, long long n_out, const unsigned long long* d_keys,
                     const int32_t* d_vals, long long cap, int k, int ts, int32_t* d_nbr, void* stream);

int cv_sp_up_map(const int32_t* d_nbr_down, long long n_coarse, long long n_fine, int32_t* d_up,
                 void* stream);

typedef struct cv_conv_desc {
    const float* in;
    long long n_in;
    int in_ld, cin;
    const float* weight;
    int K, cout;
    const int32_t* nbr;
    long long n_out;
    const float* scale;
    const float* shift;
    const float* residual;
    int res_ld;
    int relu;
    float* out;
    int out_ld;
    int flavour;
    void* ws;
    size_t ws_bytes;
    const int32_t* row_perm;
    int j_begin, j_end;
    const float* acc_in;
    int acc_ld;
    int perm_groups;
    const int32_t* plan_ent;
    const int32_t* plan_cnt;
    const float* weight_packed;
    const void* weight_x6;
    const float* in2;
    int in2_ld, cin2;
    const void* weight2_x6;
    int perm_has_map;
    int weight_pieces;
    float acc_scale;
    int32_t* range_flag;
    int in_hl, out_hl, res_hl;
    int32_t* split_tickets;
    const float* acc_scale_dev;
    const int32_t* valid_words;
} cv_conv_desc;
#define CV_SPLIT_TICKETS 4096

int cv_sp_to_hl_f32(const float* d_x, long long n, int c, int x_ld, float* d_y, int y_ld, int32_t* range_flag, void* stream);
int cv_sp_from_hl_f32(const float* d_x, long long n, int c, int x_ld, float* d_y, int y_ld, void* stream);

int cv_sp_pack_weights_x6_f32(const float* d_w, int K, int cin, int cout, const float* d_col_scale, void* d_wp6,
                              void* stream);
int cv_sp_pack_weights_h2_f32(const float* d_w, int K, int cin, int cout, const float* d_col_scale, int scale_log2,
                              void* d_wp, void* stream);
typedef struct cv_pack_job {
    const float* w;
    void* wp;
    int K, cin, cout;
    int trans;
    int scale_log2;
    int reserved;
} cv_pack_job;
int cv_sp_pack_weights_h2_batch_f32(const cv_pack_job* h_jobs, int n_jobs, void* d_jobs, void* stream);
int cv_sp_pack_weights_bf16_f32(const float* d_w, int K, int cin, int cout, const float* d_col_scale, void* d_wp,
                                void* stream);
int cv_sp_pack_weights_t_f32(const float* d_w, int K, int rows, int cols, int pieces, int scale_log2, void* d_wp, void* stream);
int cv_sp_pack_weights_stem_h2_f32(const float* d_w, int K, int cin, const float* d_col_scale, int scale_log2, void* d_wp,
                                   void* stream);

size_t cv_sp_conv_workspace_bytes(long long n_out, int cout, int K);
int cv_sp_conv_f32(const cv_conv_desc* desc, void* stream);

int cv_sp_set_split_target(int workgroups);
int cv_sp_set_split_target_thread(int workgroups);
int cv_sp_set_ablation(int bits);
int cv_sp_set_option(const char* name, long long value, long long* previous);
int cv_sp_get_option(const char* name, long long* value);

typedef struct cv_scene_maps {
    long long stem, out, down[4], k3[5], up[4], mask_perm[5], up_perm[4], scratch;
    long long bitmap;
} cv_scene_maps;
size_t cv_sp_scene_maps_words(const long long* level_rows, long long n_orig, int stem_k, int mask_groups,
                              long long masked_min_rows, cv_scene_maps* offsets);
int cv_sp_scene_maps(int32_t* const* d_coords, const unsigned long long* const* d_keys, const int32_t* const* d_vals,
                     long long cap, const long long* level_rows, const int32_t* d_perm, long long n_orig, int stem_k,
                     int mask_groups, long long masked_min_rows, int32_t* d_arena, size_t arena_words, void* stream);

size_t cv_sp_scene_plan_words(long long n, int stem_k, int mask_groups, long long masked_min_rows);
int cv_sp_scene_plan(const int32_t* d_input, long long n, int32_t* d_perm, int32_t* d_inv, int32_t* const* d_coords,
                     unsigned long long* const* d_keys, int32_t* const* d_vals, long long cap, int32_t* d_counts,
                     int32_t* h_counts, int stem_k, int mask_groups, long long masked_min_rows, int32_t* d_arena,
                     size_t arena_words, cv_scene_maps* offsets, void* d_sort_ws, size_t sort_ws_bytes, void* d_levels_ws,
                     size_t levels_ws_bytes, void* stream);

typedef struct cv_scene_plan_layout {
    long long cap;
    long long perm, inv, coords[5], vals[5], counts, arena;
    long long int_words, key_words;
    size_t sort_ws_bytes, levels_ws_bytes;
} cv_scene_plan_layout;
int cv_sp_scene_plan_layout(long long n, int stem_k, int mask_groups, long long masked_min_rows, cv_scene_plan_layout* out);
#define CV_NET_MAP_SLOTS 15
#define CV_NET_PERM_SLOTS 9
int cv_sp_scene_plan_slots(const cv_scene_plan_layout* layout, const cv_scene_maps* offsets, const long long* level_rows,
                           long long min_rows, const int32_t* d_ibuf, const int32_t** maps, const int32_t** perms);
size_t cv_sp_scene_conv_workspace_bytes(const long long* level_rows, const int* masked, int mask_groups, int max_channels);

typedef struct cv_net_buf {
    int level, channels, rows_level;
    int hl;
} cv_net_buf;
typedef struct cv_net_op {
    int in_buf, in_col, cin;
    int out_buf, out_col, cout;
    int res_buf, res_col;
    int map, K;
    int perm, perm_groups;
    int relu;
    const float* weight;
    const float* scale;
    const float* shift;
    const void* weight_x6;
    int in2_buf, in2_col, cin2;
    const void* weight2_x6;
    int weight_pieces;
    float acc_scale;
} cv_net_op;
size_t cv_net_arena_bytes(const cv_net_buf* bufs, int n_bufs, const long long* level_rows, int n_levels);
int cv_net_run_f32(const cv_net_op* ops, int n_ops, const cv_net_buf* bufs, int n_bufs, const long long* level_rows,
                   int n_levels, void* d_arena, size_t arena_bytes, const void* const* ext_ptr, const int* ext_ld,
                   const int32_t* const* maps, int n_maps, const int32_t* const* perms, int n_perms,
                   void* d_ws, size_t ws_bytes, int32_t* range_flag, void* stream);

typedef struct cv_net_model_params {
    const void* weight_x6;
    const void* weight2_x6;
    const float* scale;
    const float* shift;
    float acc_scale;
    int reserved[3];
} cv_net_model_params;
size_t cv_net_models_params_bytes(int n_ops, int K);
int cv_net_models_params_fill(const cv_net_op* const* ops, int n_ops, int K, void* h_params, size_t params_bytes);
size_t cv_net_models_arena_bytes(const cv_net_buf* bufs, int n_bufs, const long long* level_rows, int n_levels, int K);
size_t cv_net_models_workspace_bytes(size_t one_model_bytes, int K);
int cv_net_run_models_f32(const cv_net_op* const* ops, const cv_net_buf* const* bufs, int n_ops, int n_bufs, int K,
                          const long long* level_rows, int n_levels, void* d_arena, size_t arena_bytes,
                          const void* const* const* ext_ptr, const int* ext_ld, const int32_t* const* maps, int n_maps,
                          const int32_t* const* perms, int n_perms, void* d_ws, size_t ws_bytes, int32_t* range_flag,
                          const void* d_params, int params_ld, void* stream);

int cv_sp_mask_keys(const int32_t* d_nbr, long long n, int K, int j_begin, int j_end, long long* d_keys,
                    void* stream);

int cv_sp_mask_perms(const int32_t* d_nbr, long long n, int K, int groups, int32_t* d_perm, void* d_ws,
                     size_t ws_bytes, int with_map, void* stream);

int cv_sp_transpose_map(const int32_t* d_nbr, long long n_out, int K, long long n_in, int32_t* d_nbr_t, void* stream);
size_t cv_sp_wgrad_workspace_bytes(long long n_out, int cin, int cout, int K);
// ... 197 lines not shown
```

Measured before the change: 693.3.

## Use per-level mask group counts with nine line groups on coarse levels

```diff
diff --git a/canonicalvoting_amd/_lib.py b/canonicalvoting_amd/_lib.py
--- a/canonicalvoting_amd/_lib.py
+++ b/canonicalvoting_amd/_lib.py
@@ -320,6 +320,7 @@
     "cv_sp_set_ablation": (ctypes.c_int, [ctypes.c_int]),
     "cv_sp_set_option": (ctypes.c_int, [ctypes.c_char_p, ctypes.c_longlong, ctypes.POINTER(ctypes.c_longlong)]),
     "cv_sp_get_option": (ctypes.c_int, [ctypes.c_char_p, ctypes.POINTER(ctypes.c_longlong)]),
+    "cv_sp_level_mask_groups": (ctypes.c_int, [ctypes.c_int, ctypes.c_longlong, ctypes.c_int, ctypes.c_longlong, ctypes.c_int]),
     "cv_sp_pack_weights_x6_f32": (ctypes.c_int, [vp, ctypes.c_int, ctypes.c_int, ctypes.c_int, vp, vp, vp]),
     "cv_sp_pack_weights_h2_f32": (ctypes.c_int, [vp, ctypes.c_int, ctypes.c_int, ctypes.c_int, vp, ctypes.c_int, vp, vp]),
     "cv_sp_pack_weights_bf16_f32": (ctypes.c_int, [vp, ctypes.c_int, ctypes.c_int, ctypes.c_int, vp, vp, vp]),
diff --git a/canonicalvoting_amd/csrc/conv_prep.hip b/canonicalvoting_amd/csrc/conv_prep.hip
--- a/canonicalvoting_amd/csrc/conv_prep.hip
+++ b/canonicalvoting_amd/csrc/conv_prep.hip
@@ -136,14 +136,14 @@
     int m = 0;
     for (int j = jb; j < je; ++j)
         if (nbr[row * K + j] >= 0) m |= 1 << (j - jb);
-    if (je - jb <= 7) m |= __popc(m) << 7;
+    if (je - jb > 3 && je - jb <= 7) m |= __popc(m) << 7;
     (void)n;
     return m;
 }
 
 __device__ __forceinline__ int group_mask_of_word(int word, int jb, int je) {
     int m = (int)(((unsigned)word >> jb) & ((1u << (je - jb)) - 1u));
-    if (je - jb <= 7) m |= __popc(m) << 7;
+    if (je - jb > 3 && je - jb <= 7) m |= __popc(m) << 7;
     return m;
 }
 
diff --git a/canonicalvoting_amd/csrc/cv_common.h b/canonicalvoting_amd/csrc/cv_common.h
--- a/canonicalvoting_amd/csrc/cv_common.h
+++ b/canonicalvoting_amd/csrc/cv_common.h
@@ -94,12 +94,12 @@
 int cv_net_run_ex(const cv_net_op* ops, int n_ops, const cv_net_buf* bufs, int n_bufs, const long long* level_rows,
                   int n_levels, void* d_arena, size_t arena_bytes, const void* const* ext_ptr, const int* ext_ld,
                   const int32_t* const* maps, int n_maps, const int32_t* const* perms, int n_perms,
-                  void* d_ws, size_t ws_bytes, int32_t* range_flag, bool plan_maps, void* stream);
+                  void* d_ws, size_t ws_bytes, int32_t* range_flag, const int* plan_groups, void* stream);
 int cv_net_run_models_ex(const cv_net_op* const* ops, const cv_net_buf* const* bufs, int n_ops, int n_bufs, int K,
                          const long long* level_rows, int n_levels, void* d_arena, size_t arena_bytes,
                          const void* const* const* ext_ptr, const int* ext_ld, const int32_t* const* maps, int n_maps,
                          const int32_t* const* perms, int n_perms, void* d_ws, size_t ws_bytes, int32_t* range_flag,
-                         const void* d_params, int params_ld, bool plan_maps, void* stream);
+                         const void* d_params, int params_ld, const int* plan_groups, void* stream);
 int cv_sp_mask_perms_batch(const CvPermJob* jobs, int n_jobs, void* d_ws, size_t ws_bytes, void* stream,
                            bool pre_zeroed);
 
diff --git a/canonicalvoting_amd/csrc/net_exec.cpp b/canonicalvoting_amd/csrc/net_exec.cpp
--- a/canonicalvoting_amd/csrc/net_exec.cpp
+++ b/canonicalvoting_amd/csrc/net_exec.cpp
@@ -20,28 +20,48 @@
 int net_run(const cv_net_op* ops, int n_ops, const cv_net_buf* bufs, int n_bufs, const long long* level_rows, int n_levels,
             void* d_arena, size_t arena_bytes, const void* const* ext_ptr, const int* ext_ld, const int32_t* const* maps,
             int n_maps, const int32_t* const* perms, int n_perms, void* d_ws, size_t ws_bytes, int32_t* range_flag,
-            const NetModels* nm, bool plan_maps, void* stream);
+            const NetModels* nm, const int* plan_groups, void* stream);
 
 }
 
 extern "C" {
 
+static size_t mask_perm_words(int groups) {
+    return groups > 1 ? (size_t)groups * (1 + (27 + groups - 1) / groups) + (groups + 3) / 4 : 0;
+}
+
+static void scene_level_groups(const long long* rows, int mask_groups, long long masked_min_rows, int* groups) {
+    for (int i = 0; i < 5; ++i) groups[i] = cv_sp_level_mask_groups(i, rows[i], mask_groups, masked_min_rows, 0);
+}
+
 static void scene_maps_layout(const long long* rows, int stem_k, int mask_groups, long long masked_min_rows, cv_scene_maps* o,
-                              size_t* total) {
+                              size_t* total, bool bound = false) {
     size_t off = 0;
     auto take = [&](size_t words) { const size_t at = off; off += cv_align_up(words, 64); return (long long)at; };
     const size_t K5 = (size_t)stem_k * stem_k * stem_k;
-    const size_t mp_w = mask_groups > 1 ? (size_t)mask_groups * (1 + (27 + mask_groups - 1) / mask_groups) + (mask_groups + 3) / 4 : 0;
+    int groups[5];
+    scene_level_groups(rows, mask_groups, masked_min_rows, groups);
+    auto perm_words = [&](int i) {
+        size_t w = mask_perm_words(groups[i]) * (size_t)rows[i];
+        if (bound && i > 0 && masked_min_rows > 1) {
+            const long long below = std::min(rows[i], masked_min_rows - 1);
+            w = std::max(w, mask_perm_words(cv_sp_level_mask_groups(i, below, mask_groups, masked_min_rows, 0)) * (size_t)below);
+        }
+        return w;
+    };
     o->stem = take((size_t)rows[0] * K5);
     o->k3[0] = take((size_t)rows[0] * 28);
-    o->mask_perm[0] = (mask_groups > 1 && rows[0] >= masked_min_rows) ? take(mp_w * rows[0]) : -1;
-    o->scratch = take((size_t)(5 * std::max(mask_groups, 1) + 4) * 2048);
+    o->mask_perm[0] = groups[0] > 1 ? take(perm_words(0)) : -1;
+    int line_groups = 0;
+    for (int i = 3; i < 5; ++i)
+        if (cv_sp_level_mask_groups(i, 128, mask_groups, 129, 0) == CV_COARSE_LINE_GROUPS) line_groups += CV_COARSE_LINE_GROUPS;
+    o->scratch = take((size_t)(5 * std::max(mask_groups, 1) + 4 + line_groups) * 2048);
     o->bitmap = take((size_t)CV_BITMAP_WORDS);
     o->out = -1;
     for (int i = 0; i < 4; ++i) o->down[i] = take((size_t)rows[i + 1] * 8);
     for (int i = 1; i < 5; ++i) o->k3[i] = take((size_t)rows[i] * 28);
     for (int i = 0; i < 4; ++i) o->up[i] = take((size_t)rows[3 - i] * 8);
-    for (int i = 1; i < 5; ++i) o->mask_perm[i] = (mask_groups > 1 && rows[i] >= masked_min_rows) ? take(mp_w * rows[i]) : -1;
+    for (int i = 1; i < 5; ++i) o->mask_perm[i] = (groups[i] > 1 || (bound && perm_words(i) > 0)) ? take(perm_words(i)) : -1;
     for (int i = 0; i < 4; ++i) o->up_perm[i] = take((size_t)rows[3 - i]);
     *total = off;
 }
@@ -84,8 +104,10 @@
 }
 
 static int scene_maps_coarse(int32_t* const* d_coords, const unsigned long long* const* d_keys, const int32_t* const* d_vals,
-                             long long cap, const long long* level_rows, int mask_groups, const cv_scene_maps& o,
-                             int32_t* d_arena, void* stream, bool from_plan) {
+                             long long cap, const long long* level_rows, int mask_groups, long long masked_min_rows,
+                             const cv_scene_maps& o, int32_t* d_arena, void* stream, bool from_plan) {
+    int level_groups[5];
+    scene_level_groups(level_rows, mask_groups, masked_min_rows, level_groups);
     CvMapJob mj[CV_MAX_MAP_JOBS];
     int nm = 0;
     for (int i = 0; i < 4; ++i)
@@ -105,9 +127,9 @@
     int np = 0, groups = 0;
     for (int i = 1; i < 5; ++i)
         if (o.mask_perm[i] >= 0) {
-            pj[np++] = {d_arena + o.k3[i], level_rows[i], 27, mask_groups, d_arena + o.mask_perm[i], 1,
+            pj[np++] = {d_arena + o.k3[i], level_rows[i], 27, level_groups[i], d_arena + o.mask_perm[i], 1,
                         scene_mask_words(d_arena, o, i, level_rows[i])};
-            groups += mask_groups;
+            groups += level_groups[i];
         }
     for (int i = 0; i < 4; ++i) {
         pj[np++] = {d_arena + o.up[i], level_rows[3 - i], 8, 1, d_arena + o.up_perm[i], 0, nullptr};
@@ -129,7 +151,8 @@
     int rc = scene_maps_level0(d_coords, d_keys, d_vals, cap, n_orig, d_perm, stem_k, mask_groups, o, d_arena,
                                 nullptr, stream);
     if (rc != CV_OK) return rc;
-    return scene_maps_coarse(d_coords, d_keys, d_vals, cap, level_rows, mask_groups, o, d_arena, stream,  false);
+    return scene_maps_coarse(d_coords, d_keys, d_vals, cap, level_rows, mask_groups, masked_min_rows, o, d_arena, stream,
+                              false);
 }
 
 namespace {
@@ -172,7 +195,7 @@
     const long long rows[5] = {n, n, n, n, n};
     cv_scene_maps o;
     size_t total = 0;
-    scene_maps_layout(rows, stem_k, mask_groups, masked_min_rows, &o, &total);
+    scene_maps_layout(rows, stem_k, mask_groups, masked_min_rows, &o, &total,  true);
     return total;
 }
 
@@ -201,7 +224,10 @@
     for (int i = 0; i < 5; ++i) maps[5 + i] = ap + off.k3[i];
     for (int i = 0; i < 4; ++i) maps[10 + i] = ap + off.up[i];
     maps[14] = d_ibuf + layout->inv;
-    for (int i = 0; i < 5; ++i) perms[i] = (off.mask_perm[i] >= 0 && level_rows[i] >= min_rows) ? ap + off.mask_perm[i] : nullptr;
+    for (int i = 0; i < 5; ++i) {
+        const bool lines = cv_sp_level_mask_groups(i, level_rows[i], 2, level_rows[i] + 1, 0) == CV_COARSE_LINE_GROUPS;
+        perms[i] = (off.mask_perm[i] >= 0 && (level_rows[i] >= min_rows || lines)) ? ap + off.mask_perm[i] : nullptr;
+    }
     for (int i = 0; i < 4; ++i) perms[5 + i] = ap + off.up_perm[i];
     return CV_OK;
 }
@@ -210,7 +236,8 @@
     if (!level_rows || !masked) return 0;
     size_t bytes = 0;
     for (int i = 0; i < 5; ++i) {
-        if (masked[i]) bytes = std::max(bytes, (size_t)4 * mask_groups * (size_t)level_rows[i] * max_channels + 256);
+        const int groups = masked[i] > 1 ? masked[i] : mask_groups;
+        if (masked[i]) bytes = std::max(bytes, (size_t)4 * groups * (size_t)level_rows[i] * max_channels + 256);
         bytes = std::max(bytes, cv_sp_conv_workspace_bytes(std::min<long long>(level_rows[i], 128 * 384 - 1), max_channels, 27));
     }
     return bytes;
@@ -266,7 +293,8 @@
     scene_maps_layout(rows, stem_k, mask_groups, masked_min_rows, &o, &total);
     CV_REQUIRE(arena_words >= total, CV_ENOMEM, "scene map arena too small");
     *offsets = o;
-    return scene_maps_coarse(d_coords, d_keys, d_vals, cap, rows, mask_groups, o, d_arena, stream,  true);
+    return scene_maps_coarse(d_coords, d_keys, d_vals, cap, rows, mask_groups, masked_min_rows, o, d_arena, stream,
+                              true);
 }
 
 extern "C" {
@@ -286,7 +314,7 @@
                    const int32_t* const* maps, int n_maps, const int32_t* const* perms, int n_perms,
                    void* d_ws, size_t ws_bytes, int32_t* range_flag, void* stream) {
     return cv_net_run_ex(ops, n_ops, bufs, n_bufs, level_rows, n_levels, d_arena, arena_bytes, ext_ptr, ext_ld, maps, n_maps, perms,
-                         n_perms, d_ws, ws_bytes, range_flag,  false, stream);
+                         n_perms, d_ws, ws_bytes, range_flag,  nullptr, stream);
 }
 
 }
@@ -294,9 +322,9 @@
 int cv_net_run_ex(const cv_net_op* ops, int n_ops, const cv_net_buf* bufs, int n_bufs, const long long* level_rows,
                   int n_levels, void* d_arena, size_t arena_bytes, const void* const* ext_ptr, const int* ext_ld,
                   const int32_t* const* maps, int n_maps, const int32_t* const* perms, int n_perms,
-                  void* d_ws, size_t ws_bytes, int32_t* range_flag, bool plan_maps, void* stream) {
+                  void* d_ws, size_t ws_bytes, int32_t* range_flag, const int* plan_groups, void* stream) {
     return net_run(ops, n_ops, bufs, n_bufs, level_rows, n_levels, d_arena, arena_bytes, ext_ptr, ext_ld, maps, n_maps, perms,
-                   n_perms, d_ws, ws_bytes, range_flag, nullptr, plan_maps, stream);
+                   n_perms, d_ws, ws_bytes, range_flag, nullptr, plan_groups, stream);
 }
 
 extern "C" {
@@ -336,7 +364,7 @@
                           const int32_t* const* perms, int n_perms, void* d_ws, size_t ws_bytes, int32_t* range_flag,
                           const void* d_params, int params_ld, void* stream) {
     return cv_net_run_models_ex(ops, bufs, n_ops, n_bufs, K, level_rows, n_levels, d_arena, arena_bytes, ext_ptr, ext_ld, maps, n_maps,
-                                perms, n_perms, d_ws, ws_bytes, range_flag, d_params, params_ld,  false, stream);
+                                perms, n_perms, d_ws, ws_bytes, range_flag, d_params, params_ld,  nullptr, stream);
 }
 
 }
@@ -345,7 +373,7 @@
                          const long long* level_rows, int n_levels, void* d_arena, size_t arena_bytes,
                          const void* const* const* ext_ptr, const int* ext_ld, const int32_t* const* maps, int n_maps,
                          const int32_t* const* perms, int n_perms, void* d_ws, size_t ws_bytes, int32_t* range_flag,
-                         const void* d_params, int params_ld, bool plan_maps, void* stream) {
+                         const void* d_params, int params_ld, const int* plan_groups, void* stream) {
     CV_REQUIRE(K >= 1 && K <= CV_MAX_CATEGORIES, CV_EINVAL, "number of models out of range (%d, 1..%d)", K, CV_MAX_CATEGORIES);
     CV_REQUIRE(ops && bufs && level_rows && d_arena && ext_ptr && n_ops > 0 && n_bufs > 0 && n_levels > 0, CV_EINVAL,
                "bad network program arguments");
@@ -384,7 +412,7 @@
     const size_t ws_one = K > 1 ? ws_stride : ws_bytes;
     NetModels nm = {K, ext_ptr, arena_one, ws_stride, static_cast<const cv_net_model_params*>(d_params), params_ld};
     return net_run(ops[0], n_ops, bufs[0], n_bufs, level_rows, n_levels, d_arena, arena_one, ext_ptr[0], ext_ld, maps, n_maps,
-                   perms, n_perms, d_ws, ws_one, range_flag, &nm, plan_maps, stream);
+                   perms, n_perms, d_ws, ws_one, range_flag, &nm, plan_groups, stream);
 }
 
 namespace {
@@ -392,7 +420,7 @@
 int net_run(const cv_net_op* ops, int n_ops, const cv_net_buf* bufs, int n_bufs, const long long* level_rows, int n_levels,
             void* d_arena, size_t arena_bytes, const void* const* ext_ptr, const int* ext_ld, const int32_t* const* maps,
             int n_maps, const int32_t* const* perms, int n_perms, void* d_ws, size_t ws_bytes, int32_t* range_flag,
-            const NetModels* nm, bool plan_maps, void* stream) {
+            const NetModels* nm, const int* plan_groups, void* stream) {
     CV_REQUIRE(ops && bufs && level_rows && d_arena && n_ops > 0 && n_bufs > 0 && n_levels > 0, CV_EINVAL,
                "bad network program arguments");
     CV_REQUIRE(arena_bytes >= cv_net_arena_bytes(bufs, n_bufs, level_rows, n_levels), CV_ENOMEM, "arena too small");
@@ -462,8 +490,9 @@
         if (perm) {
             d.row_perm = perm;
             d.perm_groups = o.perm_groups;
-            d.perm_has_map = o.perm_groups > 1;
-            if (plan_maps && d.perm_has_map && o.K == 27 && d.nbr) d.valid_words = d.nbr + out.rows * 27;
+            if (plan_groups && o.perm < 5 && o.K == 27 && o.perm_groups > 1 && plan_groups[o.perm] > 1) d.perm_groups = plan_groups[o.perm];
+            d.perm_has_map = d.perm_groups > 1;
+            if (plan_groups && d.perm_has_map && o.K == 27 && d.nbr) d.valid_words = d.nbr + out.rows * 27;
         }
         int rc;
         if (nm) {
diff --git a/canonicalvoting_amd/csrc/scene_exec.cpp b/canonicalvoting_amd/csrc/scene_exec.cpp
--- a/canonicalvoting_amd/csrc/scene_exec.cpp
+++ b/canonicalvoting_amd/csrc/scene_exec.cpp
@@ -60,6 +60,7 @@
     float mn[3]; int dims[3]; size_t cells;
     const int32_t* maps[CV_NET_MAP_SLOTS]; const int32_t* perms[CV_NET_PERM_SLOTS];
     size_t conv_ws_b;
+    int groups[5];
 
     template <class D> explicit SceneFront(const D* d)
         : d_coords4(d->d_coords4), n(d->n), d_points(d->d_points), res(d->res), stem_k(d->stem_k), mask_groups(d->mask_groups),
@@ -104,9 +105,8 @@
         if (rc != CV_OK) return rc;
         for (int k = 0; k < 3; ++k) r->dims[k] = dims[k];
         cells = (size_t)dims[0] * dims[1] * dims[2];
-        int masked[5];
-        for (int i = 0; i < 5; ++i) masked[i] = off.mask_perm[i] >= 0;
-        conv_ws_b = cv_sp_scene_conv_workspace_bytes(rows, masked, mask_groups, max_channels);
+        for (int i = 0; i < 5; ++i) groups[i] = off.mask_perm[i] >= 0 ? cv_sp_level_mask_groups(i, rows[i], mask_groups, masked_min_rows, 0) : 0;
+        conv_ws_b = cv_sp_scene_conv_workspace_bytes(rows, groups, mask_groups, max_channels);
         return cv_sp_scene_plan_slots(&lay, &off, rows, masked_min_rows, ibuf, maps, perms);
     }
 };
@@ -173,7 +173,7 @@
     const void* ext_ptr[2] = {d->d_feats, d->d_out_feats};
     const int ext_ld[2] = {d->feats_ld, d->out_ld};
     rc = cv_net_run_ex(d->ops, d->n_ops, d->bufs, d->n_bufs, f.rows, 5, arena, arena_b, ext_ptr, ext_ld, f.maps, CV_NET_MAP_SLOTS,
-                       f.perms, CV_NET_PERM_SLOTS, conv_ws, f.conv_ws_b, d->use_range_flag ? d_flag : nullptr,  true, stream);
+                       f.perms, CV_NET_PERM_SLOTS, conv_ws, f.conv_ws_b, d->use_range_flag ? d_flag : nullptr,  f.groups, stream);
     if (rc != CV_OK) return rc;
     clock.lap(1);
     CV_HIP_CHECK(clock.mark(1));
@@ -305,7 +305,7 @@
         rc = cv_net_run_models_ex(d->ops + m0, d->bufs + m0, d->n_ops[0], d->n_bufs[0], g, f.rows, 5, arena, arena_all, ext_tab, ext_ld,
                                   f.maps, CV_NET_MAP_SLOTS, f.perms, CV_NET_PERM_SLOTS, conv_ws, conv_ws_all,
                                   d->use_range_flag ? d_flags + 16 * m0 : nullptr,
-                                  static_cast<const cv_net_model_params*>(d->d_model_params) + m0, K,  true, stream);
+                                  static_cast<const cv_net_model_params*>(d->d_model_params) + m0, K,  f.groups, stream);
         if (rc != CV_OK) return rc;
     }
     for (int k = 0; G == 0 && k < K; ++k) {
@@ -313,7 +313,7 @@
         const int ext_ld[2] = {d->feats_ld, d->out_ld};
         rc = cv_net_run_ex(d->ops[k], d->n_ops[k], d->bufs[k], d->n_bufs[k], f.rows, 5, arena, arena_b, ext_ptr, ext_ld, f.maps,
                            CV_NET_MAP_SLOTS, f.perms, CV_NET_PERM_SLOTS, conv_ws, f.conv_ws_b,
-                           d->use_range_flag ? d_flags + 16 * k : nullptr,  true, stream);
+                           d->use_range_flag ? d_flags + 16 * k : nullptr,  f.groups, stream);
         if (rc != CV_OK) return rc;
     }
     clock.lap(1);
diff --git a/canonicalvoting_amd/csrc/sparse_conv.hip b/canonicalvoting_amd/csrc/sparse_conv.hip
--- a/canonicalvoting_amd/csrc/sparse_conv.hip
+++ b/canonicalvoting_amd/csrc/sparse_conv.hip
@@ -223,6 +223,7 @@
 std::atomic<long long> g_opt_hd_mask{getenv("CV_HD") ? atoll(getenv("CV_HD")) : 4};
 std::atomic<long long> g_opt_hd_min_rows{getenv("CV_HD_MIN_ROWS") ? atoll(getenv("CV_HD_MIN_ROWS")) : 16384};
 std::atomic<long long> g_opt_hd_shape{getenv("CV_HD_SHAPE") ? atoll(getenv("CV_HD_SHAPE")) : 2};
+std::atomic<long long> g_opt_coarse_groups{getenv("CV_COARSE_GROUPS") ? atoll(getenv("CV_COARSE_GROUPS")) : 0};
 
 int launch_rows(ConvArgs a, const int NB, bool vec, hipStream_t st, ModelArgs* ma, int models) {
     dim3 grid((unsigned)((a.n_out + TM - 1) / TM), (unsigned)((a.cout + NB * 32 - 1) / (NB * 32)),
@@ -322,13 +323,22 @@
 static std::atomic<long long>* option_named(const char* name) {
     return !strcmp(name, "hd_mask") ? &g_opt_hd_mask : !strcmp(name, "hd_min_rows") ? &g_opt_hd_min_rows :
            !strcmp(name, "hd_shape") ? &g_opt_hd_shape : !strcmp(name, "zskip") ? &g_opt_zskip :
-           !strcmp(name, "zskip_launches") ? &g_zskip_launches : nullptr;
+           !strcmp(name, "zskip_launches") ? &g_zskip_launches : !strcmp(name, "coarse_groups") ? &g_opt_coarse_groups : nullptr;
+}
+
+int cv_sp_level_mask_groups(int level, long long rows, int mask_groups, long long masked_min_rows, int split_target_wgs) {
+    if (mask_groups <= 1 || rows <= 0) return 0;
+    if (rows >= masked_min_rows) return mask_groups;
+    const long long mode = g_opt_coarse_groups.load(std::memory_order_relaxed);
+    const long long target = split_target_wgs > 0 ? split_target_wgs : split_target();
+    const bool level_ok = (level == 3 && mode >= 1) || (level == 4 && mode >= 2);
+    return level_ok && rows >= TM && target <= 256 ? CV_COARSE_LINE_GROUPS : 0;
 }
 
 int cv_sp_set_option(const char* name, long long value, long long* previous) {
     CV_REQUIRE(name, CV_EINVAL, "null option name");
     std::atomic<long long>* o = option_named(name);
-    CV_REQUIRE(o, CV_EINVAL, "unknown option '%s' (hd_mask, hd_min_rows, hd_shape, zskip, zskip_launches)", name);
+    CV_REQUIRE(o, CV_EINVAL, "unknown option '%s' (hd_mask, hd_min_rows, hd_shape, zskip, zskip_launches, coarse_groups)", name);
     const long long before = o->exchange(value, std::memory_order_relaxed);
     if (previous) *previous = before;
     return CV_OK;
@@ -363,7 +373,8 @@
 size_t cv_sp_conv_workspace_bytes(long long n_out, int cout, int K) {
     if (n_out <= 0 || cout <= 0 || K <= 0) return 0;
     const size_t one = sizeof(float) * (size_t)n_out * (size_t)cout;
-    return 256 + std::min<size_t>(64 * one, std::max<size_t>((size_t)48 << 20, 3 * one));
+    const size_t groups = n_out < 16384 ? CV_COARSE_LINE_GROUPS : 3;
+    return 256 + std::min<size_t>(64 * one, std::max<size_t>((size_t)48 << 20, groups * one));
 }
 
 int cv_sp_conv_f32(const cv_conv_desc* d, void* stream) { return conv_dispatch(d, nullptr, stream); }
diff --git a/canonicalvoting_amd/me/__init__.py b/canonicalvoting_amd/me/__init__.py
--- a/canonicalvoting_amd/me/__init__.py
+++ b/canonicalvoting_amd/me/__init__.py
@@ -33,7 +33,8 @@
 
 
 class _FusedPlan:
-    __slots__ = ("keep", "counts", "cap", "stem_k", "groups", "off", "layout", "map_ptrs", "perm_ptrs", "views")
+    __slots__ = ("keep", "counts", "cap", "stem_k", "groups", "off", "layout", "map_ptrs", "perm_ptrs", "views", "level_groups",
+                 "line_ptrs")
 
 
 class CoordinateManager:
@@ -171,14 +172,15 @@
 
     def fused_fast(self, stem_k=5):
         cache = self.__dict__.setdefault("_fused_cache", {})
+        L = _lib.lib()
+        G = self.plan_mask_groups()
         mmr = masked_min_rows()
-        if (stem_k, mmr) in cache:
-            return cache[(stem_k, mmr)]
-        L = _lib.lib()
+        key = (stem_k, mmr) + tuple(int(L.cv_sp_level_mask_groups(i, 128, G, 129, 0)) for i in (3, 4))
+        if key in cache:
+            return cache[key]
         dev = self.device
         n = self._input.shape[0]
         NL = CoordinateManager.NUM_LEVELS
-        G = self.plan_mask_groups()
         lay = _lib.ScenePlanLayout()
         _lib.check(L.cv_sp_scene_plan_layout(n, stem_k, G, mmr, ctypes.byref(lay)), "cv_sp_scene_plan_layout")
         ibuf = torch.empty(lay.int_words, dtype=torch.int32, device=dev)
@@ -202,12 +204,16 @@
         plan.keep = (ibuf, kbuf)
         plan.counts = [int(counts_h[i]) for i in range(NL)]
         plan.cap, plan.stem_k, plan.groups, plan.off, plan.layout = lay.cap, stem_k, G, off, lay
+        plan.level_groups = [int(L.cv_sp_level_mask_groups(i, plan.counts[i], G, mmr, 0)) if off.mask_perm[i] >= 0 else 0
+                             for i in range(NL)]
         maps, perms = (vp * _lib.NET_MAP_SLOTS)(), (vp * _lib.NET_PERM_SLOTS)()
         _lib.check(L.cv_sp_scene_plan_slots(ctypes.byref(lay), ctypes.byref(off), (ctypes.c_int64 * NL)(*plan.counts), 0, vp(ib),
                                             maps, perms), "cv_sp_scene_plan_slots")
-        plan.map_ptrs, plan.perm_ptrs = list(maps), list(perms)
+        lines = [g > 1 and g != G for g in plan.level_groups]
+        plan.line_ptrs = [p if ln else None for p, ln in zip(list(perms)[:5], lines)]
+        plan.map_ptrs, plan.perm_ptrs = list(maps), [None if ln else p for p, ln in zip(list(perms)[:5], lines)] + list(perms)[5:]
         plan.views = None
-        cache[(stem_k, mmr)] = plan
+        cache[key] = plan
         self._fused = plan
         return plan
 
@@ -236,10 +242,11 @@
                 if i == 0 or off.mask_perm[i] >= 0:
                     cm_s._maps[("k", 3, 1 << i, 1)]._cv_valid_words = arena[off.k3[i] + 27 * c[i]:off.k3[i] + 28 * c[i]]
                 if off.mask_perm[i] >= 0:
-                    mp = view(off.mask_perm[i], G, c[i])
+                    Gi = plan.level_groups[i]
+                    mp = view(off.mask_perm[i], Gi, c[i])
                     mp._cv_has_map = True
                     mp._cv_from_plan = True
-                    cm_s._maps[("mp", 3, 1 << i, G)] = mp
+                    cm_s._maps[("mp", 3, 1 << i, Gi)] = mp
                     cm_s._maps[("k", 3, 1 << i, 1)]._cv_mask_perms = mp
             plan.views = (cm_s, stem_map, out_map)
         return plan.views
diff --git a/canonicalvoting_amd/minkunet.py b/canonicalvoting_amd/minkunet.py
--- a/canonicalvoting_amd/minkunet.py
+++ b/canonicalvoting_amd/minkunet.py
@@ -140,6 +140,13 @@
             return v
         return self.MASKED_MIN_ROWS if self.MASKED_MIN_ROWS is not None else ME.CoordinateManager.MASKED_MIN_ROWS
     MASK_GROUPS = ME.CoordinateManager.MASK_GROUPS
+
+    def level_groups(self, counts):
+        L, mmr = _lib.lib(), self.masked_min_rows()
+        if self.MASK_GROUPS <= 1:
+            return [self.MASK_GROUPS if c >= mmr else 0 for c in counts[:5]]
+        return [int(L.cv_sp_level_mask_groups(i, int(c), self.MASK_GROUPS, mmr, 0)) for i, c in enumerate(counts[:5])]
+
     USE_PROGRAM = os.environ.get("CV_NET_PROGRAM", "1") != "0"
     FUSE_DOWNSAMPLE = os.environ.get("CV_FUSE_DOWNSAMPLE", "1") != "0"
     PIECES = 2 if os.environ.get("CV_CONV_H2", "1") != "0" else 3
@@ -172,7 +179,8 @@
         dev = x.F.device
         exp = self.BLOCK.expansion
         n = [cm.num_rows(1 << i) for i in range(5)]
-        perms = lambda ts, rows: cm.mask_perms(3, ts, self.MASK_GROUPS) if rows >= self.masked_min_rows() else None
+        groups = dict(zip((1, 2, 4, 8, 16), self.level_groups(n)))
+        perms = lambda ts, rows: cm.mask_perms(3, ts, groups[ts]) if groups[ts] >= 1 else None
         up_c = [self.PLANES[4 + i] for i in range(4)]
         skip_c = (self.PLANES[2] * exp, self.PLANES[1] * exp, self.PLANES[0] * exp, self.INIT_DIM)
         cat = [torch.empty((n[3 - i], up_c[i] + skip_c[i]), dtype=torch.float32, device=dev) for i in range(4)]
@@ -330,16 +338,38 @@
         return 1 if ME.COMPUTE_DTYPE == "bf16" else self.PIECES
 
     def launch_args(self, plan, level_orders=None, max_planes=None):
-        masked = [c >= self.masked_min_rows() for c in plan.counts[:5]]
-        orders = plan.perm_ptrs[:5] if level_orders is None else level_orders
+        groups = self.level_groups(plan.counts)
+        masked = [g >= 1 for g in groups]
+        if level_orders is None:
+            orders = [(ln if ln is not None else o) if g == pg else None
+                      for o, ln, g, pg in zip(plan.perm_ptrs[:5], plan.line_ptrs, groups, plan.level_groups)]
+        else:
+            orders = level_orders
         if any(m and o is None for m, o in zip(masked, orders)):
             return None
         perm_ptrs = [o if m else None for m, o in zip(masked, orders)] + plan.perm_ptrs[5:]
         rows = (ctypes.c_int64 * 5)(*plan.counts)
-        sorted_levels = (ctypes.c_int * 5)(*[p is not None for p in perm_ptrs[:5]])
+        sorted_levels = (ctypes.c_int * 5)(*[g if p is not None else 0 for g, p in zip(groups, perm_ptrs[:5])])
         ws_bytes = _lib.lib().cv_sp_scene_conv_workspace_bytes(rows, sorted_levels, self.MASK_GROUPS,
                                                                max_planes or max(self.PLANES))
         return rows, ws_bytes, (vp * len(plan.map_ptrs))(*plan.map_ptrs), (vp * len(perm_ptrs))(*perm_ptrs)
+
+    def program_ops(self, c_ops, counts):
+        groups = self.level_groups(counts)
+        if all(g <= 1 or g == self.MASK_GROUPS for g in groups):
+            return c_ops
+        cache = self.__dict__.setdefault("_ops_by_groups", {})
+        hit = cache.get((id(c_ops), tuple(groups)))
+        if hit is None or hit[0] is not c_ops:
+            ops = type(c_ops)()
+            ctypes.memmove(ops, c_ops, ctypes.sizeof(c_ops))
+            for o in ops:
+                if self.PERM_K3 <= o.perm < self.PERM_K3 + 5 and o.K == 27 and groups[o.perm - self.PERM_K3] > 1:
+                    o.perm_groups = groups[o.perm - self.PERM_K3]
+            if len(cache) > 8:
+                cache.clear()
+            hit = cache[(id(c_ops), tuple(groups))] = (c_ops, ops)
+        return hit[1]
 
     def program_forward(self, x, pieces=None, defer_check=None):
         L = _lib.lib()
@@ -348,12 +378,13 @@
             pieces = self.eval_pieces()
         c_ops, c_bufs, _ = self._program(dev, pieces)
         plan = x.coordinate_manager.fused_fast(self.conv0p1s1.kernel_size)
+        c_ops = self.program_ops(c_ops, plan.counts)
         flag = ME.range_flag(dev) if pieces == 2 else None
         n = plan.counts
         args = self.launch_args(plan)
         if args is None:
             cm = x.coordinate_manager.fused_plan(self.conv0p1s1.kernel_size)[0]
-            wide = [cm.mask_perms(3, 1 << i, self.MASK_GROUPS) if n[i] >= self.masked_min_rows() else None for i in range(5)]
+            wide = [cm.mask_perms(3, 1 << i, g) if g >= 1 else None for i, g in enumerate(self.level_groups(n))]
             args = self.launch_args(plan, [w.data_ptr() if w is not None else None for w in wide])
         rows, ws_bytes, c_maps, c_perms = args
         feats = x.F.contiguous()
diff --git a/canonicalvoting_amd/pipeline.py b/canonicalvoting_amd/pipeline.py
--- a/canonicalvoting_amd/pipeline.py
+++ b/canonicalvoting_amd/pipeline.py
@@ -433,7 +433,8 @@
     with torch.cuda.device(dev):
         for k0 in range(0, K, G):
             g = min(G, K - k0)
-            ops = (vp * g)(*[ctypes.cast(p[0], vp) for p in progs[k0:k0 + g]])
+            ops_k = [m.program_ops(p[0], plan.counts) for m, p in zip(mods[k0:k0 + g], progs[k0:k0 + g])]
+            ops = (vp * g)(*[ctypes.cast(o, vp) for o in ops_k])
             bufs = (vp * g)(*[ctypes.cast(p[1], vp) for p in progs[k0:k0 + g]])
             ext = [(vp * 2)(feats.data_ptr(), y.data_ptr()) for y in ys[k0:k0 + g]]
             c_ext = (vp * g)(*[ctypes.cast(e, vp) for e in ext])
diff --git a/include/cv_hip.h b/include/cv_hip.h
--- a/include/cv_hip.h
+++ b/include/cv_hip.h
@@ -284,6 +284,8 @@
 int cv_sp_set_ablation(int bits);
 int cv_sp_set_option(const char* name, long long value, long long* previous);
 int cv_sp_get_option(const char* name, long long* value);
+#define CV_COARSE_LINE_GROUPS 9
+int cv_sp_level_mask_groups(int level, long long rows, int mask_groups, long long masked_min_rows, int split_target_wgs);
 
 typedef struct cv_scene_maps {
     long long stem, out, down[4], k3[5], up[4], mask_perm[5], up_perm[4], scratch;
diff --git a/profiles/coarse_groups/level_summary.py b/profiles/coarse_groups/level_summary.py
--- /dev/null
+++ b/profiles/coarse_groups/level_summary.py
@@ -0,0 +1,83 @@
+import collections
+import csv
+import glob
+import sys
+
+label, d = sys.argv[1:3]
+
+
+def find(pat):
+    f = glob.glob("%s/**/*%s" % (d, pat), recursive=True)
+    return sorted(f)[-1] if f else None
+
+
+def grid(r):
+    g = [int(r["Grid_Size_" + a]) // max(1, int(r["Workgroup_Size_" + a])) for a in "XYZ"]
+    return g
+
+
+def fam(r):
+    n = r["Kernel_Name"]
+    if "conv_finish_small" in n:
+        return "conv_finish_small"
+    if "conv_finish" in n:
+        return "conv_finish (other)"
+    if "conv_hd" in n:
+        return "conv_hd"
+    if "conv_hl" in n:
+        try:
+            gx, gy, gz = grid(r)
+        except (KeyError, ValueError):
+            return "conv_hl"
+        if 15 <= gx <= 24:
+            return "conv_hl ts8 (z=%d)" % gz
+        if 4 <= gx <= 7:
+            return "conv_hl ts16 (z=%d)" % gz
+        return "conv_hl mask-sorted" if gz == 3 and gx >= 64 else "conv_hl (other)"
+    if "mp_hist" in n or "mp_scatter" in n:
+        return "mp_* (orders)"
+    if "head_" in n:
+        return "head"
+    return None
+
+
+t = find("kernel_trace.csv")
+rows = list(csv.DictReader(open(t)))
+scenes = sum(1 for r in rows if "head_" in r["Kernel_Name"])
+dur = collections.defaultdict(float)
+wgs = collections.defaultdict(float)
+cnt = collections.Counter()
+tot = 0.0
+for r in rows:
+    dt = (int(r["End_Timestamp"]) - int(r["Start_Timestamp"])) * 1e-3
+    tot += dt
+    f = fam(r)
+    if f:
+        dur[f] += dt
+        cnt[f] += 1
+        try:
+            gx, gy, gz = grid(r)
+            wgs[f] += gx * gy * gz
+        except (KeyError, ValueError):
+            pass
+print("%s: %d kernels, %d scenes, %.1f us of kernel time per scene" % (label, len(rows), scenes, tot / max(scenes, 1)))
+ctr = collections.defaultdict(lambda: collections.defaultdict(float))
+c = find("counter_collection.csv")
+names = []
+if c:
+    by_id = {r.get("Dispatch_Id"): r for r in rows}
+    for r in csv.DictReader(open(c)):
+        base = by_id.get(r.get("Dispatch_Id"), r)
+        f = fam(base if "Grid_Size_Z" in base else r) or "(all other)"
+        ctr[f][r["Counter_Name"]] += float(r["Counter_Value"])
+        ctr["(every kernel)"][r["Counter_Name"]] += float(r["Counter_Value"])
+    names = sorted({k for v in ctr.values() for k in v})
+print("%-24s %9s %12s %11s %10s " % ("family", "launches", "us / launch", "us / scene", "wgs") + " ".join("%16s" % (n + " MB/sc") for n in names))
+for f in sorted(set(cnt) | set(ctr)):
+    if f == "head":
+        continue
+    n = cnt.get(f, 0)
+    print("%-24s %9.1f %12.2f %11.1f %10.0f " % (f, n / max(scenes, 1), dur[f] / max(n, 1), dur[f] / max(scenes, 1), wgs[f] / max(n, 1)) +
+          " ".join("%16.2f" % (ctr[f].get(k, 0.0) / 1024.0 / max(scenes, 1)) for k in names))
+coarse = sum(v for k, v in dur.items() if k.startswith("conv_hl ts"))
+print("conv_hl ts8 + ts16: %.1f us per scene" % (coarse / max(scenes, 1)))
diff --git a/profiles/coarse_groups/pricing.py b/profiles/coarse_groups/pricing.py
--- /dev/null
+++ b/profiles/coarse_groups/pricing.py
@@ -0,0 +1,58 @@
+import os
+import sys
+
+import numpy as np
+
+sys.path.insert(0, os.path.dirname(os.path.dirname(os.path.dirname(os.path.abspath(__file__)))))
+from canonicalvoting_amd.synth import make_scene
+from profiles.supertile_pricing import coarser, live_table, plan_order
+
+
+def units(live, groups, block):
+    n = len(live)
+    nblk = (n + block - 1) // block
+    pad = nblk * block - n
+    if groups == 0:
+        l2 = np.concatenate([live, np.zeros((pad, 27), bool)])
+        return int(l2.reshape(nblk, block, 27).any(1).sum()) / (27.0 * nblk)
+    w = 27 // groups
+    tot = 0
+    for g in range(groups):
+        lv = live[:, w * g:w * g + w]
+        mask = (lv * (1 << np.arange(w))).sum(1)
+        key = mask | (lv.sum(1) << 7) if w <= 7 else mask
+        l2 = np.concatenate([lv[np.argsort(key, kind="stable")], np.zeros((pad, w), bool)])
+        tot += int(l2.reshape(nblk, block, w).any(1).sum())
+    return tot / (27.0 * nblk)
+
+
+def dead_pairs(live, groups):
+    w = 27 // groups
+    return 1.0 - live.reshape(len(live), groups, w).any(2).mean()
+
+
+def main():
+    print("share of (row block, offset) units with a live pair; blocks of 128 / 32 rows; seeds 0 / 1")
+    print("%-6s %-13s %-11s %-13s %-25s %-25s %-13s" % ("level", "rows", "pairs live", "spatial 128", "3 groups 128, 32",
+                                                         "9 groups 128, 32", "dead (g, row) 9"))
+    rows = {}
+    for seed in (0, 1):
+        sc = make_scene(seed, n_points=80000, res=0.03)
+        c = plan_order(np.asarray(sc.coords, np.int64))
+        ts = 1
+        while ts < 16:
+            c = coarser(c, ts)
+            ts *= 2
+            if ts >= 4:
+                live = live_table(c, ts)
+                rows.setdefault(ts, []).append((len(c), live.mean(), units(live, 0, 128), units(live, 3, 128), units(live, 3, 32),
+                                                units(live, 9, 128), units(live, 9, 32), dead_pairs(live, 9)))
+    for ts in sorted(rows, reverse=True):
+        a, b = rows[ts]
+        pair = lambda i, f="%.2f": (f + " / " + f) % (a[i], b[i])
+        print("%-6s %-13s %-11s %-13s %-25s %-25s %-13s" % ("ts%d" % ts, pair(0, "%d"), pair(1), pair(2), pair(3) + ", " + pair(4),
+                                                             pair(5) + ", " + pair(6), pair(7)))
+
+
+if __name__ == "__main__":
+    main()
```

After: 692.5. No clear change (-0.1%).
